# WxuanYuan/diffusynth

Measured on AMD Instinct MI355X. Metric: denoising-steps/sec (batch x T) on 256x64 latents, higher is better.
Workload: dtype bf16x3; 1 GPU; BASELINE configs[2]: DiffSynthSampler.sample() wall-clock, production ConditionedUnet (random init, torch.manual_seed(0)), bf16x3 (fp32 tensors, dense convolutions as 3 bf16 MFMA terms with fp32 accumulation: meets 1e-3 vs the fp32 reference), batch 64/GPU, latent (4,256,64), text condition, CFG=6.0 (U-Net batch 128 per step), 33-step respaced ddpm schedule, Philox noise on device; global_batch=64, parallelism=batch-shard x1, weights replicated

## Files before the change

### diffusynth_amd/_lib.py

```python
import ctypes as C
import os
import re

_HERE = os.path.dirname(os.path.abspath(__file__))
_HEADER = os.path.join(os.path.dirname(_HERE), "include", "diffusynth_hip.h")
_LIBNAME = "libdiffusynth_hip.so"

DS_F32, DS_BF16 = 0, 1
ACT_NONE, ACT_GELU, ACT_SILU, ACT_RELU = 0, 1, 2, 3
from .conv_policy import (TILE_64x192, TILE_128x32, TILE_128x192, TILE_256x96, TILE_HALO3_256x96, TILE_HALO3_N16,
                          TILE_INIT7, TILE_QUAD_HALO3)

_SCALARS = {"int32_t": C.c_int32, "int": C.c_int, "float": C.c_float, "double": C.c_double, "int64_t": C.c_int64,
            "uint64_t": C.c_uint64, "size_t": C.c_size_t}


def _parse_structs(text):
    text = re.sub(r"/\*.*?\*/", "", text, flags=re.S)
    out = {}
    for body, name in re.findall(r"typedef\s+struct\s*\{(.*?)\}\s*(\w+)\s*;", text, flags=re.S):
        fields = []
        for decl in body.split(";"):
            decl = " ".join(decl.split())
            if not decl:
                continue
            if "*" in decl:
                names = decl.rsplit("*", 1)[1]
                ctype = C.c_void_p
            else:
                tname, names = decl.replace("const ", "").split(" ", 1)
                ctype = _SCALARS[tname]
            for n in names.split(","):
                fields.append((n.strip(), ctype))
        out[name] = type(name, (C.Structure,), {"_fields_": fields})
    return out


def _parse_defines(text, prefix):
    return {k: int(v) for k, v in re.findall(r"^#define\s+(%s\w*)\s+(-?\d+)\b" % prefix, text, flags=re.M)}


with open(_HEADER) as _f:
    _HEADER_TEXT = _f.read()
_STRUCTS = _parse_structs(_HEADER_TEXT)
SR = _parse_defines(_HEADER_TEXT, "DS_SR_")
CR = _parse_defines(_HEADER_TEXT, "DS_CR_")
DW_FAMILY = {v: k[6:].lower() for k, v in _parse_defines(_HEADER_TEXT, "DS_DW_").items()}
PV = _parse_defines(_HEADER_TEXT, "DS_PV_")
MIX_BLOCK = _parse_defines(_HEADER_TEXT, "DS_MIX_")["DS_MIX_BLOCK"]
TAIL = _parse_defines(_HEADER_TEXT, "DS_TAIL_")
ConvParams = _STRUCTS["ds_conv_params"]
PackConvParams = _STRUCTS["ds_pack_conv_params"]
DwconvParams = _STRUCTS["ds_dwconv_params"]
GnApplyParams = _STRUCTS["ds_gn_apply_params"]
AttnParams = _STRUCTS["ds_attn_params"]
StepParams = _STRUCTS["ds_step_params"]
StepRowsParams = _STRUCTS["ds_step_rows_params"]
DpmStepParams = _STRUCTS["ds_dpm_step_params"]
CfgRescaleParams = _STRUCTS["ds_cfg_rescale_params"]
CfgRescaleRowsParams = _STRUCTS["ds_cfg_rescale_rows_params"]
AttnFusedParams = _STRUCTS["ds_attn_fused_params"]
AttnX3Params = _STRUCTS["ds_attn_x3_params"]
VqAttnParams = _STRUCTS["ds_vq_attn_params"]

_P, _I, _F, _D, _SZ, _U64 = C.c_void_p, C.c_int, C.c_float, C.c_double, C.c_size_t, C.c_uint64
_PROTOS = {
    "ds_abi_version": (C.c_int, []),
    "ds_conv_igemm": (C.c_int, [C.POINTER(ConvParams), _P]),
    "ds_conv_splitk_reduce": (C.c_int, [C.POINTER(ConvParams), _P]),
    "ds_conv1x1_x3": (C.c_int, [C.POINTER(ConvParams), _P]),
    "ds_conv1x1_x3_stats_parts": (C.c_int, [C.POINTER(ConvParams)]),
    "ds_conv1x1_x3_weight_elems": (C.c_size_t, [_I, _I]),
    "ds_conv_stats_parts": (C.c_int, [C.POINTER(ConvParams)]),
    "ds_conv_tile_bn": (C.c_int, [_I]),
    "ds_pack_conv_weight": (C.c_int, [C.POINTER(PackConvParams), _P]),
    "ds_pack_conv_elems": (_SZ, [_I, _I, _I, _I, _I]),
    "ds_conv_fold_tables": (C.c_int, [_P, _P, _P, _P, _I, _I, _I, _I, _P, _P, _P]),
    "ds_dwconv7": (C.c_int, [C.POINTER(DwconvParams), _P]),
    "ds_dwconv_stats_parts": (C.c_int, [C.POINTER(DwconvParams)]),
    "ds_dwconv_launch_choice": (C.c_int, [C.POINTER(DwconvParams), C.POINTER(C.c_int32), C.POINTER(C.c_int32), C.POINTER(C.c_int32)]),
    "ds_pack_dw_weight": (C.c_int, [_P, _I, _P, _P]),
    "ds_pack_dw_weight_mfma": (C.c_int, [_P, _I, _P, _P]),
    "ds_split_planes": (C.c_int, [_P, _P, C.c_longlong, _I, _P]),
    "ds_gn_finalize": (C.c_int, [_P, _I, _I, _D, _F, _P, _P]),
    "ds_gn_stats": (C.c_int, [_P, _I, _I, _I, _I, _I, _F, _P, _P]),
    "ds_gn_stats_stream": (C.c_int, [_P, _I, _I, _I, _I, _I, _F, _P, _P, _P]),
    "ds_gn_stats_ws_floats": (_SZ, [_I, _I, _I]),
    "ds_gn_apply": (C.c_int, [C.POINTER(GnApplyParams), _P]),
    "ds_linattn_context": (C.c_int, [C.POINTER(AttnParams), _P]),
    "ds_linattn_output": (C.c_int, [C.POINTER(AttnParams), _P]),
    "ds_linattn_part_floats": (_SZ, [_I, _I, _I]),
    "ds_pack_attn_fused": (C.c_int, [_P, _P, _P, _P, _P, _I, _P]),
    "ds_attn_fused_context": (C.c_int, [C.POINTER(AttnFusedParams), _P]),
    "ds_attn_fused_output": (C.c_int, [C.POINTER(AttnFusedParams), _P]),
    "ds_attn_fused_stats_parts": (C.c_int, [C.POINTER(AttnFusedParams)]),
    "ds_attn_fused_generations": (C.c_int, [C.POINTER(AttnFusedParams)]),
    "ds_attn_fused_segments": (C.c_int, [_I, _I, _I]),
    "ds_attn_fused_segments_gen": (C.c_int, [_I, _I, _I, _I]),
    "ds_pack_attn_x3": (C.c_int, [_P, _P, _P, _I, _P]),
    "ds_attn_x3_context": (C.c_int, [C.POINTER(AttnX3Params), _P]),
    "ds_attn_x3_output": (C.c_int, [C.POINTER(AttnX3Params), _P]),
    "ds_attn_x3_stats_parts": (C.c_int, [C.POINTER(AttnX3Params)]),
    "ds_attn_x3_segments": (C.c_int, [_I, _I, _I]),
    "ds_vq_attn_segments": (C.c_int, [_I, _I, _I]),
    "ds_vq_attn_wfold_bytes": (_SZ, [_I, _I]),
    "ds_vq_attn_context": (C.c_int, [C.POINTER(VqAttnParams), _P]),
    "ds_vq_attn_output": (C.c_int, [C.POINTER(VqAttnParams), _P]),
    "ds_attn_x3_qplane_bytes": (_SZ, [_I, _I]),
    "ds_attn_x3_mfold_bytes": (_SZ, [_I, _I]),
    "ds_sinusoid": (C.c_int, [_P, _P, _I, _I, _P, _P]),
    "ds_linear": (C.c_int, [_P, _I, _P, _P, _I, _I, _I, _I, _P, _I, _P]),
    "ds_conv3x3_f32_n4_weight_floats": (C.c_size_t, [_I]),
    "ds_pack_conv3x3_f32_n4": (C.c_int, [_P, _P, _I, _I, _P, _P]),
    "ds_conv3x3_f32_n4": (C.c_int, [_P, _I, _I, _I, _I, _P, _P, _P]),
    "ds_activation": (C.c_int, [_P, C.c_size_t, _I, _P, _P]),
    "ds_add_layernorm": (C.c_int, [_P, _P, _P, _P, _I, _I, _F, _P, _P]),
    "ds_dup_batch": (C.c_int, [_P, _P, _SZ, _P]),
    "ds_nchw_to_nhwc": (C.c_int, [_P, _I, _I, _I, _I, _P, _I, _I, _P]),
    "ds_conv1x1_in_nchw": (C.c_int, [_P, _I, _I, _I, _P, _P, _I, _P, _P]),
    "ds_nhwc_to_nchw": (C.c_int, [_P, _I, _I, _I, _I, _I, _I, _P, _P]),
    "ds_ddim_step": (C.c_int, [C.POINTER(StepParams), _P]),
    "ds_step_rows": (C.c_int, [C.POINTER(StepRowsParams), _P]),
    "ds_dpm_step": (C.c_int, [C.POINTER(DpmStepParams), _P]),
    "ds_dpm_step_rows": (C.c_int, [C.POINTER(StepRowsParams), _P, _P]),
    "ds_cfg_rescale": (C.c_int, [C.POINTER(CfgRescaleParams), _P]),
    "ds_cfg_rescale_rows": (C.c_int, [C.POINTER(CfgRescaleRowsParams), _P]),
    "ds_philox_normal": (C.c_int, [_P, _SZ, _U64, _U64, _P]),
    "ds_gather_cols": (C.c_int, [_P, _I, _I, _P, _I, _P, _P]),
    "ds_vq_nearest": (C.c_int, [_P, _P, _P, _I, _I, _I, _I, _P, _P, _P]),
    "ds_vq_stats_ws_bytes": (_SZ, [_I]),
    "ds_vq_stats": (C.c_int, [_P, _P, _P, _I, _I, _I, _I, _F, _I, _P, _P, _P]),
    "ds_decoder_tail": (C.c_int, [_P, _I, _I, _I, _I, _P, _P]),
    "ds_dec_final": (C.c_int, [_P, _I, _I, _I, _I, _P, _I, _P, _P, _P, _P, _P, _P, _P, _P]),
    "ds_conv7x7_c4_weight_elems": (C.c_size_t, []),
    "ds_pack_conv7x7_c4": (C.c_int, [_P, _I, _I, _P, _P]),
    "ds_conv7x7_c4": (C.c_int, [_P, _I, _I, _I, _I, _P, _P, _P, _P]),
    "ds_pack_conv7x7_c4_x3": (C.c_int, [_P, _I, _I, _P, _P]),
    "ds_conv7x7_c4_x3": (C.c_int, [_P, _I, _I, _I, _P, _P, _P, _P]),
    "ds_conv3x3_c80_weight_elems": (C.c_size_t, []),
    "ds_pack_conv3x3_c80": (C.c_int, [_P, _I, _I, _P, _P]),
    "ds_conv3x3_c80": (C.c_int, [_P, _I, _I, _I, _P, _P, _P, _P, _I, _P, _P, _I, _I, _P, _P]),
    "ds_conv3x3_c80_stats_slots": (C.c_int, [_I, _I, _I]),
    "ds_conv3x3_c80_res": (C.c_int, [_P, _P, _I, _I, _I, _P, _P, _P, _P, _P]),
    "ds_convt4x4_c80_stats_slots": (C.c_int, [_I, _I, _I, _I]),
    "ds_gn_stats_finish": (C.c_int, [_P, _I, _I, _I, _I, _I, _F, _P, _P]),
    "ds_convt4x4_c80_weight_elems": (C.c_size_t, [_I]),
    "ds_pack_convt4x4_c80": (C.c_int, [_P, _I, _I, _P, _P]),
    "ds_convt4x4_c80": (C.c_int, [_P, _I, _I, _I, _I, _P, _P, _P, _P, _I, _P, _P, _P, _P]),
    "ds_istft_plus": (C.c_int, [_P, _I, _I, _I, _I, _P, _P, _P]),
    "ds_istft_ws_floats": (_SZ, [_I, _I, _I]),
    "ds_stft_plus": (C.c_int, [_P, _I, _I, _I, _I, _I, _P, _P]),
    "ds_stft_images_ws_floats": (_SZ, [_I, _I, _I]),
    "ds_stft_images": (C.c_int, [_P, _P, C.c_longlong, _I, _I, _I, _P, _P, _P, _P]),
    "ds_latent_image_ws_floats": (_SZ, [_I, _I]),
    "ds_latent_image": (C.c_int, [_P, _I, _I, _I, _I, _P, _P, _P]),
    "ds_pv_stft": (C.c_int, [_P, _P, _I, _I, C.c_longlong, C.c_longlong, _P, _P]),
    "ds_pv_vocode": (C.c_int, [_P, _P, _P, _P, _I, C.c_longlong, C.c_longlong, _P, _P]),
    "ds_pv_istft_ws_bytes": (_SZ, [C.c_longlong]),
    "ds_pv_istft": (C.c_int, [_P, _P, _I, _I, _I, C.c_longlong, C.c_longlong, _P, _P, _P]),
    "ds_resample_sinc": (C.c_int, [_P, _P, _P, _I, _I, C.c_longlong, C.c_longlong, _P, _P]),
    "ds_peak_normalize_ws_bytes": (_SZ, [_I, _I]),
    "ds_peak_normalize": (C.c_int, [_P, _P, _I, _I, C.c_longlong, _P, _P, _P]),
    "ds_mix_notes": (C.c_int, [_P, C.c_longlong, _P, _I, _P, _P, _I, _P, _I, _P]),
    "ds_lstm_ws_floats": (_SZ, [_I, _I]),
    "ds_lstm_layer": (C.c_int, [_P, C.c_longlong, C.c_longlong, _P, _I, _I, _I, _P, _P, _P, _P]),
    "ds_timbre_heads": (C.c_int, [_P, _I, _I, _I, _I, _I, _I, _P]),
    "ds_text_embed": (C.c_int, [_P, _I, _I, _I, _P, _I, _P, _I, _P, _P, _P, _I, _F, _P, _P]),
    "ds_text_attention": (C.c_int, [_P, _P, _I, _I, _I, _I, _I, _P, _P]),
    "ds_text_tail": (C.c_int, [_P, _I, _I, _I, _F, _P, _P]),
    "ds_bounds_report": (C.c_int, [C.c_char_p, _I, _I]),
}
_UNCHECKED = {"ds_conv3x3_f32_n4_weight_floats", "ds_bounds_report", "ds_abi_version", "ds_conv_stats_parts", "ds_conv1x1_x3_stats_parts", "ds_conv_tile_bn", "ds_dwconv_stats_parts", "ds_attn_fused_stats_parts", "ds_attn_fused_generations", "ds_attn_fused_segments", "ds_attn_fused_segments_gen", "ds_attn_x3_stats_parts", "ds_attn_x3_segments", "ds_vq_attn_segments", "ds_conv3x3_c80_stats_slots", "ds_convt4x4_c80_stats_slots"}
EXPORTS = sorted(list(_PROTOS) + ["ds_last_error_string"])

_lib = None


def lib_path():
    return os.path.join(_HERE, os.environ.get("DS_LIB", _LIBNAME))


class DsError(RuntimeError):
    pass


def load():
    global _lib
    if _lib is not None:
        return _lib
    path = lib_path()
    if not os.path.exists(path):
        raise DsError(f"{path} is missing: build it with `python -c 'import __graft_entry__ as g; g.build()'` "
                      "(hipcc --offload-arch=gfx950).  diffusynth_amd has no CPU fallback.")
    lib = C.CDLL(path)
    lib.ds_last_error_string.restype = C.c_char_p
    lib.ds_last_error_string.argtypes = []
    for name, (res, args) in _PROTOS.items():
        fn = getattr(lib, name)
        fn.restype, fn.argtypes = res, args
    _lib = lib
    return lib


def check(rc, what=""):
    if rc != 0:
        msg = load().ds_last_error_string().decode("utf-8", "replace")
        raise DsError(f"{what} failed with code {rc}: {msg}")


def call(name, *args):
    rc = getattr(load(), name)(*args)
    if name not in _UNCHECKED:
        check(rc, name)
    return rc


def ptr(t):
    return None if t is None else t.data_ptr()


def current_stream():
    import torch
    return C.c_void_p(torch.cuda.current_stream().cuda_stream)
```

### diffusynth_amd/conv_policy.py

```python
from collections import namedtuple

KSPLIT_FILL = 256
TILE_128x192, TILE_256x96, TILE_128x32, TILE_64x192 = 0, 1, 2, 3
TILE_HALO3_256x96, TILE_QUAD_HALO3, TILE_HALO3_N16, TILE_INIT7 = 11, 12, 13, 14
_IGEMM_BM_BN = {TILE_64x192: (64, 192), TILE_128x192: (128, 192), TILE_256x96: (256, 96)}


def up(x, m):
    return (x + m - 1) // m * m


class ConvLayer(namedtuple("ConvLayer", "Cout Cin cin_pad k transposed gain halo small_out bf16 split3")):
    bn = property(lambda s: 32 if s.small_out else 192 if s.Cout % 192 == 0 else 96)
    cout_pad = property(lambda s: up(s.Cout, s.bn))
    dense3x3 = property(lambda s: s.k == (3, 3) and not s.transposed and s.cin_pad == s.Cin and s.Cin % 32 == 0)
    k_order = property(lambda s: int(s.halo and s.bf16 and s.k == (3, 3) and not s.transposed and s.cin_pad % 32 == 0 and s.bn in (96, 192)))
    f32n4_fits = property(lambda s: not s.bf16 and not s.gain and s.dense3x3 and s.Cout <= 4)
    n16_fits = property(lambda s: s.bf16 and not s.gain and s.dense3x3 and s.Cout <= 16)
    x3_1x1_fits = property(lambda s: s.split3 and s.k == (1, 1) and not s.transposed and s.cin_pad == s.Cin and s.Cin % 32 == 0
                           and s.Cout % 8 == 0)
    split3_fits = property(lambda s: s.halo and s.split3 and s.dense3x3 and s.cout_pad % 96 == 0 and s.Cout % 8 == 0)
    init7_fits = property(lambda s: s.bf16 and s.k == (7, 7) and s.Cout == 96 and s.Cin <= 4 and s.cin_pad in (4, 8))
    init7x3_fits = property(lambda s: s.split3 and s.k == (7, 7) and s.Cout == 96 and s.Cin <= 4 and s.cin_pad == 4)

    @property
    def quad_fits(s):
        return ((s.bf16 or (s.split3 and s.Cout % 8 == 0)) and not s.gain and s.cin_pad == s.Cin and s.Cin % 32 == 0 and s.k == (4, 4)
                and ((s.transposed and (s.Cin // 32) % 6 == 0 and s.Cout % 96 == 0) or (not s.transposed and (s.Cin // 32) % 3 == 0)))


def igemm_tile(bn, npix, korder):
    if korder == 1:
        return TILE_HALO3_256x96
    if bn == 192:
        return TILE_64x192 if npix <= 1024 else TILE_128x192
    return TILE_256x96 if bn == 96 else TILE_128x32


def halo_patches(H, W):
    twl = 3
    while (1 << twl) < W and twl < 5:
        twl += 1
    return -(-H // (256 >> twl)) * -(-W // (1 << twl))


def _fill(blocks, factors):
    ks = 1
    if blocks < KSPLIT_FILL:
        for c in factors:
            ks = c
            if blocks * c >= KSPLIT_FILL:
                break
    return ks


def halo3_ksplit(B, H, W, cout_pad, ncc, split):
    ok = [c for c in ((2, 3, 4, 6, 8) if split else (2, 4, 8)) if ncc % c == 0 and ncc // c >= (1 if split else 2)]
    return _fill(halo_patches(H, W) * (cout_pad // 96) * B, ok)


def quad_ksplit(B, Ho, Wo, cout_pad, nch, split):
    ok = [c for c in ((2, 3, 4, 6, 8) if split else (2, 4, 8)) if nch % c == 0 and (nch // c) % 6 == 0]
    return _fill(halo_patches(Ho, Wo) * (cout_pad // 96) * B, ok)


def x3_1x1_ksplit(B, Ho, Wo, cout_pad, nq):
    ok = [c for c in (2, 3, 4, 6, 8) if nq // c >= 3 and (c - 1) * -(-nq // c) < nq]
    return _fill(-(-(Ho * Wo) // 256) * (cout_pad // 96) * B, ok)


def igemm_ksplit(B, tile, Ho, Wo, cout_pad, nq, phases):
    if tile not in _IGEMM_BM_BN:
        return 1
    bm, bn = _IGEMM_BM_BN[tile]
    blocks = -(-(Ho * Wo) // bm) * (cout_pad // bn) * B * phases
    ks = 1
    while ks < 8 and blocks * ks < 384 and nq // (ks * 2) >= 6:
        ks *= 2
    while ks > 1 and (ks - 1) * -(-nq // ks) >= nq:
        ks //= 2
    return ks


def conv_meta(tile, B, Ho, Wo, Cout, kh, kw, transposed, cin, cin_real, res_cin=0):
    flops = 2.0 * B * Ho * Wo * Cout * (16 if transposed else kh * kw) * min(cin, cin_real)
    if res_cin:
        flops += 2.0 * B * Ho * Wo * Cout * res_cin
    return (tile, flops, f"{kh}x{kw}{'T' if transposed else ''} {cin}->{Cout} @{Ho}x{Wo}" + (f" +1x1 {res_cin}" if res_cin else ""))
```

### diffusynth_amd/csrc/conv1x1_x3.hip

```cpp
#include "common.hpp"
#include "conv_halo3_common.hpp"

namespace {

constexpr int X3_OFF_XH = 0, X3_OFF_XL = BM * PSTR, X3_OFF_WH = 2 * BM * PSTR, X3_OFF_WL = X3_OFF_WH + B_BYTES, X3_OFF_SHL = X3_OFF_WL + B_BYTES;
constexpr int X3_OFF_RED = X3_OFF_SHL + SHL_BYTES, X3_LDS = X3_OFF_RED + 64;
constexpr int X3_XIT = BM * 8 / NT;
constexpr int X3_WIT = 2 * BN * 4 / NT;

static_assert(4 * EPI_F32_WAVE <= X3_OFF_SHL, "the epilogue's staging tiles reuse the x / w buffers, the shift table stays");

__global__ __launch_bounds__(NT, DS_MINBLK) void conv1x1_x3_kernel(const ds_conv_params p) {
    extern __shared__ __attribute__((aligned(16))) char smem[];
    float* const shl = reinterpret_cast<float*>(smem + X3_OFF_SHL);
    float* const red = reinterpret_cast<float*>(smem + X3_OFF_RED);
    const int tid = threadIdx.x, lane = tid & 63, wave = tid >> 6, m = lane & 15, q = lane >> 4;
    const int gy = p.cout_pad / BN, HW = p.H * p.W, gx = (HW + BM - 1) / BM, nwg = gridDim.x;
    int wid = blockIdx.x;
    if ((nwg & 7) == 0) wid = (wid & 7) * (nwg >> 3) + (wid >> 3);
    const int by = wid % gy, bxz = wid / gy, bx = bxz % gx;
    const int zb = bxz / gx, ksplit = p.ksplit > 1 ? p.ksplit : 1, kz = zb / p.B;
    const int b = zb - kz * p.B, n0 = by * BN, px0 = bx * BM;
    const int NC0 = p.C0 >> 5, NCC = (p.C0 + p.C1) >> 5;
    const int ncs = (NCC + ksplit - 1) / ksplit, c_lo = kz * ncs, c_hi = min(NCC, c_lo + ncs);
    const bool raw = p.ksplit > 1;

    const float* const sp0 = reinterpret_cast<const float*>(p.src0) + (size_t)b * HW * p.C0;
    const float* const sp1 = p.C1 ? reinterpret_cast<const float*>(p.src1) + (size_t)b * p.H1 * p.W1 * p.C1 : nullptr;
    unsigned off0[X3_XIT], off1[X3_XIT];
#pragma unroll
    for (int it = 0; it < X3_XIT; ++it) {
        const int px = px0 + (tid >> 3) + 32 * it;
        off0[it] = ((unsigned)(px * p.C0 + 4 * (tid & 7)) * 4u & 0x7fffffffu) | ((unsigned)(px >= HW) << 31);
        off1[it] = 0x80000000u;
        if (p.C1) {
            const int h = px / p.W - p.off_h1, w = px % p.W - p.off_w1;
            const unsigned bad = (unsigned)(px >= HW) | (unsigned)((unsigned)h >= (unsigned)p.H1) | (unsigned)((unsigned)w >= (unsigned)p.W1);
            off1[it] = ((unsigned)((h * p.W1 + w) * p.C1 + 4 * (tid & 7)) * 4u & 0x7fffffffu) | (bad << 31);
        }
    }
    const rsrc_t rs0 = __builtin_amdgcn_make_buffer_rsrc(const_cast<float*>(sp0), (short)0, HW * p.C0 * 4, 0x00020000);
    const rsrc_t rs1 = __builtin_amdgcn_make_buffer_rsrc(const_cast<float*>(p.C1 ? sp1 : sp0), (short)0, p.C1 ? p.H1 * p.W1 * p.C1 * 4 : 0, 0x00020000);
    const char* const wbase = reinterpret_cast<const char*>(p.wpk);
    const size_t wchunk = (size_t)2 * p.cout_pad * 64;
    f32x4 rx[X3_XIT];
    u32x4 rw[X3_WIT];
    auto load_chunk = [&](int cc) {
        const bool first = cc < NC0;
        const float* const s = first ? sp0 : sp1;
        const int c0 = (first ? cc : cc - NC0) * 32;
#if DS_BOUNDS
#pragma unroll
        for (int it = 0; it < X3_XIT; ++it) {
            const unsigned o = first ? off0[it] : off1[it];
            const bool in = o < 0x80000000u;
            const f32x4 v = DS_LD(f32x4, reinterpret_cast<const f32x4*>(reinterpret_cast<const char*>(s) + (in ? o + c0 * 4 : 0)), first ? DS_BX_SRC0 : DS_BX_SRC1);
            rx[it] = in ? v : f32x4{0.f, 0.f, 0.f, 0.f};
        }
#else
        (void)s;
#pragma unroll
        for (int it = 0; it < X3_XIT; ++it)
            rx[it] = __builtin_bit_cast(f32x4, __builtin_amdgcn_raw_buffer_load_b128(first ? rs0 : rs1, (int)((first ? off0[it] : off1[it]) + c0 * 4), 0, 0));
#endif
#pragma unroll
        for (int it = 0; it < X3_WIT; ++it) {
            const int piece = tid + it * NT, plane = piece / (BN * 4), r = piece - plane * (BN * 4);
            rw[it] = DS_LD(u32x4, reinterpret_cast<const u32x4*>(wbase + (size_t)cc * wchunk + ((size_t)plane * p.cout_pad + n0) * 64 + (size_t)r * 16), DS_BX_W);
        }
    };
    auto store_chunk = [&]() {
#pragma unroll
        for (int it = 0; it < X3_XIT; ++it) {
            const int pl = (tid >> 3) + 32 * it, e = tid & 7;
            const int a = pl * PSTR + ((((e >> 1) ^ (((pl >> 2) & 1) << 1))) << 4) + ((e & 1) << 3);
            const f32x4 v = rx[it];
            uint2 hi, lo;
            ds_split2(v[0], v[1], hi.x, lo.x);
            ds_split2(v[2], v[3], hi.y, lo.y);
            *reinterpret_cast<uint2*>(smem + X3_OFF_XH + a) = hi;
            *reinterpret_cast<uint2*>(smem + X3_OFF_XL + a) = lo;
        }
#pragma unroll
        for (int it = 0; it < X3_WIT; ++it) {
            const int piece = tid + it * NT, plane = piece / (BN * 4), r = piece - plane * (BN * 4), row = r >> 2, qq = r & 3;
            *reinterpret_cast<u32x4*>(smem + (plane ? X3_OFF_WL : X3_OFF_WH) + row * PSTR + ((qq ^ W_SWZ(row)) << 4)) = rw[it];
        }
    };

    load_chunk(c_lo);
    float gn_a = 1.f, gn_am = 0.f;
    const bool fold = p.gn_ab != nullptr && !raw;
    if (fold) {
        gn_a = DS_LD(float, p.gn_ab + 2 * b, DS_BX_GNAB);
        gn_am = DS_LD(float, p.gn_ab + 2 * b + 1, DS_BX_GNAB);
    }
    for (int e = tid; e < 10 * BN; e += NT) {
        float v = 0.f;
        const int n = n0 + e;
        if (e < BN && n < p.Cout) {
            if (fold) v = DS_LD(float, p.fold_t1 + n, DS_BX_T1) - gn_am * DS_LD(float, p.fold_t2 + n, DS_BX_T2);
            else if (p.bias && !raw) v = DS_LD(float, p.bias + n, DS_BX_BIAS);
        }
        shl[e] = v;
    }
    int xa[XT];
#pragma unroll
    for (int i = 0; i < XT; ++i) {
        const int pl = 64 * wave + 16 * i + m;
        xa[i] = pl * PSTR + ((q ^ (((pl >> 2) & 1) << 1)) << 4);
    }
    const int wa = W_ROW0(m) * PSTR + ((q ^ ((-(m >> 2)) & 3)) << 4);
    f32x4 acc[XT][WT];
#pragma unroll
    for (int i = 0; i < XT; ++i)
#pragma unroll
        for (int j = 0; j < WT; ++j) acc[i][j] = f32x4{0.f, 0.f, 0.f, 0.f};

    for (int cc = c_lo; cc < c_hi; ++cc) {
        store_chunk();
        __syncthreads();
        if (cc + 1 < c_hi) load_chunk(cc + 1);
        bf16x8 xh[XT], xl[XT];
#pragma unroll
        for (int i = 0; i < XT; ++i) {
            xh[i] = *reinterpret_cast<const bf16x8*>(smem + X3_OFF_XH + xa[i]);
            xl[i] = *reinterpret_cast<const bf16x8*>(smem + X3_OFF_XL + xa[i]);
        }
#pragma unroll
        for (int j = 0; j < WT; ++j) {
            const bf16x8 wh = *reinterpret_cast<const bf16x8*>(smem + X3_OFF_WH + wa + EPI_CH(j) * PSTR);
            const bf16x8 wl = *reinterpret_cast<const bf16x8*>(smem + X3_OFF_WL + wa + EPI_CH(j) * PSTR);
#pragma unroll
            for (int i = 0; i < XT; ++i) {
                acc[i][j] = __builtin_amdgcn_mfma_f32_16x16x32_bf16(wl, xh[i], acc[i][j], 0, 0, 0);
                acc[i][j] = __builtin_amdgcn_mfma_f32_16x16x32_bf16(wh, xl[i], acc[i][j], 0, 0, 0);
                acc[i][j] = __builtin_amdgcn_mfma_f32_16x16x32_bf16(wh, xh[i], acc[i][j], 0, 0, 0);
            }
        }
        __syncthreads();
    }

    auto coord2 = [&](int i, int mm) {
        ConvCoord c;
        const int px = px0 + 64 * wave + 16 * i + mm;
        c.ok = px < HW;
        c.ho = 0;
        c.wo = 0;
        c.pix = px;
        return c;
    };
    auto coord = [&](int i) { return coord2(i, m); };
    float s1 = 0.f, s2 = 0.f;
    char* const stage = smem + wave * EPI_F32_WAVE;
    if (raw) {
        ds_conv_params qp = p;
        qp.out = p.slab;
        qp.out_C = (p.Cout + 7) / 8 * 8;
        qp.out_c0 = 0;
        qp.res = nullptr;
        halo3_epilogue_rows_f32<false, false>(qp, acc, zb, n0, HW, shl, coord, coord2, stage, s1, s2, 1.0f, lane);
        return;
    }
    if (p.res) halo3_epilogue_rows_f32<false, true>(p, acc, b, n0, HW, shl, coord, coord2, stage, s1, s2, gn_a, lane);
    else halo3_epilogue_rows_f32<false, false>(p, acc, b, n0, HW, shl, coord, coord2, stage, s1, s2, gn_a, lane);
    if (p.stats_part) block_stats_write(s1, s2, red, p.stats_part + ((size_t)b * (gx * gy) + by * gx + bx) * 2);
}

}

extern "C" size_t ds_conv1x1_x3_weight_elems(int Cin, int Cout) { return (size_t)((Cin + 31) / 32) * 2 * ((Cout + BN - 1) / BN * BN) * 32; }

int ds_conv_splitk_parts(const ds_conv_params* p);
extern "C" int ds_conv1x1_x3_stats_parts(const ds_conv_params* p) {
    return p->ksplit > 1 ? ds_conv_splitk_parts(p) : ((p->H * p->W + BM - 1) / BM) * (p->cout_pad / BN);
}

extern "C" int ds_conv1x1_x3(const ds_conv_params* p, void* stream) {
    DS_REQUIRE(p && p->src0 && p->wpk && p->out, "conv1x1_x3: null pointer");
    DS_REQUIRE(p->KH == 1 && p->KW == 1 && p->stride == 1 && p->pad_h == 0 && p->pad_w == 0 && !p->transposed && p->Ho == p->H && p->Wo == p->W,
               "conv1x1_x3: 1x1 stride 1 only");
    DS_REQUIRE(p->B > 0 && p->H > 0 && p->W > 0 && p->Cout > 0, "conv1x1_x3: empty problem");
    DS_REQUIRE(p->batch_hint >= 0, "conv1x1_x3: batch_hint must be 0 or a batch (this launcher takes no decision from either), got %d", p->batch_hint);
    DS_REQUIRE(p->C0 > 0 && p->C0 % 32 == 0 && p->C1 >= 0 && p->C1 % 32 == 0, "conv1x1_x3: channel counts (%d,%d) must be multiples of 32", p->C0, p->C1);
    DS_REQUIRE(p->C1 == 0 || (p->src1 && p->H1 > 0 && p->W1 > 0), "conv1x1_x3: second source incomplete");
    DS_REQUIRE(p->cout_pad % BN == 0 && p->Cout <= p->cout_pad, "conv1x1_x3: cout_pad %d must be a multiple of %d", p->cout_pad, BN);
    DS_REQUIRE(p->flags == (DS_CONV_F_IN_F32 | DS_CONV_F_OUT_F32) && p->act == DS_ACT_NONE && !p->res_steps && !p->gn_part && !p->out_nchw_f32,
               "conv1x1_x3: fp32 in / fp32 out (flags = DS_CONV_F_IN_F32 | DS_CONV_F_OUT_F32), no activation, no fused res_conv, statistics through gn_ab");
    {
        const int nq = (p->C0 + p->C1) / 32, ks = p->ksplit, nqs = ks > 1 ? (nq + ks - 1) / ks : nq;
        DS_REQUIRE(ks <= 1 || (p->slab && (ks == 2 || ks == 3 || ks == 4 || ks == 6 || ks == 8) && (ks - 1) * nqs < nq),
                   "conv1x1_x3: ksplit=%d needs a slab, a value in {2, 3, 4, 6, 8} and no empty slice over %d chunks", ks, nq);
    }
    DS_REQUIRE(!p->gn_ab || (p->fold_t1 && p->fold_t2 && p->ncls == 1), "conv1x1_x3: the GroupNorm fold needs t1 / t2 tables with one border class");
    DS_REQUIRE(p->out_C % 4 == 0 && p->out_c0 % 4 == 0 && p->out_C >= p->out_c0 + p->Cout && p->Cout % 8 == 0, "conv1x1_x3: out_C / out_c0 multiples of 4, Cout a multiple of 8");
    DS_REQUIRE((long long)p->H * p->W * p->out_C * 4 < (1ll << 31) && (long long)p->H * p->W * p->C0 * 4 < (1ll << 31) && (long long)p->H1 * p->W1 * p->C1 * 4 < (1ll << 31),
               "conv1x1_x3: one sample of the output and of either source must stay below 2 GiB (32-bit buffer offsets)");
    if (!ds_aligned16(p->src0) || !ds_aligned16(p->wpk) || !ds_aligned16(p->out) || (p->C1 && !ds_aligned16(p->src1)) || (p->res && !ds_aligned16(p->res)))
        DS_FAIL(DS_EALIGN, "conv1x1_x3: tensors must be 16-byte aligned");
    hipStream_t st = reinterpret_cast<hipStream_t>(stream);
    const int gx = (p->H * p->W + BM - 1) / BM, gy = p->cout_pad / BN;
    dim3 grid(gx * gy * p->B * (p->ksplit > 1 ? p->ksplit : 1));
#if DS_BOUNDS
    {
        DsBxHost h(DS_K_CONV_IGEMM);
        const int NCC = (p->C0 + p->C1) / 32;
        h.set(DS_BX_SRC0, p->src0, (long long)p->B * p->H * p->W * p->C0 * 4);
        h.set(DS_BX_SRC1, p->C1 ? p->src1 : nullptr, (long long)p->B * p->H1 * p->W1 * p->C1 * 4);
        h.set(DS_BX_W, p->wpk, (long long)NCC * 2 * p->cout_pad * 64);
        if (p->ksplit > 1) h.set(DS_BX_OUT, p->slab, (long long)p->ksplit * p->B * p->H * p->W * ((p->Cout + 7) / 8 * 8) * 4);
        else h.set(DS_BX_OUT, p->out, (long long)p->B * p->H * p->W * p->out_C * 4);
        h.set(DS_BX_RES, p->res, (long long)p->B * p->H * p->W * p->out_C * 4);
        h.set(DS_BX_BIAS, p->bias, (long long)p->Cout * 4);
        h.set(DS_BX_T1, p->fold_t1, (long long)p->Cout * 4).set(DS_BX_T2, p->fold_t2, (long long)p->Cout * 4);
        h.set(DS_BX_GNAB, p->gn_ab, (long long)p->B * 2 * 4);
        h.set(DS_BX_STATS, p->stats_part, (long long)p->B * gx * gy * 2 * 4);
        h.publish(st);
    }
#endif
    DS_SET_MAX_LDS(conv1x1_x3_kernel, X3_LDS, "conv1x1_x3");
    hipLaunchKernelGGL(conv1x1_x3_kernel, grid, dim3(NT), X3_LDS, st, *p);
    DS_CHECK_LAUNCH("conv1x1_x3");
    return DS_OK;
}

#if DS_BOUNDS
extern "C" int ds_bounds_fetch_conv1x1_x3(ds_bounds_rec* out, int reset) { return ds_bounds_fetch_tu(out, reset); }
#endif
```

### diffusynth_amd/csrc/conv3x3_halo3.hip

```cpp
#include "common.hpp"
#ifndef DS_STAMP
#define DS_STAMP 0
#endif
#if DS_BOUNDS
void ds_conv_bounds_table(const ds_conv_params& p, int kernel, int stats_parts, ds_bx* out);
#endif

#include "conv_halo3_common.hpp"

namespace {

__device__ __attribute__((aligned(16))) float g_gelu_lut[GELU_TAB_N];

#ifdef DS_FORCE_VGPRS
#define DS_VGPR_ATTR __attribute__((amdgpu_num_vgpr(DS_FORCE_VGPRS)))
#else
#define DS_VGPR_ATTR
#endif
template <int TWL, bool HP, bool PAIR = false>
__global__ __launch_bounds__(NT, PAIR ? 1 : DS_MINBLK) DS_VGPR_ATTR void conv3x3_halo3_kernel(const ds_conv_params p) {
    static_assert(!PAIR || (HP && TWL == 3), "two samples per block: the 8 x 32 tile of the split-precision instantiation");
    using G = HG<TWL>;
    constexpr int TW = G::TW, TH = G::TH, HCP = G::HCP, NPX = G::NPX, H_IT = G::H_IT, HH0 = G::HH0, HH1 = G::HH1;
    extern __shared__ __attribute__((aligned(16))) char smem[];
    float* const shl = reinterpret_cast<float*>(smem + OFF_SHL);
    float* const red = reinterpret_cast<float*>(smem + OFF_B);

    const int tid = threadIdx.x, lane = tid & 63, wave = tid >> 6;
    const long st_k0 = DS_STAMP ? __builtin_amdgcn_s_memrealtime() : 0;
    const int m = lane & 15, q = lane >> 4;
    const int tiles_w = (p.W + TW - 1) >> TWL;
    const int gx = gridDim.x, gy = gridDim.y, nwg = gx * gy * gridDim.z;
    int wid = blockIdx.x + gx * (blockIdx.y + gy * blockIdx.z);
    if ((nwg & 7) == 0) wid = (wid & 7) * (nwg >> 3) + (wid >> 3);
    constexpr int NGROUP = 2;
    int by, bxz;
    if (gy % NGROUP == 0 && gy > NGROUP) {
        const int lo = wid % NGROUP, t = wid / NGROUP, nxz = gx * (int)gridDim.z;
        bxz = t % nxz;
        by = (t / nxz) * NGROUP + lo;
    } else {
        by = wid % gy;
        bxz = wid / gy;
    }
    const int bx = bxz % gx, bz = bxz / gx;
    const int th = bx / tiles_w, tw = bx - th * tiles_w;
    const int h0 = th * TH, w0 = tw * TW;
    const int ksplit = p.ksplit > 1 ? p.ksplit : 1;
    const int b = (PAIR ? 2 : 1) * (bz / ksplit), kz = bz - (bz / ksplit) * ksplit, n0 = by * BN;
    const bool has2 = PAIR && b + 1 < p.B;
    constexpr bool split_in = HP;
    const int Cin = p.C0, NSRC = Cin >> 5;
    const int NCC = (split_in ? NSRC + (NSRC >> 1) : NSRC) / ksplit;
    const int cc_lo = kz * NCC;
    const int nsteps = NCC * 9;
    auto src_chunk = [&](int cc) {
        const int v = cc_lo + cc;
        if (!split_in) return v;
        const int c = v / 3, j = v - 3 * c;
        return j == 2 ? (NSRC >> 1) + c : c;
    };

    const int NR = (HP || ksplit > 1) ? 0 : p.res_steps, R0 = p.res_C0 >> 5;
    const char* const wbase = reinterpret_cast<const char*>(p.wpk);
    const unsigned wbytes = (unsigned)(NCC * ksplit * 9 + p.res_steps) * p.cout_pad * 64;
    const rsrc_t rs_w = __builtin_amdgcn_make_buffer_rsrc(const_cast<char*>(wbase), (short)0, (int)wbytes, 0x00020000);

    unsigned hvo[H_IT];
    rsrc_t rs_h;
    const char* hbase;
    int h_buf = DS_BX_SRC0;
    auto use_source = [&](const void* ptr, int sH, int sW, int sC, int offh, int offw, bool centre_only, int bounds_buf) {
        hbase = reinterpret_cast<const char*>(ptr) + (size_t)b * sH * sW * sC * 2;
        rs_h = __builtin_amdgcn_make_buffer_rsrc(const_cast<char*>(hbase), (short)0, (int)((unsigned)sH * sW * sC * 2) * (has2 ? 2 : 1), 0x00020000);
        h_buf = bounds_buf;
#pragma unroll
        for (int it = 0; it < H_IT; ++it) {
            const int slot = tid + it * NT, hp = slot >> 2, dq = slot & 3;
            int hr = hp / HCP;
            const int hc = hp - hr * HCP;
            const int smp = PAIR ? (int)(hr >= 18) : 0;
            if constexpr (PAIR) hr -= 18 * smp;
            const int hi = h0 + hr - 1 - offh, wi = w0 + hc - 1 - offw;
            const unsigned ring = (unsigned)(hr < 1) | (unsigned)(hr > TH) | (unsigned)(hc < 1) | (unsigned)(hc > TW);
            const unsigned bad = (unsigned)(hp >= (PAIR ? 36 * HCP : NPX)) | (unsigned)(hc >= TW + 2) | ((unsigned)centre_only & ring) |
                                 (unsigned)((unsigned)hi >= (unsigned)sH) | (unsigned)((unsigned)wi >= (unsigned)sW) | (unsigned)(smp && !has2);
            hvo[it] = (((unsigned)(((smp * sH + hi) * sW + wi) * sC + dq * 8) * 2u) & 0x7fffffffu) | (bad << 31);
        }
    };
    unsigned h_so = 0;
    auto set_res_src = [&](int r) {
        if (r == R0 && r < NR) use_source(p.res_src1, p.res_H1, p.res_W1, p.res_C1, p.res_off_h1, p.res_off_w1, true, DS_BX_AUX1);
        if (r == NR) use_source(p.src0, p.H, p.W, Cin, 0, 0, false, DS_BX_SRC0);
        h_so = r == NR ? (unsigned)src_chunk(0) * 64u : (unsigned)(r < R0 ? r : r - R0) * 64u;
    };
    if (NR > 0) use_source(p.res_src0, p.H, p.W, p.res_C0, 0, 0, true, DS_BX_AUX0);
    else use_source(p.src0, p.H, p.W, Cin, 0, 0, false, DS_BX_SRC0);

    const int lds_h = OFF_H + (tid >> 2) * PSTR + (((tid & 3) ^ (((tid >> 4) & 1) << 1)) << 4);
    const int wr0 = tid >> 2, wr1 = 64 + (tid >> 2);
    const int bst0 = OFF_B + wr0 * PSTR + (((tid & 3) ^ W_SWZ(wr0)) << 4);
    const int bst1 = tid < BN * 4 - NT ? OFF_B + wr1 * PSTR + (((tid & 3) ^ W_SWZ(wr1)) << 4) : OFF_B + B_BYTES;
    const unsigned wvo0 = (unsigned)tid * 16u, wvo1 = tid < BN * 4 - NT ? (unsigned)(tid + NT) * 16u : VOFF_NONE;
    const unsigned wstep = (unsigned)p.cout_pad * 64u;
    const unsigned w_first = ((unsigned)(p.res_steps - NR + cc_lo * 9) * p.cout_pad + n0) * 64u, w_last = w_first + (unsigned)(nsteps + NR - 1) * wstep;
    unsigned w_pf = w_first;

    u32x4 rb[3][2], rh[H_IT];
    auto load_b = [&](auto slotc) {
        constexpr int sl = decltype(slotc)::value;
        rb[sl][0] = buf_ld16(rs_w, wbase, wvo0, w_pf, DS_BX_W);
        rb[sl][1] = buf_ld16(rs_w, wbase, wvo1, w_pf, DS_BX_W);
        const unsigned nx = w_pf + wstep;
        w_pf = nx < w_last ? nx : w_last;
    };
    auto store_b = [&](auto slotc, auto bufc) {
        constexpr int sl = decltype(slotc)::value, buf = decltype(bufc)::value;
        *reinterpret_cast<u32x4*>(smem + buf * B_STRIDE + bst0) = rb[sl][0];
        *reinterpret_cast<u32x4*>(smem + buf * B_STRIDE + bst1) = rb[sl][1];
    };
    auto load_halo_to = [&](u32x4* dst, auto halfc) {
        constexpr int half = decltype(halfc)::value, n = half ? HH1 : HH0;
#pragma unroll
        for (int k = 0; k < n; ++k) dst[k] = buf_ld16(rs_h, hbase, hvo[half * HH0 + k], h_so, h_buf);
    };
    auto load_halo = [&](auto halfc) { load_halo_to(rh, halfc); };
    auto store_halo_from = [&](const u32x4* src, auto bufc, auto halfc) {
        constexpr int buf = decltype(bufc)::value, half = decltype(halfc)::value, n = half ? HH1 : HH0;
#pragma unroll
        for (int k = 0; k < n; ++k) *reinterpret_cast<u32x4*>(smem + lds_h + buf * G::HB + (half * HH0 + k) * 64 * PSTR) = src[k];
    };
    auto store_halo = [&](auto bufc, auto halfc) { store_halo_from(rh, bufc, halfc); };

    int xb[XT];
#pragma unroll
    for (int i = 0; i < XT; ++i) {
        int row_l, col_l;
        halo_tile_rc<TWL>(wave, i, m, row_l, col_l);
        const int hp0 = (row_l + (PAIR ? 2 * (row_l >> 4) : 0)) * HCP + col_l;
        xb[i] = OFF_H + hp0 * PSTR + ((q ^ (((hp0 >> 2) & 1) << 1)) << 4);
    }
    static_assert(((HCP >> 2) & 1) == 1 && ((2 * HCP >> 2) & 1) == 0, "tap-row swizzle flips assume HCP / 4 odd");
    const int xm1 = ((m & 3) == 3) << 5, xm2 = ((m & 3) >= 2) << 5;
    const int xm1n = xm1 ^ 32, xm2n = xm2 ^ 32;
    const int bw = OFF_B + W_ROW0(m) * PSTR + ((q ^ ((-(m >> 2)) & 3)) << 4);

    bf16x8 fx[2][XT], fw[WT];
    auto read_x = [&](auto setc, auto tyc, auto txc, int imm) {
        constexpr int set = decltype(setc)::value, ty = decltype(tyc)::value, tx = decltype(txc)::value;
#pragma unroll
        for (int i = 0; i < XT; ++i) {
            int a = xb[i];
            if constexpr (HP) {
                if constexpr (tx == 1) a ^= xm1;
                if constexpr (tx == 2) a ^= xm2;
                if constexpr (ty == 1) {
                    if constexpr (tx != 0) asm volatile("" : "+v"(a));
                    a ^= 32;
                }
            } else {
                if constexpr (tx == 0 && ty == 1) a ^= 32;
                if constexpr (tx == 1) a ^= (ty == 1 ? xm1n : xm1);
                if constexpr (tx == 2) a ^= (ty == 1 ? xm2n : xm2);
            }
            fx[set][i] = *reinterpret_cast<const bf16x8*>(smem + a + (ty * HCP + tx) * PSTR + imm);
        }
    };
#ifndef DS_HALO3_ABL
#define DS_HALO3_ABL 0
#endif
    auto read_w = [&](int j, int imm) { fw[j] = *reinterpret_cast<const bf16x8*>(smem + bw + EPI_CH(j) * PSTR + imm); };
    f32x4 acc[XT][WT];
    auto mma_j = [&](auto setc, int j) {
        constexpr int set = decltype(setc)::value;
#pragma unroll
        for (int i = 0; i < XT; ++i) acc[i][j] = __builtin_amdgcn_mfma_f32_16x16x32_bf16(fw[j], fx[set][i], acc[i][j], 0, 0, 0);
    };
    using I0 = std::integral_constant<int, 0>;
    using I1 = std::integral_constant<int, 1>;
    using I2 = std::integral_constant<int, 2>;

    GnPartialLoads gnl;
    const bool raw = ksplit > 1;
    if (p.gn_part && !raw) gn_partials_issue(p.gn_part, p.gn_parts, b, gnl);
    const bool fold = !raw && CONV_FOLD(p);
    const int ncls = fold ? p.ncls : 1;
    constexpr int ST_IT = (10 * BN + NT - 1) / NT;
#if !DS_BOUNDS
    float t1v[ST_IT], t2v[ST_IT], rbv[ST_IT];
    {
        auto tab = [&](const float* ptr, int n) {
            return __builtin_amdgcn_make_buffer_rsrc(const_cast<char*>(ptr ? reinterpret_cast<const char*>(ptr) : wbase), (short)0, ptr ? n * 4 : 0, 0x00020000);
        };
        const bool use_bias = !fold && p.bias && !raw;
        const rsrc_t rs_t1 = tab(fold ? p.fold_t1 : (use_bias ? p.bias : nullptr), fold ? ncls * p.Cout : p.Cout);
        const rsrc_t rs_t2 = tab(fold ? p.fold_t2 : nullptr, ncls * p.Cout);
        const rsrc_t rs_rb = tab((NR > 0 && p.res_bias) ? p.res_bias : nullptr, p.Cout);
#pragma unroll
        for (int k = 0; k < ST_IT; ++k) {
            const int e = tid + k * NT, cls = e / BN, n = n0 + e - cls * BN;
            const unsigned bad = ((unsigned)(e >= ncls * BN) | (unsigned)(n >= p.Cout)) << 31;
            const unsigned o = (unsigned)((fold ? cls * p.Cout : 0) + n) * 4u;
            t1v[k] = __builtin_bit_cast(float, __builtin_amdgcn_raw_buffer_load_b32(rs_t1, (int)((o & 0x7fffffffu) | bad), 0, 0));
            t2v[k] = __builtin_bit_cast(float, __builtin_amdgcn_raw_buffer_load_b32(rs_t2, (int)((o & 0x7fffffffu) | bad), 0, 0));
            rbv[k] = NR > 0 ? __builtin_bit_cast(float, __builtin_amdgcn_raw_buffer_load_b32(rs_rb, (int)((((unsigned)n * 4u) & 0x7fffffffu) | bad), 0, 0)) : 0.f;
        }
    }
#endif
    const bool use_lut = !HP && G::LUT && p.act == DS_ACT_GELU && !raw;
    static_assert(GELU_TAB_N * 4 <= 2 * NT * 16 && GELU_TAB_N % 4 == 0, "the table is staged as two 16-byte vectors per thread");
    u32x4 lutv = {0u, 0u, 0u, 0u}, lutv2 = {0u, 0u, 0u, 0u};
    if (use_lut) {
        lutv = *reinterpret_cast<const u32x4*>(reinterpret_cast<const char*>(g_gelu_lut) + tid * 16);
        lutv2 = *reinterpret_cast<const u32x4*>(reinterpret_cast<const char*>(g_gelu_lut) + (NT + min(tid, GELU_TAB_N / 4 - NT - 1)) * 16);
    }
    const long st_p1 = DS_STAMP ? __builtin_amdgcn_s_memrealtime() : 0;
    u32x4 rh2[HH0];
    h_so = NR > 0 ? 0u : (unsigned)src_chunk(0) * 64u;
    load_halo_to(rh2, I0{});
    load_halo(I1{});
    load_b(I0{});
    load_b(I1{});
    float gn_a = 1.f, gn_am = 0.f;
    if (raw) {
    } else if (p.gn_part) gn_partials_finish(gnl, p.gn_part, p.gn_parts, p.gn_count, p.gn_eps, b, gn_a, gn_am);
    else if (p.gn_ab) {
        gn_a = DS_LD(float, p.gn_ab + 2 * b, DS_BX_GNAB);
        gn_am = DS_LD(float, p.gn_ab + 2 * b + 1, DS_BX_GNAB);
    }
    if constexpr (PAIR) {
        const int b1 = has2 ? b + 1 : b;
        float a1 = 1.f, am1 = 0.f;
        if (p.gn_part) gn_from_partials(p.gn_part, p.gn_parts, p.gn_count, p.gn_eps, b1, a1, am1);
        else if (p.gn_ab) {
            a1 = DS_LD(float, p.gn_ab + 2 * b1, DS_BX_GNAB);
            am1 = DS_LD(float, p.gn_ab + 2 * b1 + 1, DS_BX_GNAB);
        }
        if (tid == 0) {
            reinterpret_cast<float*>(smem + G::LDS)[0] = a1;
            reinterpret_cast<float*>(smem + G::LDS)[1] = am1;
        }
    }
#if DS_BOUNDS
    conv_shift_table<BN, 10, NT>(raw ? conv_kslice_view(p) : p, fold, n0, gn_am, NR > 0 ? p.res_bias : nullptr, shl);
#else
#pragma unroll
    for (int k = 0; k < ST_IT; ++k) {
        const int e = tid + k * NT;
        if (e < 10 * BN) shl[e] = (t1v[k] + rbv[k]) - gn_am * t2v[k];
    }
#endif
    const long st_p2 = DS_STAMP ? __builtin_amdgcn_s_memrealtime() : 0;
#pragma unroll
    for (int i = 0; i < XT; ++i)
#pragma unroll
        for (int j = 0; j < WT; ++j) acc[i][j] = f32x4{0.f, 0.f, 0.f, 0.f};
    if (use_lut) {
        *reinterpret_cast<u32x4*>(smem + G::OFF_LUT + tid * 16) = lutv;
        if (tid < GELU_TAB_N / 4 - NT) *reinterpret_cast<u32x4*>(smem + G::OFF_LUT + (NT + tid) * 16) = lutv2;
    }
    store_halo_from(rh2, I0{}, I0{});
    store_halo(I0{}, I1{});
    store_b(I0{}, I0{});
    store_b(I1{}, I1{});
    load_b(I2{});
    load_b(I0{});
    load_b(I1{});
    __syncthreads();

    if constexpr (!HP) if (NR > 0) {
        set_res_src(1);
        load_halo_to(rh, I0{});
        load_halo_to(rh + HH0, I1{});
        auto res_step = [&](auto hbc, auto phc, int r) {
            constexpr int hb = decltype(hbc)::value, ph = decltype(phc)::value, rs = (ph + 2) % 3;
            read_x(I0{}, I1{}, I1{}, hb * G::HB);
#pragma unroll
            for (int j = 0; j < WT; ++j) read_w(j, ph * B_STRIDE);
            __builtin_amdgcn_sched_barrier(0);
            store_halo_from(rh, std::integral_constant<int, hb ^ 1>{}, I0{});
            store_halo_from(rh + HH0, std::integral_constant<int, hb ^ 1>{}, I1{});
            store_b(std::integral_constant<int, rs>{}, std::integral_constant<int, rs>{});
            __builtin_amdgcn_sched_barrier(0);
            load_b(std::integral_constant<int, rs>{});
            if (r + 2 <= NR) {
                set_res_src(r + 2);
                __builtin_amdgcn_sched_barrier(0);
                load_halo_to(rh, I0{});
                load_halo_to(rh + HH0, I1{});
            }
            __builtin_amdgcn_sched_barrier(0);
#pragma unroll
            for (int j = 0; j < WT; ++j) mma_j(I0{}, j);
            __builtin_amdgcn_sched_barrier(0);
            __syncthreads();
        };
        for (int r = 0; r < NR; r += 6) {
            res_step(I0{}, I0{}, r);
            res_step(I1{}, I1{}, r + 1);
            res_step(I0{}, I2{}, r + 2);
            if (r + 3 < NR) {
                res_step(I1{}, I0{}, r + 3);
                res_step(I0{}, I1{}, r + 4);
                res_step(I1{}, I2{}, r + 5);
            }
        }
        const float inv_a = 1.0f / gn_a;
#pragma unroll
        for (int i = 0; i < XT; ++i)
#pragma unroll
            for (int j = 0; j < WT; ++j)
#pragma unroll
                for (int r = 0; r < 4; ++r) acc[i][j][r] *= inv_a;
    }
    const int par = HP ? 0 : (NR & 1);
    if (par) read_x(I1{}, I0{}, I0{}, G::HB);
    else read_x(I0{}, I0{}, I0{}, 0);
#pragma unroll
    for (int j = 0; j < WT; ++j) read_w(j, 0);

    auto chunk = [&](auto hbufc, auto keepc, auto fsc, int cc) {
        constexpr int hbuf = decltype(hbufc)::value, KEEP = decltype(keepc)::value, FS = decltype(fsc)::value;
        if constexpr (!KEEP) h_so = (unsigned)src_chunk(cc + 1 < NCC ? cc + 1 : cc) * 64u;
        auto step = [&](auto tapc) {
            constexpr int tap = decltype(tapc)::value;
            constexpr int rs = (tap + 2) % 3;
            constexpr int cur = (tap + FS) & 1;
            constexpr int ntap = (tap + 1) % 9, nty = ntap / 3, ntx = ntap % 3, nhb = (tap == 8 && !KEEP) ? (hbuf ^ 1) : hbuf;
            constexpr int nW = 2 + (KEEP ? 0 : (tap == 3 ? HH0 : (tap == 7 ? HH1 : 0))), nV = 2 + (KEEP ? 0 : (tap == 1 ? HH0 : (tap == 4 ? HH1 : 0)));
            if constexpr (tap == 3 && !KEEP) store_halo(std::integral_constant<int, hbuf ^ 1>{}, I0{});
            if constexpr (tap == 7 && !KEEP) store_halo(std::integral_constant<int, hbuf ^ 1>{}, I1{});
            store_b(std::integral_constant<int, rs>{}, std::integral_constant<int, rs>{});
            load_b(std::integral_constant<int, rs>{});
            if constexpr (tap == 1 && !KEEP) load_halo(I0{});
            if constexpr (tap == 4 && !KEEP) load_halo(I1{});
            mma_j(std::integral_constant<int, (DS_HALO3_ABL & 2) ? 0 : cur>{}, 0);
            if constexpr (!(DS_HALO3_ABL & 1)) read_w(0, ((tap + 1) % 3) * B_STRIDE);
            if constexpr (!(DS_HALO3_ABL & 2))
                read_x(std::integral_constant<int, cur ^ 1>{}, std::integral_constant<int, nty>{}, std::integral_constant<int, ntx>{}, nhb * G::HB);
#pragma unroll
            for (int j = 1; j < WT; ++j) {
                mma_j(std::integral_constant<int, (DS_HALO3_ABL & 2) ? 0 : cur>{}, j);
                if constexpr (!(DS_HALO3_ABL & 1)) read_w(j, ((tap + 1) % 3) * B_STRIDE);
            }
#pragma unroll
            for (int k = 0; k < nW; ++k) { SGB(SG_MFMA, 1); SGB(SG_DSW, 1); }
#pragma unroll
            for (int k = 0; k < nV; ++k) { SGB(SG_MFMA, 1); SGB(SG_VMEM, 1); }
            constexpr int L0 = nW + nV;
#pragma unroll
            for (int k = 0; k < 5; ++k) { SGB(SG_MFMA, 1); SGB(SG_DSR, 1); }
            constexpr int L1 = L0 + 5;
#pragma unroll
            for (int j = 1; j < WT; ++j) {
                const int before = (4 * j + 4 > L1 + j - 1 ? 4 * j + 4 : L1 + j - 1);
                const int prev = j == 1 ? L1 : (4 * (j - 1) + 4 > L1 + j - 2 ? 4 * (j - 1) + 4 : L1 + j - 2);
                if (before - prev == 1) SGB(SG_MFMA, 1);
                else if (before - prev == 2) SGB(SG_MFMA, 2);
                else if (before - prev == 3) SGB(SG_MFMA, 3);
                else if (before - prev == 4) SGB(SG_MFMA, 4);
                else if (before - prev == 5) SGB(SG_MFMA, 5);
                else if (before - prev == 6) SGB(SG_MFMA, 6);
                else if (before - prev == 7) SGB(SG_MFMA, 7);
                SGB(SG_DSR, 1);
            }
            __builtin_amdgcn_sched_barrier(0);
#if DS_BOUNDS || defined(DS_LGKM0)
            asm volatile("s_waitcnt lgkmcnt(0)" ::: "memory");
#else
            asm volatile("s_waitcnt lgkmcnt(10)" ::: "memory");
#endif
            if constexpr (!(DS_HALO3_ABL & 4)) __builtin_amdgcn_s_barrier();
            __builtin_amdgcn_sched_barrier(0);
        };
        step(std::integral_constant<int, 0>{});
        step(std::integral_constant<int, 1>{});
        step(std::integral_constant<int, 2>{});
        step(std::integral_constant<int, 3>{});
        step(std::integral_constant<int, 4>{});
        step(std::integral_constant<int, 5>{});
        step(std::integral_constant<int, 6>{});
        step(std::integral_constant<int, 7>{});
        step(std::integral_constant<int, 8>{});
    };
    long st_t0 = 0, st_r0 = 0;
    if constexpr (DS_STAMP) {
        st_t0 = __builtin_amdgcn_s_memtime();
        st_r0 = __builtin_amdgcn_s_memrealtime();
        __builtin_amdgcn_s_waitcnt(0xC07F);
    }
    if constexpr (HP) {
        int cc = 0;
        for (; cc + 6 <= NCC; cc += 6) {
            chunk(I0{}, I1{}, I0{}, cc);
            chunk(I0{}, I0{}, I1{}, cc + 1);
            chunk(I1{}, I0{}, I0{}, cc + 2);
            chunk(I0{}, I1{}, I1{}, cc + 3);
            chunk(I0{}, I0{}, I0{}, cc + 4);
            chunk(I1{}, I0{}, I1{}, cc + 5);
        }
        if (cc < NCC) {
            chunk(I0{}, I1{}, I0{}, cc);
            chunk(I0{}, I0{}, I1{}, cc + 1);
            chunk(I1{}, I0{}, I0{}, cc + 2);
        }
    } else {
        int cc0 = 0;
        if (par) {
            chunk(I1{}, I0{}, I1{}, 0);
            cc0 = 1;
        }
        for (int cc = cc0; cc < NCC; cc += 2) {
            chunk(I0{}, I0{}, I0{}, cc);
            if (cc + 1 < NCC) chunk(I1{}, I0{}, I1{}, cc + 1);
        }
    }

#pragma unroll
    for (int i = 0; i < XT; ++i) {
        asm volatile("" ::"v"(fx[0][i]));
        asm volatile("" ::"v"(fx[1][i]));
    }
#pragma unroll
    for (int j = 0; j < WT; ++j) asm volatile("" ::"v"(fw[j]));
    if constexpr (DS_STAMP) {
        const long st_t1 = __builtin_amdgcn_s_memtime();
        if (p.slab && lane == 0) {
            long* d = reinterpret_cast<long*>(p.slab) + ((size_t)(bz * gy + by) * gx + bx) * 32 + wave * 8;
            d[0] = st_t1 - st_t0; d[1] = st_p1 - st_k0; d[2] = st_p2 - st_k0; d[3] = nsteps;
            d[4] = st_r0 - st_k0; d[5] = __builtin_amdgcn_s_memrealtime() - st_r0; d[6] = st_k0;
        }
    }
    auto at = [&](int row_l, int col_l) {
        ConvCoord c;
        if constexpr (PAIR) {
            const int smp = row_l >> 4;
            c.ho = row_l & 15;
            c.wo = w0 + col_l;
            c.ok = c.ho < p.H && c.wo < p.W && (!smp || has2);
            c.pix = (smp * p.H + c.ho) * p.W + c.wo;
            return c;
        }
        c.ho = h0 + row_l;
        c.wo = w0 + col_l;
        c.ok = c.ho < p.H && c.wo < p.W;
        c.pix = c.ho * p.W + c.wo;
        return c;
    };
    auto coord2 = [&](int i, int mm) { int row_l, col_l; halo_tile_rc<TWL>(wave, i, mm, row_l, col_l); return at(row_l, col_l); };
    auto coord = [&](int i) { return coord2(i, m); };
    char* const stage = smem + OFF_H + wave * EPI_F32_WAVE;
    static_assert(4 * EPI_F32_WAVE <= 2 * G::HB, "the staging tiles fit the halo buffers");
    float s1 = 0.f, s2 = 0.f;
    const int outHW = p.H * p.W;
    const long st_e1 = DS_STAMP ? __builtin_amdgcn_s_memrealtime() : 0;
    const int out_mode = HP ? (p.flags >> 1) & 3 : 0;
    const float* shl_w = shl;
    float ga_w = gn_a;
    int b_e = b, outHW_e = outHW;
    if constexpr (PAIR) {
        const float gn_a1 = reinterpret_cast<const float*>(smem + G::LDS)[0], gn_am1 = reinterpret_cast<const float*>(smem + G::LDS)[1];
        float* const shl1 = reinterpret_cast<float*>(smem + OFF_H + 4 * EPI_F32_WAVE);
        static_assert(4 * EPI_F32_WAVE + SHL_BYTES <= 2 * G::HB, "the second shift table fits the halo buffers too");
        conv_shift_table<BN, 10, NT>(p, fold, n0, gn_am1, nullptr, shl1);
        __syncthreads();
        if (__builtin_amdgcn_readfirstlane(wave) >= 2) {
            shl_w = shl1;
            ga_w = gn_a1;
        }
        b_e = b >> 1;
        outHW_e = 2 * outHW;
    }
    if (raw) {
        halo3_epilogue_hp<DS_ACT_NONE, 2>(conv_kslice_view(p), acc, kz * p.B + b, n0, outHW, shl, coord, s1, s2, 1.0f, lane);
    } else if constexpr (HP) {
      if (out_mode == 1) {
        if (p.act == DS_ACT_GELU) halo3_epilogue_hp<DS_ACT_GELU, 1>(p, acc, b_e, n0, outHW_e, shl_w, coord, s1, s2, ga_w, lane);
        else halo3_epilogue_hp<DS_ACT_NONE, 1>(p, acc, b_e, n0, outHW_e, shl_w, coord, s1, s2, ga_w, lane);
      } else if (out_mode == 2) {
        if (p.res) halo3_epilogue_rows_f32<true, true>(p, acc, b_e, n0, outHW_e, shl_w, coord, coord2, stage, s1, s2, ga_w, lane);
        else halo3_epilogue_rows_f32<true, false>(p, acc, b_e, n0, outHW_e, shl_w, coord, coord2, stage, s1, s2, ga_w, lane);
      } else {
        if (p.act == DS_ACT_GELU) halo3_epilogue<DS_ACT_GELU, true, false>(p, acc, b_e, n0, outHW_e, shl_w, coord, s1, s2, ga_w, lane);
        else halo3_epilogue<DS_ACT_NONE, true, false>(p, acc, b_e, n0, outHW_e, shl_w, coord, s1, s2, ga_w, lane);
      }
    } else
    if (p.act == DS_ACT_GELU) {
        const char* const lut = smem + G::OFF_LUT;
        if (use_lut) {
            if (p.res) halo3_epilogue<DS_ACT_GELU, true, true, true>(p, acc, b, n0, outHW, shl, coord, s1, s2, gn_a, lane, lut);
            else halo3_epilogue<DS_ACT_GELU, true, false, true>(p, acc, b, n0, outHW, shl, coord, s1, s2, gn_a, lane, lut);
        } else {
            if (p.res) halo3_epilogue<DS_ACT_GELU, true, true>(p, acc, b, n0, outHW, shl, coord, s1, s2, gn_a, lane);
            else halo3_epilogue<DS_ACT_GELU, true, false>(p, acc, b, n0, outHW, shl, coord, s1, s2, gn_a, lane);
        }
    } else {
        if (p.res) halo3_epilogue_rows<DS_ACT_NONE, true, true>(p, acc, b, n0, outHW, shl, coord, coord2, stage, s1, s2, gn_a, lane);
        else halo3_epilogue<DS_ACT_NONE, true, false>(p, acc, b, n0, outHW, shl, coord, s1, s2, gn_a, lane);
    }
    long st_e2 = 0, st_e3 = 0;
    if constexpr (DS_STAMP) {
        st_e2 = __builtin_amdgcn_s_memrealtime();
        __builtin_amdgcn_s_waitcnt(0x0F70);
        st_e3 = __builtin_amdgcn_s_memrealtime();
    }
    __syncthreads();
    if (p.stats_part && !raw) {
        const int parts = gridDim.x * gridDim.y;
        if constexpr (PAIR) {
            s1 = wave_sum(s1);
            s2 = wave_sum(s2);
            if (lane == 0) {
                red[2 * wave] = s1;
                red[2 * wave + 1] = s2;
            }
            __syncthreads();
            if (lane == 0 && (wave == 0 || (wave == 2 && has2))) {
                float* const dst = p.stats_part + ((size_t)(b + (wave >> 1)) * parts + by * gx + bx) * 2;
                DS_ST(float, dst, DS_BX_STATS, red[2 * wave] + red[2 * wave + 2]);
                DS_ST(float, dst + 1, DS_BX_STATS, red[2 * wave + 1] + red[2 * wave + 3]);
            }
        } else
        block_stats_write(s1, s2, red, p.stats_part + ((size_t)b * parts + by * gx + bx) * 2);
    }
    if constexpr (DS_STAMP) {
        if (p.slab && lane == 0) {
            long* d = reinterpret_cast<long*>(p.slab) + ((size_t)(bz * gy + by) * gx + bx) * 32 + wave * 8;
            d[7] = __builtin_amdgcn_s_memrealtime() - st_k0;
            if (DS_STAMP == 2) { d[1] = st_e2 - st_e1; d[2] = st_e3 - st_e2; }
        }
    }
}

}

int ds_conv3x3_halo3_parts(const ds_conv_params* p) {
    const int twl = halo_twl(p->W), TW = 1 << twl, TH = BM >> twl;
    return ((p->H + TH - 1) / TH) * ((p->W + TW - 1) / TW) * (p->cout_pad / BN);
}

static int halo3_batch(const ds_conv_params* p) { return p->batch_hint > 0 ? p->batch_hint : p->B; }

int ds_conv3x3_halo3_launch(const ds_conv_params* p, hipStream_t st) {
    DS_REQUIRE(p->dtype == DS_BF16, "conv3x3_halo3: bf16 only");
    DS_REQUIRE(p->KH == 3 && p->KW == 3 && p->stride == 1 && p->pad_h == 1 && p->pad_w == 1 && !p->transposed,
               "conv3x3_halo3: 3x3 stride 1 pad 1 only");
    DS_REQUIRE(p->C1 == 0 && p->C0 % 32 == 0, "conv3x3_halo3: single source, Cin multiple of 32 (got %d+%d)", p->C0, p->C1);
    DS_REQUIRE(p->Ho == p->H && p->Wo == p->W && !p->out_nchw_f32, "conv3x3_halo3: same-size NHWC output only");
    DS_REQUIRE(p->cout_pad % BN == 0 && p->wk_order == 1, "conv3x3_halo3: cout_pad %% 96 == 0 and chunk-major weights (wk_order = 1)");
    const bool split_in = (p->flags & DS_CONV_F_SPLIT_IN) != 0;
    DS_REQUIRE(p->ksplit <= 1 || (p->slab && (p->flags == 0 || split_in) && ((split_in ? p->C0 / 64 : p->C0 / 32) % p->ksplit) == 0 && !p->res_steps),
               "conv3x3_halo3: ksplit=%d needs a slab, must divide the %d source chunks and excludes the fused res_conv", p->ksplit, split_in ? p->C0 / 64 : p->C0 / 32);
    const int out_mode = (p->flags >> 1) & 3;
    DS_REQUIRE(out_mode <= 2 && (p->flags & ~7) == 0, "conv3x3_halo3: unknown flags %d", p->flags);
    DS_REQUIRE(!split_in || (p->C0 % 64 == 0 && !p->res_steps), "conv3x3_halo3: split input needs C0 = 2C with C %% 32 == 0 and no fused res_conv");
    DS_REQUIRE(p->flags == 0 || split_in, "conv3x3_halo3: the split-precision launches (flags != 0) take a split input (DS_CONV_F_SPLIT_IN)");
    DS_REQUIRE(out_mode == 0 || !p->res_steps, "conv3x3_halo3: split / fp32 output excludes the fused res_conv");
    DS_REQUIRE(out_mode != 2 || p->act == DS_ACT_NONE, "conv3x3_halo3: fp32 output has no activation variant");
    DS_REQUIRE(!p->res || out_mode == 2 || p->flags == 0, "conv3x3_halo3: in the split-precision modes a residual needs the fp32 output");
    DS_REQUIRE(out_mode != 1 || p->out_C >= p->out_c0 + 2 * p->Cout, "conv3x3_halo3: split output needs out_C >= 2 Cout");
    const int nchunks = split_in ? (p->C0 / 32) * 3 / 2 : p->C0 / 32;
    if (p->res_steps) {
        DS_REQUIRE(!p->res, "conv3x3_halo3: a fused res_conv excludes a residual tensor");
        DS_REQUIRE(p->res_src0 && p->res_C0 > 0 && p->res_C0 % 32 == 0 && p->res_C1 % 32 == 0 && p->res_steps == (p->res_C0 + p->res_C1) / 32 &&
                       p->res_steps % 3 == 0,
                   "conv3x3_halo3: res_conv channels (%d,%d) must be multiples of 32 (96 in total) and res_steps = their chunks", p->res_C0, p->res_C1);
        DS_REQUIRE(p->res_C1 == 0 || (p->res_src1 && p->res_H1 > 0 && p->res_W1 > 0), "conv3x3_halo3: second res_conv source incomplete");
        DS_REQUIRE(ds_aligned16(p->res_src0) && (!p->res_C1 || ds_aligned16(p->res_src1)), "conv3x3_halo3: res_conv sources must be 16-byte aligned");
    }
    DS_REQUIRE((long long)p->H * p->W * (p->C0 > p->res_C0 ? p->C0 : p->res_C0) * 2 < (1ll << 31) &&
                   (long long)(nchunks * 9 + p->res_steps) * p->cout_pad * 64 < (1ll << 31),
               "conv3x3_halo3: one sample / the packed weights must stay below 2 GiB (32-bit buffer offsets)");
    DS_REQUIRE((long long)p->H * p->W * p->out_C * (out_mode == 2 ? 4 : 2) < (1ll << 31), "conv3x3_halo3: one output sample must stay below 2 GiB (32-bit buffer offsets)");
    const int twl = halo_twl(p->W), TW = 1 << twl, TH = BM >> twl;
    const bool pair = p->flags != 0 && twl == 3 && 2 * p->H <= TH && p->W <= TW && p->ksplit <= 1 && !p->res_steps && halo3_batch(p) >= 2;
    dim3 grid(((p->H + TH - 1) / TH) * ((p->W + TW - 1) / TW), p->cout_pad / BN, pair ? (p->B + 1) / 2 : p->B * (p->ksplit > 1 ? p->ksplit : 1));
#if DS_BOUNDS
    {
        DsBxHost h(DS_K_CONV_HALO);
        ds_conv_bounds_table(*p, DS_K_CONV_HALO, grid.x * grid.y, &h.t);
        h.set(DS_BX_W, p->wpk, (long long)(nchunks * 9 + p->res_steps) * p->cout_pad * 64);
        h.set(DS_BX_AUX0, p->res_steps ? p->res_src0 : nullptr, (long long)p->B * p->H * p->W * p->res_C0 * 2);
        h.set(DS_BX_AUX1, p->res_C1 ? p->res_src1 : nullptr, (long long)p->B * p->res_H1 * p->res_W1 * p->res_C1 * 2);
        h.set(DS_BX_AUX2, p->res_bias, (long long)p->Cout * 4);
        if (out_mode == 2) {
            h.set(DS_BX_OUT, p->out, (long long)p->B * p->H * p->W * p->out_C * 4);
            h.set(DS_BX_RES, p->res, (long long)p->B * p->H * p->W * p->out_C * 4);
        }
        h.publish(st);
    }
#endif
    {
        static DsDevOnce once;
        int dev;
        if (once.need(&dev)) {
            float h[GELU_TAB_N];
            auto T = [](double a) { return a * 0.5 * erfc(a * 0.70710678118654752440); };
            for (int i = 0; i < GELU_TAB_N; ++i) {
                const unsigned lo = (unsigned)(GELU_TAB_BASE + i) << 16, hi = lo + 0x10000u;
                float flo, fhi;
                memcpy(&flo, &lo, 4);
                memcpy(&fhi, &hi, 4);
                h[i] = (float)T(0.5 * ((double)flo + (double)fhi));
            }
            hipError_t e = hipMemcpyToSymbol(HIP_SYMBOL(g_gelu_lut), h, sizeof(h));
            if (e != hipSuccess) DS_FAIL(DS_ELAUNCH, "conv3x3_halo3: GELU table upload: %s", hipGetErrorString(e));
            once.done(dev);
        }
    }
    int lds = twl == 3 ? HG<3>::LDS : (twl == 4 ? HG<4>::LDS : HG<5>::LDS);
#define DS_H3_LAUNCH(TWL_, HP_, PAIR_)                                                                        \
    do {                                                                                               \
        DS_SET_MAX_LDS((conv3x3_halo3_kernel<TWL_, HP_, PAIR_>), 100 * 1024, "conv3x3_halo3");                \
        hipLaunchKernelGGL((conv3x3_halo3_kernel<TWL_, HP_, PAIR_>), grid, dim3(NT), lds, st, *p);            \
    } while (0)
    if (pair) {
        lds += 64;
        DS_H3_LAUNCH(3, true, true);
    }
    else if (p->flags) {
        if (twl == 5) DS_H3_LAUNCH(5, true, false);
        else if (twl == 4) DS_H3_LAUNCH(4, true, false);
        else DS_H3_LAUNCH(3, true, false);
    } else {
        if (twl == 5) DS_H3_LAUNCH(5, false, false);
        else if (twl == 4) DS_H3_LAUNCH(4, false, false);
        else DS_H3_LAUNCH(3, false, false);
    }
#undef DS_H3_LAUNCH
    DS_CHECK_LAUNCH("conv3x3_halo3");
    return DS_OK;
}

#if DS_BOUNDS
extern "C" int ds_bounds_fetch_conv_halo3(ds_bounds_rec* out, int reset) { return ds_bounds_fetch_tu(out, reset); }
#endif
```

### diffusynth_amd/csrc/conv_igemm.hip

```cpp
#include <type_traits>

#include "common.hpp"
#include "conv_epilogue.hpp"

namespace {

inline bool is_halo_tile(int tile) { return tile == DS_CONV_TILE_HALO3_256x96; }

template <typename T> struct Lds;
template <> struct Lds<float> {
    static constexpr int CPR = 8;
    static constexpr int RPB = 2;
    static constexpr int RB = 128;
};
template <> struct Lds<bf16> {
    static constexpr int CPR = 4;
    static constexpr int RPB = 4;
    static constexpr int RB = 64;
};

template <typename T> __device__ __forceinline__ int swz(int row, int chunk) {
    return row * Lds<T>::RB + ((chunk ^ ((row / Lds<T>::RPB) & (Lds<T>::CPR - 1))) << 4);
}

template <typename T> __device__ __forceinline__ void store_out(T* p, float v);
template <> __device__ __forceinline__ void store_out<float>(float* p, float v) { *p = v; }
template <> __device__ __forceinline__ void store_out<bf16>(bf16* p, float v) { *p = (bf16)v; }

template <typename T, int BM, int BN, int WM, int WN>
__global__ __launch_bounds__(256, (sizeof(T) == 4 && BM == 256) ? 1 : 2) void conv_igemm_kernel(const ds_conv_params p) {
    using L = Lds<T>;
    constexpr int EPC = ElemTr<T>::EPC;
    constexpr int CPR = L::CPR;
    constexpr int RSTEP = 256 / CPR;
    constexpr int A_IT = (BM + RSTEP - 1) / RSTEP;
    constexpr int B_IT = (BN + RSTEP - 1) / RSTEP;
    constexpr int TM = BM / WM, TN = BN / WN;
    constexpr int FM = TM / 32, FN = TN / 32;
    static_assert(WM * WN == 4, "4 waves");
    static_assert(TM % 32 == 0 && TN % 32 == 0, "tile shape");
    constexpr int A_BYTES = BM * L::RB, B_BYTES = BN * L::RB;

    extern __shared__ __attribute__((aligned(16))) char smem[];
    char* const ldsA = smem;
    char* const ldsB = smem + 2 * A_BYTES;
    float* const red = reinterpret_cast<float*>(smem);

    const int tid = threadIdx.x, lane = tid & 63, wave = tid >> 6;
    const int wm = wave / WN, wn = wave % WN;
    const int nphase = p.transposed ? 4 : 1;
    const int ksplit = p.ksplit > 1 ? p.ksplit : 1;
    const int zb = blockIdx.z / ksplit, kz = blockIdx.z - zb * ksplit;
    const int b = zb / nphase, phase = zb % nphase;
    const int pa = phase >> 1, pb = phase & 1;
    const int HoWo = p.Ho * p.Wo;
    const int m0 = blockIdx.x * BM, n0 = blockIdx.y * BN;
    const int Cin = p.C0 + p.C1;
    const int pad_h = p.transposed ? 1 - pa : p.pad_h;
    const int pad_w = p.transposed ? 1 - pb : p.pad_w;
    const int ntap = p.KH * p.KW;
    const int nq = (ntap * Cin + 31) / 32;

    float gn_a = 1.f, gn_am = 0.f;

    const T* src0 = reinterpret_cast<const T*>(p.src0) + (size_t)b * p.H * p.W * p.C0;
    const T* src1 = p.C1 ? reinterpret_cast<const T*>(p.src1) + (size_t)b * p.H1 * p.W1 * p.C1 : nullptr;
    const T* wq = reinterpret_cast<const T*>(p.wpk) + ((size_t)phase * nq * p.cout_pad + n0) * 32 +
                  (tid * EPC / 32 < BN ? tid * EPC : (tid * EPC) % 32);

    const int ch = tid % CPR, r0 = tid / CPR;
    int hb[A_IT], wb[A_IT];
#pragma unroll
    for (int i = 0; i < A_IT; ++i) {
        const int m = m0 + r0 + i * RSTEP;
        if (m < HoWo && r0 + i * RSTEP < BM) {
            const int ho = m / p.Wo, wo = m - ho * p.Wo;
            hb[i] = ho * p.stride - pad_h;
            wb[i] = wo * p.stride - pad_w;
        } else {
            hb[i] = -(1 << 28);
            wb[i] = -(1 << 28);
        }
    }
    const int nqs = (nq + ksplit - 1) / ksplit, q_lo = kz * nqs, q_hi = min(nq, q_lo + nqs);
    int kc = (q_lo * 32 + ch * EPC) % Cin, tap = (q_lo * 32 + ch * EPC) / Cin;
    int tap_h = tap / p.KW;

    constexpr int PF = sizeof(T) == 2 ? 3 : 2;
    u32x4 ra[PF][A_IT], rb[PF][B_IT];
    int qload = q_lo;
    int boff[B_IT];
#pragma unroll
    for (int i = 0; i < B_IT; ++i) boff[i] = ((i + 1) * RSTEP <= BN || r0 + i * RSTEP < BN) ? i * 256 * EPC : 0;
    auto load_tiles = [&](auto slotc) {
        constexpr int sl = decltype(slotc)::value;
        const int kh = tap_h, kw = tap - tap_h * p.KW;
        const bool tap_ok = tap < ntap && qload < q_hi;
        const bool first = kc < p.C0;
        const T* base = first ? src0 : src1;
        const int Cs = first ? p.C0 : p.C1, cc = first ? kc : kc - p.C0;
        const int Hs = first ? p.H : p.H1, Ws = first ? p.W : p.W1;
        const int dh = first ? kh : kh - p.off_h1, dw = first ? kw : kw - p.off_w1;
#pragma unroll
        for (int i = 0; i < A_IT; ++i) {
            const int hi = hb[i] + dh, wi = wb[i] + dw;
            const bool ok = tap_ok && (unsigned)hi < (unsigned)Hs && (unsigned)wi < (unsigned)Ws;
            const u32x4 v = DS_LD(u32x4, ok ? base + ((size_t)(hi * Ws + wi) * Cs + cc) : src0, (ok && !first) ? DS_BX_SRC1 : DS_BX_SRC0);
            ra[sl][i] = ok ? v : u32x4{0u, 0u, 0u, 0u};
        }
        const T* wsrc = wq + (size_t)(qload < q_hi ? qload : (q_lo < nq ? q_lo : nq - 1)) * p.cout_pad * 32;
#pragma unroll
        for (int i = 0; i < B_IT; ++i) rb[sl][i] = DS_LD(u32x4, wsrc + boff[i], DS_BX_W);
        ++qload;
        kc += 32;
        while (kc >= Cin) {
            kc -= Cin;
            ++tap;
            if (tap - tap_h * p.KW >= p.KW) ++tap_h;
        }
    };
    auto store_tiles = [&](auto slotc, int buf) {
        constexpr int sl = decltype(slotc)::value;
        char* a = ldsA + buf * A_BYTES;
        char* bb = ldsB + buf * B_BYTES;
#pragma unroll
        for (int i = 0; i < A_IT; ++i)
            if ((i + 1) * RSTEP <= BM || r0 + i * RSTEP < BM) *reinterpret_cast<u32x4*>(a + swz<T>(r0 + i * RSTEP, ch)) = ra[sl][i];
#pragma unroll
        for (int i = 0; i < B_IT; ++i)
            if ((i + 1) * RSTEP <= BN || r0 + i * RSTEP < BN) *reinterpret_cast<u32x4*>(bb + swz<T>(r0 + i * RSTEP, ch)) = rb[sl][i];
    };

    f32x16 acc[FM][FN];
#pragma unroll
    for (int i = 0; i < FM; ++i)
#pragma unroll
        for (int j = 0; j < FN; ++j)
#pragma unroll
            for (int r = 0; r < 16; ++r) acc[i][j][r] = 0.f;

    const int frow = lane & 31, fh = lane >> 5;
    auto compute = [&](int buf) {
        const char* a = ldsA + buf * A_BYTES;
        const char* bb = ldsB + buf * B_BYTES;
        if constexpr (sizeof(T) == 2) {
#pragma unroll
            for (int s = 0; s < 2; ++s) {
                bf16x8 af[FM], bf[FN];
#pragma unroll
                for (int i = 0; i < FM; ++i)
                    af[i] = *reinterpret_cast<const bf16x8*>(a + swz<T>(wm * TM + i * 32 + frow, 2 * s + fh));
#pragma unroll
                for (int j = 0; j < FN; ++j)
                    bf[j] = *reinterpret_cast<const bf16x8*>(bb + swz<T>(wn * TN + j * 32 + frow, 2 * s + fh));
#pragma unroll
                for (int i = 0; i < FM; ++i)
#pragma unroll
                    for (int j = 0; j < FN; ++j)
                        acc[i][j] = __builtin_amdgcn_mfma_f32_32x32x16_bf16(af[i], bf[j], acc[i][j], 0, 0, 0);
            }
        } else {
#pragma unroll
            for (int u = 0; u < 4; ++u) {
                f32x4 af[FM], bf[FN];
#pragma unroll
                for (int i = 0; i < FM; ++i)
                    af[i] = *reinterpret_cast<const f32x4*>(a + swz<T>(wm * TM + i * 32 + frow, 2 * u + fh));
#pragma unroll
                for (int j = 0; j < FN; ++j)
                    bf[j] = *reinterpret_cast<const f32x4*>(bb + swz<T>(wn * TN + j * 32 + frow, 2 * u + fh));
#pragma unroll
                for (int e = 0; e < 4; ++e)
#pragma unroll
                    for (int i = 0; i < FM; ++i)
#pragma unroll
                        for (int j = 0; j < FN; ++j)
                            acc[i][j] = __builtin_amdgcn_mfma_f32_32x32x2f32(af[i][e], bf[j][e], acc[i][j], 0, 0, 0);
            }
        }
    };

    using R0 = std::integral_constant<int, 0>;
    using R1 = std::integral_constant<int, 1>;
    using R2 = std::integral_constant<int, 2>;
    load_tiles(R0{});
    load_tiles(R1{});
    if constexpr (PF == 3) load_tiles(R2{});
    if (p.gn_part) gn_from_partials(p.gn_part, p.gn_parts, p.gn_count, p.gn_eps, b, gn_a, gn_am);
    store_tiles(R0{}, 0);
    __syncthreads();
    const int nqp = (q_hi - q_lo + PF - 1) / PF * PF;
    auto step = [&](auto sc, int q) {
        constexpr int sl = decltype(sc)::value;
        load_tiles(sc);
        compute(q & 1);
        store_tiles(std::integral_constant<int, (sl + 1) % PF>{}, (q + 1) & 1);
        __syncthreads();
    };
    for (int q0 = 0; q0 < nqp; q0 += PF) {
        step(R0{}, q0);
        step(R1{}, q0 + 1);
        if constexpr (PF == 3) step(R2{}, q0 + 2);
    }

    const int outW = p.transposed ? 2 * p.Wo : p.Wo;
    const int outHW = p.transposed ? 4 * HoWo : HoWo;
    const bool need_hw = p.ncls == 9 || p.transposed;
    auto coord = [&](int ml) {
        ConvCoord c;
        const int m = m0 + ml;
        c.ok = m < HoWo;
        c.ho = c.wo = 0;
        c.pix = m;
        if (need_hw) {
            c.ho = m / p.Wo;
            c.wo = m - c.ho * p.Wo;
            if (p.transposed) c.pix = (2 * c.ho + pa) * outW + 2 * c.wo + pb;
        }
        return c;
    };
    float s1 = 0.f, s2 = 0.f;
    float* stage = reinterpret_cast<float*>(smem) + wave * (32 * (TN + 4));
    if (ksplit > 1) {
        const ds_conv_params q = conv_kslice_view(p);
        conv_epilogue_body<float, FM, FN, DS_ACT_NONE, false>(q, acc, kz * p.B + b, n0 + wn * TN, wm * TM, outHW, stage, coord, s1, s2);
        return;
    }
    conv_epilogue<T, FM, FN>(p, acc, b, n0 + wn * TN, wm * TM, outHW, stage, coord, s1, s2, gn_a, gn_am);
    __syncthreads();
    if (p.stats_part) {
        const int parts = gridDim.x * gridDim.y * nphase;
        const int slot = (phase * gridDim.y + blockIdx.y) * gridDim.x + blockIdx.x;
        block_stats_write(s1, s2, red, p.stats_part + ((size_t)b * parts + slot) * 2);
    }
}

}
#if DS_BOUNDS
void ds_conv_bounds_table(const ds_conv_params& p, int kernel, int stats_parts, ds_bx* out) {
    DsBxHost h(kernel);
    const long long es = p.dtype == DS_BF16 ? 2 : 4;
    const long long oH = p.transposed ? 2 * p.Ho : p.Ho, oW = p.transposed ? 2 * p.Wo : p.Wo;
    const int Cin = p.C0 + p.C1;
    h.set(DS_BX_SRC0, p.src0, (long long)p.B * p.H * p.W * p.C0 * es);
    h.set(DS_BX_SRC1, p.C1 ? p.src1 : nullptr, (long long)p.B * p.H1 * p.W1 * p.C1 * es);
    h.set(DS_BX_W, p.wpk, (long long)ds_pack_conv_elems(Cin, p.KH, p.KW, p.cout_pad, p.transposed) * es);
    if (p.ksplit > 1) h.set(DS_BX_OUT, p.slab, (long long)p.ksplit * p.B * oH * oW * ((p.Cout + 7) / 8 * 8) * 4);
    else h.set(DS_BX_OUT, p.out, (long long)p.B * oH * oW * p.out_C * es);
    h.set(DS_BX_RES, p.res, (long long)p.B * oH * oW * p.out_C * es);
    h.set(DS_BX_BIAS, p.bias, (long long)p.Cout * 4);
    h.set(DS_BX_T1, p.fold_t1, (long long)p.ncls * p.Cout * 4);
    h.set(DS_BX_T2, p.fold_t2, (long long)p.ncls * p.Cout * 4);
    h.set(DS_BX_GNAB, p.gn_ab, (long long)p.B * 2 * 4);
    h.set(DS_BX_GNPART, p.gn_part, (long long)p.B * p.gn_parts * 2 * 4);
    h.set(DS_BX_STATS, p.stats_part, (long long)p.B * stats_parts * 2 * 4);
    *out = h.t;
}
static void ds_conv_publish_bounds(const ds_conv_params& p, int kernel, int stats_parts, hipStream_t st) {
    DsBxHost h(kernel);
    ds_conv_bounds_table(p, kernel, stats_parts, &h.t);
    h.publish(st);
}
extern "C" int ds_bounds_fetch_conv_igemm(ds_bounds_rec* out, int reset) { return ds_bounds_fetch_tu(out, reset); }
__global__ void ds_bounds_selftest_kernel(const float* buf, float* sink) {
    const f32x4 v = DS_LD(f32x4, buf + 14, DS_BX_AUX3);
    if (v[0] == 12345.f) *sink = v[1];
}
extern "C" int ds_bounds_selftest(const float* buf64, float* sink, void* stream) {
    hipStream_t st = reinterpret_cast<hipStream_t>(stream);
    DsBxHost h(DS_K_CONV_IGEMM);
    h.set(DS_BX_AUX3, buf64, 64);
    h.publish(st);
    hipLaunchKernelGGL(ds_bounds_selftest_kernel, dim3(1), dim3(1), 0, st, buf64, sink);
    DS_CHECK_LAUNCH("bounds_selftest");
    return DS_OK;
}
#endif
namespace {

template <typename T, int BM, int BN, int WM, int WN>
int launch_cfg(const ds_conv_params& p, hipStream_t st) {
    constexpr size_t lds_main = 2 * (size_t)(BM + BN) * Lds<T>::RB;
    constexpr size_t lds_epi = 4 * 32 * (size_t)(BN / WN + 4) * sizeof(float);
    constexpr size_t lds = lds_main > lds_epi ? lds_main : lds_epi;
    auto kern = conv_igemm_kernel<T, BM, BN, WM, WN>;
    DS_SET_MAX_LDS(kern, lds, "conv_igemm");
    const int HoWo = p.Ho * p.Wo;
    dim3 grid((HoWo + BM - 1) / BM, p.cout_pad / BN, p.B * (p.transposed ? 4 : 1) * (p.ksplit > 1 ? p.ksplit : 1));
#if DS_BOUNDS
    ds_conv_publish_bounds(p, DS_K_CONV_IGEMM, grid.x * grid.y * (p.transposed ? 4 : 1), st);
#endif
    hipLaunchKernelGGL(kern, grid, dim3(256), lds, st, p);
    DS_CHECK_LAUNCH("conv_igemm");
    return DS_OK;
}

template <typename T> int launch_tile(const ds_conv_params& p, hipStream_t st) {
    switch (p.tile) {
        case DS_CONV_TILE_128x192: return launch_cfg<T, 128, 192, 2, 2>(p, st);
        case DS_CONV_TILE_256x96: return launch_cfg<T, 256, 96, 4, 1>(p, st);
        case DS_CONV_TILE_128x32: return launch_cfg<T, 128, 32, 4, 1>(p, st);
        case DS_CONV_TILE_64x96: return launch_cfg<T, 64, 192, 2, 2>(p, st);
    }
    DS_FAIL(DS_EINVAL, "conv_igemm: unknown tile %d", p.tile);
}

void tile_dims(int tile, int* bm, int* bn) {
    switch (tile) {
        case DS_CONV_TILE_QUAD_HALO3:
        case DS_CONV_TILE_HALO3_256x96: *bm = 256; *bn = 96; break;
        case DS_CONV_TILE_128x192: *bm = 128; *bn = 192; break;
        case DS_CONV_TILE_256x96: *bm = 256; *bn = 96; break;
        case DS_CONV_TILE_128x32: *bm = 128; *bn = 32; break;
        case DS_CONV_TILE_HALO3_N16: *bm = 256; *bn = 16; break;
        case DS_CONV_TILE_64x96: *bm = 64; *bn = 192; break;
        default: *bm = 0; *bn = 0;
    }
}

int validate(const ds_conv_params* p) {
    DS_REQUIRE(p != nullptr, "conv_igemm: null params");
    int bm, bn;
    tile_dims(p->tile, &bm, &bn);
    DS_REQUIRE(bm > 0, "conv_igemm: unknown tile %d", p->tile);
    const int epc = p->dtype == DS_BF16 ? 8 : 4;
    DS_REQUIRE(p->dtype == DS_F32 || p->dtype == DS_BF16, "conv_igemm: dtype %d", p->dtype);
    DS_REQUIRE(p->B > 0 && p->Ho > 0 && p->Wo > 0 && p->H > 0 && p->W > 0, "conv_igemm: empty problem");
    DS_REQUIRE(p->batch_hint >= 0, "conv_igemm: batch_hint must be 0 (use B) or the batch the launch decisions look at, got %d", p->batch_hint);
    DS_REQUIRE(p->C0 > 0 && p->C0 % epc == 0 && p->C1 >= 0 && p->C1 % epc == 0,
               "conv_igemm: channel counts (%d,%d) must be multiples of %d", p->C0, p->C1, epc);
    DS_REQUIRE(p->C1 == 0 || (p->src1 && p->H1 > 0 && p->W1 > 0), "conv_igemm: second source incomplete");
    DS_REQUIRE(p->cout_pad % bn == 0 && p->Cout <= p->cout_pad && p->Cout > 0,
               "conv_igemm: cout_pad %d must be a multiple of the tile's BN %d", p->cout_pad, bn);
    DS_REQUIRE(p->KH > 0 && p->KW > 0 && p->stride > 0, "conv_igemm: bad geometry");
    DS_REQUIRE(!p->transposed || (p->KH == 2 && p->KW == 2 && p->stride == 1), "conv_igemm: transposed needs KH=KW=2");
    DS_REQUIRE(p->ncls == 1 || p->ncls == 9, "conv_igemm: ncls must be 1 or 9");
    DS_REQUIRE(!(p->gn_ab || p->gn_part) || (p->fold_t1 && p->fold_t2), "conv_igemm: GN fold needs t1/t2 tables");
    DS_REQUIRE(!p->gn_part || (p->gn_parts > 0 && p->gn_count > 0), "conv_igemm: gn_part needs gn_parts and gn_count");
    DS_REQUIRE(p->ncls == 1 || (p->KH == 3 && p->KW == 3 && p->pad_h == 1 && p->pad_w == 1 && p->stride == 1 &&
                                p->Ho == p->H && p->Wo == p->W && p->H >= 2 && p->W >= 2),
               "conv_igemm: 9 border classes are defined for 3x3 pad 1 stride 1 only");
    DS_REQUIRE(!p->out_nchw_f32, "conv_igemm: NCHW output was removed from the kernel; convert with ds_nhwc_to_nchw");
    DS_REQUIRE(p->act == DS_ACT_NONE || p->act == DS_ACT_GELU, "conv_igemm: epilogue activation must be NONE or GELU (got %d)", p->act);
    DS_REQUIRE(p->out_C % epc == 0 && p->out_c0 % epc == 0 && p->out_C >= p->out_c0 + (p->Cout + epc - 1) / epc * epc,
               "conv_igemm: out_C=%d / out_c0=%d must be multiples of %d and hold Cout=%d rounded up", p->out_C, p->out_c0, epc, p->Cout);
    if (!ds_aligned16(p->src0) || !ds_aligned16(p->wpk) || (p->C1 && !ds_aligned16(p->src1)))
        DS_FAIL(DS_EALIGN, "conv_igemm: src/weight pointers must be 16-byte aligned");
    DS_REQUIRE(p->out != nullptr, "conv_igemm: null output");
    DS_REQUIRE(p->ksplit <= 1 || (p->dtype == DS_BF16 && p->slab && (p->ksplit == 2 || p->ksplit == 3 || p->ksplit == 4 || p->ksplit == 6 || p->ksplit == 8)),
               "conv_igemm: split-K needs bf16, a slab and ksplit in {2, 3, 4, 6, 8} (got %d)", p->ksplit);
    DS_REQUIRE(p->ksplit <= 1 || is_halo_tile(p->tile) ||
                   ((p->transposed ? 4 : p->KH * p->KW) * (p->C0 + p->C1) + 31) / 32 >= 2 * p->ksplit,
               "conv_igemm: ksplit=%d leaves fewer than two K steps per slice", p->ksplit);
    if (p->ksplit > 1 && !is_halo_tile(p->tile)) {
        const int nq = ((p->transposed ? 4 : p->KH * p->KW) * (p->C0 + p->C1) + 31) / 32, nqs = (nq + p->ksplit - 1) / p->ksplit;
        DS_REQUIRE((p->ksplit - 1) * nqs < nq, "conv_igemm: ksplit=%d over %d K steps leaves the last slice empty", p->ksplit, nq);
    }
    DS_REQUIRE((p->wk_order == 2) == (p->tile == DS_CONV_TILE_QUAD_HALO3), "conv_igemm: wk_order=%d does not match tile %d (quad tiles are for DS_CONV_TILE_QUAD_HALO3 only)",
               p->wk_order, p->tile);
    DS_REQUIRE((p->wk_order == 1) == (p->tile == DS_CONV_TILE_HALO3_256x96 || p->tile == DS_CONV_TILE_HALO3_N16),
               "conv_igemm: wk_order=%d does not match tile %d (chunk-major weights are for DS_CONV_TILE_HALO3_256x96 / _N16 only)", p->wk_order, p->tile);
    DS_REQUIRE(p->flags == 0 || p->tile == DS_CONV_TILE_HALO3_256x96 || p->tile == DS_CONV_TILE_QUAD_HALO3,
               "conv_igemm: flags=%d (split precision) is implemented by DS_CONV_TILE_HALO3_256x96 / QUAD_HALO3 only, not tile %d", p->flags, p->tile);
    DS_REQUIRE(p->res_steps == 0 || p->tile == DS_CONV_TILE_HALO3_256x96,
               "conv_igemm: a fused res_conv (res_steps=%d) is implemented by DS_CONV_TILE_HALO3_256x96 only, not tile %d", p->res_steps, p->tile);
    DS_REQUIRE(p->res_steps != 0 || (!p->res_src0 && !p->res_src1 && !p->res_bias),
               "conv_igemm: res_src0 / res_src1 / res_bias given with res_steps = 0");
    return DS_OK;
}

}

int ds_conv_splitk_parts(const ds_conv_params* p);
int ds_conv3x3_halo3_launch(const ds_conv_params* p, hipStream_t st);
int ds_conv3x3_halo3_parts(const ds_conv_params* p);
int ds_conv_quad_halo3_launch(const ds_conv_params* p, hipStream_t st);
int ds_conv_quad_halo3_parts(const ds_conv_params* p);
int ds_conv3x3_smalln_launch(const ds_conv_params* p, hipStream_t st);

extern "C" int ds_conv_tile_bn(int tile) {
    int bm, bn;
    tile_dims(tile, &bm, &bn);
    return bn;
}

extern "C" int ds_conv_stats_parts(const ds_conv_params* p) {
    int bm, bn;
    tile_dims(p->tile, &bm, &bn);
    if (!bm) return DS_EINVAL;
    if (p->ksplit > 1) return ds_conv_splitk_parts(p);
    if (p->tile == DS_CONV_TILE_QUAD_HALO3) return ds_conv_quad_halo3_parts(p);
    if (p->tile == DS_CONV_TILE_HALO3_256x96) return ds_conv3x3_halo3_parts(p);
    return ((p->Ho * p->Wo + bm - 1) / bm) * (p->cout_pad / bn) * (p->transposed ? 4 : 1);
}

extern "C" int ds_conv_igemm(const ds_conv_params* p, void* stream) {
    int rc = validate(p);
    if (rc) return rc;
    hipStream_t st = reinterpret_cast<hipStream_t>(stream);
    if (p->tile == DS_CONV_TILE_HALO3_256x96) return ds_conv3x3_halo3_launch(p, st);
    if (p->tile == DS_CONV_TILE_QUAD_HALO3) return ds_conv_quad_halo3_launch(p, st);
    if (p->tile == DS_CONV_TILE_HALO3_N16) return ds_conv3x3_smalln_launch(p, st);
    return p->dtype == DS_BF16 ? launch_tile<bf16>(*p, st) : launch_tile<float>(*p, st);
}

namespace {

template <typename T>
__global__ void pack_conv_kernel(const ds_pack_conv_params p, int nq, size_t total) {
    for (size_t idx = blockIdx.x * (size_t)blockDim.x + threadIdx.x; idx < total; idx += (size_t)gridDim.x * blockDim.x) {
        const int j = idx & 31;
        size_t r = idx >> 5;
        const int n = r % p.cout_pad;
        r /= p.cout_pad;
        const int q = r % nq;
        const int phase = r / nq;
        const int k = q * 32 + j;
        int tap = k / p.cin_pad, c = k % p.cin_pad;
        if (p.k_order == 1) {
            const int ntap = p.KH * p.KW;
            tap = q % ntap;
            c = (q / ntap) * 32 + j;
        }
        float v = 0.f;
        if (n < p.Cout && c < p.Cin && tap < p.KH * p.KW) {
            const int kh = tap / p.KW, kw = tap % p.KW;
            if (p.transposed) {
                const int a = phase >> 1, bph = phase & 1;
                const int ky = a ? 2 - 2 * kh : 3 - 2 * kh, kx = bph ? 2 - 2 * kw : 3 - 2 * kw;
                v = p.w[(((size_t)c * p.Cout + n) * 4 + ky) * 4 + kx];
            } else {
                v = p.w[(((size_t)n * p.Cin + c) * p.KH + kh) * p.KW + kw];
            }
            if (p.gamma) v *= p.gamma[c];
        }
        reinterpret_cast<T*>(p.dst)[idx] = from_f32<T>(v);
    }
}

__global__ void fold_tables_kernel(const float* w, const float* bias, const float* gamma, const float* beta, int Cout,
                                   int Cin, int KH, int KW, float* t1, float* t2) {
    const int ncls = (KH == 3 && KW == 3) ? 9 : 1;
    const int wid = (blockIdx.x * blockDim.x + threadIdx.x) >> 6, lane = threadIdx.x & 63;
    if (wid >= ncls * Cout) return;
    const int cls = wid / Cout, o = wid % Cout;
    const int ch = cls / 3, cw = cls % 3;
    float a1 = 0.f, a2 = 0.f;
    for (int idx = lane; idx < Cin * KH * KW; idx += 64) {
        const int c = idx / (KH * KW), t = idx % (KH * KW), kh = t / KW, kw = t % KW;
        bool ok = true;
        if (ncls == 9) ok = !(ch == 0 && kh == 0) && !(ch == 2 && kh == 2) && !(cw == 0 && kw == 0) && !(cw == 2 && kw == 2);
        if (ok) {
            const float wv = w[((size_t)o * Cin + c) * KH * KW + t];
            a1 += wv * beta[c];
            a2 += wv * gamma[c];
        }
    }
    a1 = wave_sum(a1);
    a2 = wave_sum(a2);
    if (lane == 0) {
        t1[cls * Cout + o] = a1 + (bias ? bias[o] : 0.f);
        t2[cls * Cout + o] = a2;
    }
}

}

extern "C" size_t ds_pack_conv_elems(int cin_pad, int KH, int KW, int cout_pad, int transposed) {
    const size_t nq = ((size_t)KH * KW * cin_pad + 31) / 32;
    return (transposed ? 4 : 1) * nq * cout_pad * 32;
}

extern "C" int ds_pack_conv_weight(const ds_pack_conv_params* p, void* stream) {
    DS_REQUIRE(p && p->w && p->dst, "pack_conv: null pointer");
    DS_REQUIRE(p->cin_pad >= p->Cin && p->cout_pad >= p->Cout, "pack_conv: pads too small");
    DS_REQUIRE(!p->transposed || (p->KH == 2 && p->KW == 2), "pack_conv: transposed packs 2x2 sub-kernels");
    DS_REQUIRE(p->k_order == 0 || (p->k_order == 1 && p->cin_pad % 32 == 0 && !p->transposed), "pack_conv: k_order 1 needs cin_pad %% 32 == 0");
    const int nq = (p->KH * p->KW * p->cin_pad + 31) / 32;
    const size_t total = ds_pack_conv_elems(p->cin_pad, p->KH, p->KW, p->cout_pad, p->transposed);
    const int blocks = (int)((total + 255) / 256 < 4096 ? (total + 255) / 256 : 4096);
    hipStream_t st = reinterpret_cast<hipStream_t>(stream);
    if (p->dtype == DS_BF16) hipLaunchKernelGGL(pack_conv_kernel<bf16>, dim3(blocks), dim3(256), 0, st, *p, nq, total);
    else hipLaunchKernelGGL(pack_conv_kernel<float>, dim3(blocks), dim3(256), 0, st, *p, nq, total);
    DS_CHECK_LAUNCH("pack_conv");
    return DS_OK;
}

extern "C" int ds_conv_fold_tables(const float* w, const float* bias, const float* gamma, const float* beta, int Cout,
                                   int Cin, int KH, int KW, float* t1, float* t2, void* stream) {
    DS_REQUIRE(w && gamma && beta && t1 && t2, "fold_tables: null pointer");
    DS_REQUIRE((KH == 3 && KW == 3) || (KH == 1 && KW == 1), "fold_tables: 3x3 or 1x1 only");
    const int ncls = KH == 3 ? 9 : 1;
    const int waves = ncls * Cout;
    hipLaunchKernelGGL(fold_tables_kernel, dim3((waves + 3) / 4), dim3(256), 0, reinterpret_cast<hipStream_t>(stream), w, bias,
                       gamma, beta, Cout, Cin, KH, KW, t1, t2);
    DS_CHECK_LAUNCH("fold_tables");
    return DS_OK;
}
```

### diffusynth_amd/engine.py

```python
import collections
import ctypes as C
import math
import os
from typing import NamedTuple

import torch

from . import _lib as L
from . import conv_policy as policy
from .conv_policy import up as _up

_ESIZE = {L.DS_F32: 4, L.DS_BF16: 2}
_TDT = {L.DS_F32: torch.float32, L.DS_BF16: torch.bfloat16}
_X, _TIME, _COND, _OUT = range(4)


class _Arena:

    def __init__(self):
        self.free = [[0, 1 << 62]]
        self.peak = 0

    def alloc(self, nbytes):
        nbytes = _up(max(int(nbytes), 1), 256)
        for seg in self.free:
            if seg[1] - seg[0] >= nbytes:
                off = seg[0]
                seg[0] += nbytes
                if seg[0] == seg[1]:
                    self.free.remove(seg)
                self.peak = max(self.peak, off + nbytes)
                return off, nbytes
        raise MemoryError("arena exhausted")

    def release(self, off, nbytes):
        self.free.append([off, off + nbytes])
        self.free.sort()
        merged = []
        for s in self.free:
            if merged and merged[-1][1] >= s[0]:
                merged[-1][1] = max(merged[-1][1], s[1])
            else:
                merged.append(s)
        self.free = merged


class _Partials(NamedTuple):
    buf: tuple
    parts: int


class _Finished(NamedTuple):
    buf: tuple


class _ChanSums(NamedTuple):
    buf: tuple
    slots: int


class _Op(NamedTuple):
    name: str
    fn: object
    args: tuple
    late: tuple = None


class _Act:
    __slots__ = ("off", "nbytes", "C", "H", "W", "stats", "split", "planes")

    def __init__(self, off, nbytes, Cc, H, W):
        self.off, self.nbytes, self.C, self.H, self.W = off, nbytes, Cc, H, W
        self.stats = None
        self.split = False
        self.planes = None


class _ConvW:
    __slots__ = ("w", "bias", "t1", "t2", "ncls", "Cout", "cout_pad", "cin_pad", "cin_real", "KH", "KW", "bn", "transposed", "k_order",
                 "w_f32n4", "w_x3", "x3_cout_pad", "w_n16", "w_split", "w_quad", "quad_cout_pad", "w_init7", "w_init7x3",
                 "w_fused", "res_steps", "res_bias")

    def __init__(self, s):
        self.Cout, self.cin_pad, self.cin_real, self.transposed = s.Cout, s.cin_pad, s.Cin, s.transposed
        self.KH, self.KW = (2, 2) if s.transposed else s.k
        self.bn, self.cout_pad, self.k_order = s.bn, s.cout_pad, s.k_order
        self.w = self.bias = self.t1 = self.t2 = None
        self.w_f32n4 = self.w_x3 = self.w_n16 = self.w_split = self.w_quad = self.w_init7 = self.w_init7x3 = None
        self.ncls, self.x3_cout_pad, self.quad_cout_pad = 1, 0, 0
        self.w_fused, self.res_steps, self.res_bias = None, 0, None


def split3_weight(w, gamma=None):
    w = w.detach().float()
    if gamma is not None:
        w = w * gamma.detach().float().view(1, -1, 1, 1)
    hi = w.bfloat16().float()
    lo = w - hi
    Cout, Cin, kh, kw = w.shape
    assert Cin % 32 == 0, Cin
    hic, loc = hi.view(Cout, Cin // 32, 32, kh, kw), lo.view(Cout, Cin // 32, 32, kh, kw)
    return torch.stack([hic, loc, hic], 2).reshape(Cout, 3 * Cin, kh, kw).contiguous()


def pack_x3_1x1(w, gamma=None):
    w = w.detach().float().reshape(w.shape[0], -1)
    if gamma is not None:
        w = w * gamma.detach().float().view(1, -1)
    Cout, Cin = w.shape
    cout_pad, ncc = _up(Cout, 96), _up(Cin, 32) // 32
    wp = torch.zeros(cout_pad, ncc * 32, dtype=torch.float32, device=w.device)
    wp[:Cout, :Cin] = w
    hi = wp.bfloat16()
    lo = (wp - hi.float()).bfloat16()
    planes = torch.stack([hi, lo], 0).view(2, cout_pad, ncc, 32).permute(2, 0, 1, 3)
    return planes.contiguous().view(-1), cout_pad


def to_split_planes(x_nhwc):
    hi = x_nhwc.float().bfloat16()
    lo = (x_nhwc.float() - hi.float()).bfloat16()
    return torch.cat([hi, lo], -1).contiguous()


def pack_quad_weights(w, transposed, dtype=torch.bfloat16):
    w = w.detach().float()
    if transposed:
        Cin, Cout = w.shape[:2]
        cc, cp = Cin // 32, 4 * Cout
        out = torch.zeros(cc, 4, cp, 32, device=w.device)
        for ph in range(4):
            py, px = ph >> 1, ph & 1
            for t in range(4):
                a, b = t >> 1, t & 1
                m = w[:, :, 3 - py - 2 * a, 3 - px - 2 * b]
                out[:, t, ph * Cout:(ph + 1) * Cout, :] = m.t().reshape(Cout, cc, 32).permute(1, 0, 2)
    else:
        Cout, Cin = w.shape[:2]
        cc, cp = Cin // 32, _up(Cout, 96)
        out = torch.zeros(4, cc, 4, cp, 32, device=w.device)
        for par in range(4):
            p_, q_ = par >> 1, par & 1
            for t in range(4):
                a, b = t >> 1, t & 1
                m = w[:, :, 1 - p_ + 2 * a, 1 - q_ + 2 * b]
                out[par, :, t, :Cout, :] = m.reshape(Cout, cc, 32).permute(1, 0, 2)
    return out.reshape(-1).to(dtype).contiguous(), cp


def max_plans():
    return max(1, int(os.environ.get("DS_MAX_PLANS", "8")))


class _EngineBase:

    def _init_common(self, module, compute_dtype):
        L.load()
        self.m = module
        self.dt = L.DS_BF16 if compute_dtype == "bf16" else L.DS_F32
        self.split3 = compute_dtype == "bf16x3"
        self.es = _ESIZE[self.dt]
        self.vec = 16 // self.es
        self.dev = next(module.parameters()).device
        if self.dev.type != "cuda":
            raise RuntimeError("parameters must live on a HIP device ('cuda'); diffusynth_amd has no CPU path")
        self.plans = collections.OrderedDict()
        self._max_plans = max_plans()
        self._arena, self._arena_base, self._arena_bytes = None, 0, 0
        self.hip_graph = False
        self.plan_builds = 0
        self._keep = []
        self.side_stream = None
        self._tb_total = 0
        self._lab_total = 0
        self._pack_tmp = []

    def _pack_done(self):
        torch.cuda.current_stream(self.dev).synchronize()
        self._pack_tmp = []

    def _cached_plan(self, key, make):
        plan = self.plans.get(key)
        if plan is not None:
            self.plans.move_to_end(key)
            return plan
        self.plan_builds += 1
        dry = make()
        dry.build(0)
        peak = dry.arena.peak
        if peak > self._arena_bytes:
            self.plans.clear()
            self._arena_bytes = int(max(peak, 1.25 * self._arena_bytes))
            self._arena = torch.empty(self._arena_bytes + 256, dtype=torch.uint8, device=self.dev)
            self._arena_base = _up(self._arena.data_ptr(), 256)
        plan = make()
        plan.build(self._arena_base)
        plan.ws = self._arena
        self.plans[key] = plan
        while len(self.plans) > self._max_plans:
            self.plans.popitem(last=False)
        return plan

    def _f32(self, t):
        return t.detach().to(device=self.dev, dtype=torch.float32).contiguous()

    def _pack_weight(self, w, gamma, dtype, Cout, Cin, cin_pad, KH, KW, cout_pad, transposed=False, k_order=1):
        dst = torch.empty(L.load().ds_pack_conv_elems(cin_pad, KH, KW, cout_pad, int(transposed)), dtype=_TDT[dtype], device=self.dev)
        pp = L.PackConvParams(w=w.data_ptr(), gamma=L.ptr(gamma), dst=dst.data_ptr(), dtype=dtype, Cout=Cout, Cin=Cin, cin_pad=cin_pad,
                              KH=KH, KW=KW, cout_pad=cout_pad, transposed=int(transposed), k_order=k_order)
        L.call("ds_pack_conv_weight", C.byref(pp), L.current_stream())
        return dst

    def _pack_init7(self, w, fn, planes):
        dst = torch.empty(planes * L.load().ds_conv7x7_c4_weight_elems(), dtype=torch.bfloat16, device=self.dev)
        L.call(fn, w.data_ptr(), 96, int(w.shape[1]), dst.data_ptr(), L.current_stream())
        return dst

    def _pack_conv(self, weight, bias, cin_pad=None, gamma=None, beta=None, transposed=False, small_out=False, halo=False):
        w = self._f32(weight)
        Cin, Cout = (w.shape[0], w.shape[1]) if transposed else (w.shape[1], w.shape[0])
        s = policy.ConvLayer(Cout, Cin, Cin if cin_pad is None else cin_pad, tuple(w.shape[2:]), transposed, gamma is not None, halo,
                             small_out, self.dt == L.DS_BF16, self.split3)
        cw = _ConvW(s)
        g = self._f32(gamma) if gamma is not None else None
        cw.w = self._pack_weight(w, g, self.dt, Cout, Cin, s.cin_pad, cw.KH, cw.KW, cw.cout_pad, transposed, cw.k_order)
        cw.bias = self._f32(bias) if bias is not None else None
        if s.f32n4_fits:
            cw.w_f32n4 = torch.empty(L.load().ds_conv3x3_f32_n4_weight_floats(Cin), dtype=torch.float32, device=self.dev)
            L.call("ds_pack_conv3x3_f32_n4", w.data_ptr(), L.ptr(cw.bias), Cout, Cin, cw.w_f32n4.data_ptr(), L.current_stream())
        if s.x3_1x1_fits:
            cw.w_x3, cw.x3_cout_pad = pack_x3_1x1(weight.to(self.dev), gamma.to(self.dev) if gamma is not None else None)
        if s.n16_fits:
            cw.w_n16 = self._pack_weight(w, None, L.DS_BF16, Cout, Cin, Cin, 3, 3, 16)
        if s.split3_fits:
            ws = split3_weight(weight, gamma)
            cw.w_split = self._pack_weight(ws, None, L.DS_BF16, Cout, 3 * Cin, 3 * Cin, 3, 3, cw.cout_pad)
            self._pack_tmp.append(ws)
        if s.quad_fits:
            wq = weight
            if self.split3:
                w32 = weight.detach().float()
                hi = w32.bfloat16().float()
                wq = torch.cat([hi, hi, w32 - hi], 0 if transposed else 1)
            cw.w_quad, cw.quad_cout_pad = pack_quad_weights(wq, transposed)
        if s.init7_fits:
            cw.w_init7 = self._pack_init7(w, "ds_pack_conv7x7_c4", 1)
        if s.init7x3_fits:
            cw.w_init7x3 = self._pack_init7(w, "ds_pack_conv7x7_c4_x3", 2)
        if gamma is not None:
            cw.ncls = 9 if cw.KH == 3 else 1
            cw.t1 = torch.empty(cw.ncls * Cout, dtype=torch.float32, device=self.dev)
            cw.t2 = torch.empty(cw.ncls * Cout, dtype=torch.float32, device=self.dev)
            b = self._f32(beta)
            L.call("ds_conv_fold_tables", w.data_ptr(), L.ptr(cw.bias), g.data_ptr(), b.data_ptr(), Cout, Cin, cw.KH, cw.KW,
                   cw.t1.data_ptr(), cw.t2.data_ptr(), L.current_stream())
            self._keep += [g, b]
        self._pack_tmp += [w, g]
        return cw


class _PlanBase:
    prof_all = False

    def __init__(self, eng, B, H, W):
        self.e, self.B, self.H, self.W = eng, B, H, W
        self.alloc_B = 0
        self.Btile = getattr(eng, "launch_batch", None) or B
        self.tb_all = self.lab_all = None
        self.arena = _Arena()
        self.ops = []
        self.ws = None
        self.lib = L.load()
        self.conv_meta = {}
        self.prof = None
        self.prof_every = 1
        self.calls = 0

    def act(self, Cc, H, W):
        off, n = self.arena.alloc(max(self.B, self.alloc_B) * H * W * Cc * self.e.es)
        return _Act(self.base + off, n, Cc, H, W)

    def raw(self, nbytes):
        off, n = self.arena.alloc(nbytes)
        return (self.base + off, n)

    def free(self, a):
        if isinstance(a, _Act):
            if a.nbytes:
                self.arena.release(a.off - self.base, a.nbytes)
            if a.stats is not None:
                self.free_raw(a.stats.buf)
                a.stats = None
            if a.planes is not None:
                self.free(a.planes)
                a.planes = None
        else:
            self.free_raw(a)

    def free_raw(self, r):
        self.arena.release(r[0] - self.base, r[1])

    def op(self, name, *args, late=None):
        self.ops.append(_Op(name, getattr(self.lib, name), args, late))

    def _prof_now(self):
        prof = self.prof
        if prof is not None:
            if self.calls % self.prof_every:
                prof = None
            self.calls += 1
        return prof

    def launch(self, lo, hi, st, tensors, prof):
        meta = None if self.prof_all else self.conv_meta
        for k, (name, fn, args, late) in enumerate(self.ops[lo:hi], lo):
            if late is not None:
                args = list(args)
                for pos, t in late:
                    args[pos] = tensors[t].data_ptr()
            if prof is not None and (meta is None or k in meta):
                ev0, ev1 = torch.cuda.Event(enable_timing=True), torch.cuda.Event(enable_timing=True)
                ev0.record()
                rc = fn(*args, st)
                ev1.record()
                prof.append((k, ev0, ev1))
            else:
                rc = fn(*args, st)
            if rc != 0:
                L.check(rc, name)

    def _halo3_ksplit(self, cw, x, split):
        return policy.halo3_ksplit(self.Btile, x.H, x.W, cw.cout_pad, x.C // 32, split)

    def _split_takes(self, cw, src1=None, stride=1, pad=1, out_nchw_ptr=False):
        return cw.w_split is not None and src1 is None and stride == 1 and pad == 1 and not out_nchw_ptr

    def _quad_takes(self, cw, x, stride=1, pad=0, src1=None, res=None, gn_ab=None, out_nchw_ptr=False):
        return (cw.w_quad is not None and src1 is None and res is None and gn_ab is None and not out_nchw_ptr and (not x.split or self.e.split3)
                and (cw.transposed or (stride == 2 and pad == 1 and x.H % 2 == 0 and x.W % 2 == 0)))

    def _conv_route(self, cw, src0, src1, stride, pad, gn_ab, act, res, want_stats, out, out_nchw_ptr, gn_src, res_fuse):
        plain = src1 is None and stride == 1 and pad == 1 and not out_nchw_ptr and res is None and gn_ab is None and not want_stats
        if cw.w_f32n4 is not None and plain and not src0.split and out.C == 4 and act == L.ACT_NONE and res_fuse is None:
            return "f32n4"
        if (cw.w_x3 is not None and stride == 1 and pad == 0 and not out_nchw_ptr and not src0.split and gn_src is None and act == L.ACT_NONE
                and src0.C % 32 == 0 and (src1.C if src1 is not None else 0) % 32 == 0):
            return "x3"
        if cw.w_n16 is not None and plain and not src0.split:
            return "n16"
        if self._split_takes(cw, src1, stride, pad, out_nchw_ptr) and src0.split:
            return "split"
        if self._quad_takes(cw, src0, stride, pad, src1, res, gn_ab, out_nchw_ptr):
            return "quad"
        if cw.k_order == 1:
            assert src1 is None and stride == 1 and pad == 1 and src0.C % 32 == 0, "chunk-major weights reached a layer the halo kernel cannot run"
            return "halo3"
        return "igemm"

    def conv(self, cw, src0, src1=None, off1=(0, 0), stride=1, pad=0, gn_ab=None, act=L.ACT_NONE, res=None,
             want_stats=False, out=None, out_nchw_ptr=False, gn_src=None, res_fuse=None, out_split=False):
        if gn_src is not None:
            gn_ab = True
        e, B = self.e, self.B
        H, W = src0.H, src0.W
        if cw.transposed:
            Ho, Wo, oh, ow = H, W, 2 * H, 2 * W
        else:
            Ho = (H + 2 * pad - cw.KH) // stride + 1
            Wo = (W + 2 * pad - cw.KW) // stride + 1
            oh, ow = Ho, Wo
        C1 = src1.C if src1 is not None else 0
        assert src0.C + C1 == cw.cin_pad, (src0.C, C1, cw.cin_pad)
        if out is None:
            out = self.act(_up(cw.Cout, e.vec), oh, ow)
        route = self._conv_route(cw, src0, src1, stride, pad, gn_ab, act, res, want_stats, out, out_nchw_ptr, gn_src, res_fuse)
        if route == "f32n4":
            self.op("ds_conv3x3_f32_n4", src0.off, B, H, W, src0.C, cw.w_f32n4.data_ptr(), out.off)
            return out
        tile, dtype, src, C0, flags, wpk, cout_pad, korder, out_C = None, e.dt, src0, src0.C, 0, cw.w, cw.cout_pad, cw.k_order, out.C
        xsplit = None
        if route == "x3":
            tile, dtype, flags, wpk, cout_pad, korder = 0, L.DS_BF16, 8 | 4, cw.w_x3, cw.x3_cout_pad, 0
        elif route == "n16":
            tile, wpk, cout_pad, korder = L.TILE_HALO3_N16, cw.w_n16, 16, 1
        elif route == "split":
            tile, dtype, C0, flags, wpk, korder = L.TILE_HALO3_256x96, L.DS_BF16, 2 * src0.C, 1 | (2 if out_split else 4), cw.w_split, 1
            out_C = 2 * out.C if out_split else out.C
            out.split = bool(out_split)
        elif route == "quad":
            tile, wpk, cout_pad, korder = L.TILE_QUAD_HALO3, cw.w_quad, cw.quad_cout_pad, 2
            if e.split3:
                src = src0 if src0.split else src0.planes
                if src is None:
                    src = xsplit = self.act(src0.C, H, W)
                    self.op("ds_split_planes", src0.off, xsplit.off, B * H * W, src0.C)
                elif not src0.split:
                    xsplit, src0.planes = src, None
                dtype, C0, flags = L.DS_BF16, 2 * src0.C, 1 | 4
        else:
            tile = policy.igemm_tile(cw.bn, Ho * Wo, cw.k_order)
        extra = {}
        if gn_src is not None:
            extra.update(gn_part=gn_src[0], gn_parts=gn_src[1], gn_count=float(gn_src[2]), gn_eps=gn_src[3])
        if res_fuse is not None:
            x0, x1, xoff = res_fuse
            assert tile == L.TILE_HALO3_256x96 and cw.res_steps == (x0.C + (x1.C if x1 is not None else 0)) // 32 and res is None
            wpk = cw.w_fused
            extra.update(res_src0=x0.off, res_C0=x0.C, res_steps=cw.res_steps, res_bias=L.ptr(cw.res_bias))
            if x1 is not None:
                extra.update(res_src1=x1.off, res_C1=x1.C, res_H1=x1.H, res_W1=x1.W, res_off_h1=xoff[0], res_off_w1=xoff[1])
        ks = 1
        if route in ("halo3", "split") and res_fuse is None:
            ks = self._halo3_ksplit(cw, src0, route == "split")
        elif route == "quad":
            ks = policy.quad_ksplit(self.Btile, Ho, Wo, cw.quad_cout_pad, (1 if cw.transposed else 4) * (3 if e.split3 else 1) * src0.C // 32, e.split3)
        elif route == "igemm" and e.dt == L.DS_BF16:
            nq = -(-((4 if cw.transposed else cw.KH * cw.KW) * (src0.C + C1)) // 32)
            ks = policy.igemm_ksplit(self.Btile, tile, Ho, Wo, cw.cout_pad, nq, 4 if cw.transposed else 1)
        elif route == "x3":
            ks = policy.x3_1x1_ksplit(self.Btile, Ho, Wo, cw.x3_cout_pad, (src0.C + C1) // 32)
        slab = None
        if ks > 1:
            slab = self.raw(ks * B * oh * ow * _up(cw.Cout, 8) * 4)
            extra.update(ksplit=ks, slab=slab[0])
        if src1 is not None:
            extra.update(src1=src1.off, H1=src1.H, W1=src1.W)
        p = L.ConvParams(src0=src.off, C0=C0, C1=C1, H=H, W=W, off_h1=off1[0], off_w1=off1[1], wpk=wpk.data_ptr(), Cout=cw.Cout,
                         cout_pad=cout_pad, KH=cw.KH, KW=cw.KW, stride=stride, pad_h=pad, pad_w=pad, Ho=Ho, Wo=Wo,
                         transposed=int(cw.transposed), out=out.off, out_C=out_C, out_c0=0, out_nchw_f32=0,
                         bias=L.ptr(cw.bias), gn_ab=(gn_ab if gn_src is None else None), fold_t1=L.ptr(cw.t1) if gn_ab else None,
                         fold_t2=L.ptr(cw.t2) if gn_ab else None, ncls=cw.ncls if gn_ab else 1, act=act,
                         res=(res.off if res is not None else None), stats_part=None, B=B, dtype=dtype, tile=tile, wk_order=korder,
                         flags=flags, batch_hint=self.Btile, **extra)
        if want_stats:
            parts = (self.lib.ds_conv1x1_x3_stats_parts if route == "x3" else self.lib.ds_conv_stats_parts)(C.byref(p))
            st = self.raw(B * parts * 2 * 4)
            p.stats_part = st[0]
            out.stats = _Partials(st, parts)
        if route == "x3":
            self.op("ds_conv1x1_x3", C.byref(p))
        else:
            self.conv_meta[len(self.ops)] = policy.conv_meta(tile, B, Ho, Wo, cw.Cout, cw.KH, cw.KW, cw.transposed, src0.C + C1, cw.cin_real,
                                                             32 * cw.res_steps if res_fuse is not None else 0)
            self.op("ds_conv_igemm", C.byref(p))
        if xsplit is not None:
            self.free(xsplit)
        if slab is not None:
            self.op("ds_conv_splitk_reduce", C.byref(p))
            self.free_raw(slab)
        return out

    @staticmethod
    def _partials(a, who):
        assert isinstance(a.stats, _Partials), f"{who}() reads a producer's partial sums, not {type(a.stats).__name__}"
        return a.stats

    def finalize(self, a, count, eps=1e-5):
        st, parts = self._partials(a, "finalize")
        ab = self.raw(self.B * 2 * 4)
        self.op("ds_gn_finalize", st[0], self.B, parts, float(count), eps, ab[0])
        self.free_raw(st)
        a.stats = None
        return ab

    def stats_src(self, a, count, eps=1e-5):
        st, parts = self._partials(a, "stats_src")
        a.stats = None
        return (st[0], parts, count, eps), st

    def srcs(self, x):
        if isinstance(x, _Act):
            return x, None, (0, 0)
        enc, dec = x
        return enc, dec, ((enc.H - dec.H) // 2, (enc.W - dec.W) // 2)

    def _stats_op(self, a, G, eps, ab):
        e, B = self.e, self.B
        if isinstance(a.stats, _ChanSums):
            ws, slots = a.stats
            self.op("ds_gn_stats_finish", ws[0], B, slots, a.C, G, a.H * a.W, eps, ab[0])
            self.free_raw(ws)
            a.stats = None
            return
        if a.C % e.vec == 0 and a.C // e.vec <= 256:
            ws = self.raw(self.lib.ds_gn_stats_ws_floats(B, a.H * a.W, a.C) * 4)
            self.op("ds_gn_stats_stream", a.off, e.dt, B, a.H * a.W, a.C, G, eps, ws[0], ab[0])
            self.free_raw(ws)
        else:
            self.op("ds_gn_stats", a.off, e.dt, B, a.H * a.W, a.C, G, eps, ab[0])

    def _gn_explicit(self, y, nrm, G, act, cbias=None, res=None, eps=1e-5):
        e, B = self.e, self.B
        ab = self.raw(B * G * 2 * 4)
        self._stats_op(y, G, eps, ab)
        out = self.act(y.C, y.H, y.W)
        p = L.GnApplyParams(x=y.off, res=(res.off if res is not None else None), out=out.off, gn_ab=ab[0],
                            gamma=nrm[0].data_ptr(), beta=nrm[1].data_ptr(),
                            cbias=(self.tb_all[0] + 4 * cbias) if (cbias is not None and self.tb_all) else None,
                            cb_stride=e._tb_total, B=B, HW=y.H * y.W, C=y.C, G=G, act=act, dtype=e.dt)
        self.op("ds_gn_apply", C.byref(p))
        self.free_raw(ab)
        return out


class UnetEngine(_EngineBase):
    use_cfg_pair = True

    def __init__(self, module, compute_dtype="fp32"):
        self._init_common(module, compute_dtype)
        self.cfg = module.config
        self.launch_batch = None
        with torch.cuda.device(self.dev):
            self._pack()
            self._pack_done()

    def _pack_block(self, blk, dim):
        d = {}
        if self.cfg["use_convnext"]:
            C_ = blk.ds_conv.weight.shape[0]
            dw = torch.empty(49 * C_, dtype=torch.float32, device=self.dev)
            w = self._f32(blk.ds_conv.weight)
            L.call("ds_pack_dw_weight", w.data_ptr(), C_, dw.data_ptr(), L.current_stream())
            self._pack_tmp.append(w)
            d["dw"], d["dw_bias"] = dw, self._f32(blk.ds_conv.bias)
            d["dw_exp"] = None
            if self.dt == L.DS_BF16 and C_ % 32 == 0:
                we = torch.empty(C_ * 6 * 64 * 8, dtype=torch.bfloat16, device=self.dev)
                L.call("ds_pack_dw_weight_mfma", w.data_ptr(), C_, we.data_ptr(), L.current_stream())
                d["dw_exp"] = we
            n0, c1, n3, c4 = blk.net[0], blk.net[1], blk.net[3], blk.net[4]
            d["conv1"] = self._pack_conv(c1.weight, c1.bias, gamma=n0.weight, beta=n0.bias, halo=True)
            d["conv2"] = self._pack_conv(c4.weight, c4.bias, gamma=n3.weight, beta=n3.bias, halo=True)
            d["dim"], d["dim_out"] = C_, c4.weight.shape[0]
        else:
            b1, b2 = blk.block1, blk.block2
            d["conv1"] = self._pack_conv(b1.proj.weight, b1.proj.bias)
            d["conv2"] = self._pack_conv(b2.proj.weight, b2.proj.bias, halo=True)
            d["n1"] = (self._f32(b1.norm.weight), self._f32(b1.norm.bias))
            d["n2"] = (self._f32(b2.norm.weight), self._f32(b2.norm.bias))
            d["dim"], d["dim_out"] = b1.proj.weight.shape[1], b1.proj.weight.shape[0]
        d["res"] = None
        if isinstance(blk.res_conv, torch.nn.Conv2d):
            d["res"] = self._pack_conv(blk.res_conv.weight, blk.res_conv.bias)
            c2, cx = d["conv2"], blk.res_conv.weight.shape[1]
            if c2.k_order == 1 and cx % 96 == 0:
                w = self._f32(blk.res_conv.weight)
                c2.w_fused = torch.cat([self._pack_weight(w, None, self.dt, c2.Cout, cx, cx, 1, 1, c2.cout_pad), c2.w])
                c2.res_steps, c2.res_bias = cx // 32, d["res"].bias
                self._pack_tmp.append(w)
        d["tb_off"] = None
        if getattr(blk, "mlp", None) is not None:
            d["tb_off"] = self._tb_total
            self._tb_w.append(self._f32(blk.mlp[1].weight))
            self._tb_b.append(self._f32(blk.mlp[1].bias))
            self._tb_total += blk.mlp[1].weight.shape[0]
        return d

    def _pack_attn(self, res):
        pre, a = res.fn, res.fn.fn
        d = {"C": a.to_qkv.weight.shape[1]}
        d["qkv"] = self._pack_conv(a.to_qkv.weight, None, gamma=pre.norm.weight, beta=pre.norm.bias)
        d["out"] = self._pack_conv(a.to_out[0].weight, a.to_out[0].bias)
        d["on"] = (self._f32(a.to_out[1].weight), self._f32(a.to_out[1].bias))
        d["l_off"] = self._lab_total
        d["fused"] = None
        Cc = d["C"]
        if self.dt == L.DS_BF16 and self.cfg["attn_type"] == "linear_add" and Cc in (96, 192, 384):
            wq = self._f32(a.to_qkv.weight).reshape(384, Cc).contiguous()
            wo = self._f32(a.to_out[0].weight).reshape(Cc, 128).contiguous()
            g = self._f32(pre.norm.weight)
            wq16 = torch.empty(384 * Cc, dtype=torch.bfloat16, device=self.dev)
            wo16 = torch.empty(Cc * 128, dtype=torch.bfloat16, device=self.dev)
            L.call("ds_pack_attn_fused", wq.data_ptr(), g.data_ptr(), wo.data_ptr(), wq16.data_ptr(), wo16.data_ptr(), Cc, L.current_stream())
            self._pack_tmp += [wq, wo, g]
            d["fused"] = (wq16, wo16)
        d["x3"] = None
        if self.split3 and self.cfg["attn_type"] == "linear_add" and Cc in (96, 192, 384):
            wq = self._f32(a.to_qkv.weight).reshape(384, Cc).contiguous()
            g = self._f32(pre.norm.weight)
            whl = torch.empty(2 * 384 * Cc, dtype=torch.bfloat16, device=self.dev)
            L.call("ds_pack_attn_x3", wq.data_ptr(), g.data_ptr(), whl.data_ptr(), Cc, L.current_stream())
            self._pack_tmp += [wq, g]
            d["x3"] = (whl, self._f32(a.to_out[0].weight).reshape(Cc, 128).contiguous())
        if self.cfg["attn_type"] == "linear_add":
            self._lab_w.append(self._f32(a.label_query.weight))
            self._lab_b.append(self._f32(a.label_query.bias))
            self._lab_total += a.label_query.weight.shape[0]
        else:
            self._lab_w += [self._f32(a.label_key.weight), self._f32(a.label_value.weight)]
            self._lab_b += [self._f32(a.label_key.bias), self._f32(a.label_value.bias)]
            self._lab_total += 2 * a.label_key.weight.shape[0]
        return d

    def _pack(self):
        m, cfg = self.m, self.cfg
        self._tb_w, self._tb_b, self._tb_total = [], [], 0
        self._lab_w, self._lab_b, self._lab_total = [], [], 0
        self.cin0 = _up(cfg["in_dim"], self.vec)
        P = {}
        P["init"] = self._pack_conv(m.init_conv.weight, m.init_conv.bias, cin_pad=self.cin0)
        P["downs"] = []
        for blk1, at1, blk2, at2, down in m.downs:
            P["downs"].append((self._pack_block(blk1, None), self._pack_attn(at1), self._pack_block(blk2, None),
                               self._pack_attn(at2), self._pack_conv(down.weight, down.bias)))
        P["mid_left"] = [self._pack_block(b, None) for b in m.mid_left]
        P["mid_mid"] = (self._pack_block(m.mid_mid[0], None), self._pack_attn(m.mid_mid[1]), self._pack_block(m.mid_mid[2], None))
        P["mid_right"] = [self._pack_block(b, None) for b in m.mid_right]
        P["ups"] = []
        for b1, a1, up, b2, a2, b3, a3 in m.ups:
            P["ups"].append((self._pack_block(b1, None), self._pack_attn(a1),
                             self._pack_conv(up.weight, up.bias, transposed=True),
                             self._pack_block(b2, None), self._pack_attn(a2), self._pack_block(b3, None), self._pack_attn(a3)))
        P["final_block"] = self._pack_block(m.final_conv[0], None)
        fc = m.final_conv[1]
        P["final"] = self._pack_conv(fc.weight, fc.bias, small_out=True)
        self.P = P
        if m.time_mlp is not None:
            half = cfg["down_dims"][0] // 2
            self.freqs = torch.exp(torch.arange(half, dtype=torch.float32) * -(math.log(10000) / (half - 1))).to(self.dev)
            self.tm1 = (self._f32(m.time_mlp[1].weight), self._f32(m.time_mlp[1].bias))
            self.tm3 = (self._f32(m.time_mlp[3].weight), self._f32(m.time_mlp[3].bias))
            self.tb_W = torch.cat(self._tb_w, 0).contiguous() if self._tb_w else None
            self.tb_b = torch.cat(self._tb_b, 0).contiguous() if self._tb_b else None
        emb = m.label_embedding.embedding
        self.emb_is_linear = isinstance(emb, torch.nn.Linear)
        self.emb_w = self._f32(emb.weight)
        self.emb_b = self._f32(emb.bias) if self.emb_is_linear else None
        self.lab_W = torch.cat(self._lab_w, 0).contiguous()
        self.lab_b = torch.cat(self._lab_b, 0).contiguous()
        self.label_dim = cfg["label_emb_dim"]

    def _plan(self, B, H, W, has_cond, paired=False):
        key = (B, H, W, has_cond) if not paired else (B, H, W, has_cond, "paired")
        if self.launch_batch is not None:
            key += ("pin", self.launch_batch)
        return self._cached_plan(key, lambda: _PlanBuilder(self, B, H, W, has_cond, paired))

    def forward(self, x, time, condition, paired=False):
        cfg = self.cfg
        assert x.dim() == 4 and x.shape[1] == cfg["in_dim"], "x must be (B, in_dim, H, W)"
        B, _, H, W = x.shape
        x = x.to(torch.float32).contiguous()
        time = time.to(device=x.device, dtype=torch.int64).contiguous()
        cond = None
        if condition is not None:
            if self.emb_is_linear:
                cond = condition.to(device=x.device, dtype=torch.float32).contiguous()
            else:
                cond = self.emb_w[condition.to(x.device)].contiguous()
        out = torch.empty((B, cfg["out_dim"], H, W), dtype=torch.float32, device=x.device)
        with torch.cuda.device(x.device):
            paired = bool(paired) and B % 2 == 0 and cond is not None and self.use_cfg_pair and cfg["use_convnext"]
            plan = self._plan(B, H, W, cond is not None, paired)
            if self.hip_graph and plan.prof is None and not L.lib_path().endswith("_bounds.so"):
                plan.run_graphed(x, time, cond, out)
            else:
                plan.run(x, time, cond, out)
        return out


class _PlanBuilder(_PlanBase):

    def __init__(self, eng, B, H, W, has_cond, paired=False):
        super().__init__(eng, B, H, W)
        self.has_cond, self.paired = has_cond, paired
        self._graph = None

    def launch_signature(self):
        cat, counts = [], []
        lib = self.lib
        for op in self.ops:
            name = op.name
            ref = op.args[0]
            if name in ("ds_conv_igemm", "ds_conv1x1_x3"):
                p = ref._obj
                ks = max(1, p.ksplit)
                pair = bool(name == "ds_conv_igemm" and p.tile == L.TILE_HALO3_256x96 and p.flags != 0 and p.W <= 8 and 2 * p.H <= 32
                            and ks == 1 and not p.res_steps and (p.batch_hint or p.B) >= 2)
                cat.append((name, p.tile, ks, p.flags, p.res_steps, pair))
            elif name == "ds_dwconv7":
                fam, ranges, spc = C.c_int32(), C.c_int32(), C.c_int32()
                L.call("ds_dwconv_launch_choice", ref, C.byref(fam), C.byref(ranges), C.byref(spc))
                cat.append((name, L.DW_FAMILY[fam.value], ranges.value, spc.value > 1))
            elif name == "ds_attn_fused_context":
                counts.append((ref._obj.nseg, lib.ds_attn_fused_stats_parts(ref)))
                cat.append((name, lib.ds_attn_fused_generations(ref)))
            elif name == "ds_attn_x3_context":
                counts.append((ref._obj.nseg, lib.ds_attn_x3_stats_parts(ref)))
                cat.append((name, 0))
            elif name == "ds_linattn_context":
                counts.append((ref._obj.nseg, 0))
                cat.append((name, 0))
            else:
                cat.append((name,))
        return tuple(cat), tuple(counts)

    def dup(self, a):
        nb = (self.B // 2) * a.H * a.W * a.C * self.e.es
        assert a.nbytes >= 2 * nb, "dup() of a tensor not carved at the full batch"
        out = _Act(a.off, a.nbytes, a.C, a.H, a.W)
        out.split = a.split
        self.op("ds_dup_batch", a.off, a.off, nb)
        a.nbytes = 0
        if a.stats is not None:
            st, parts = self._partials(a, "dup")
            ns = self.raw(self.B * parts * 2 * 4)
            self.op("ds_dup_batch", st[0], ns[0], (self.B // 2) * parts * 2 * 4)
            out.stats = _Partials(ns, parts)
        return out

    def convnext(self, d, x, want_stats):
        e, B = self.e, self.B
        s0, s1, off1 = self.srcs(x)
        H, W = s0.H, s0.W
        dim, dim_out = d["dim"], d["dim_out"]
        h = self.act(dim, H, W)
        p = L.DwconvParams(src0=s0.off, src1=(s1.off if s1 else None), C0=s0.C, C1=(s1.C if s1 else 0), H=H, W=W,
                           H1=(s1.H if s1 else 0), W1=(s1.W if s1 else 0), off_h1=off1[0], off_w1=off1[1],
                           wt=d["dw"].data_ptr(), bias=d["dw_bias"].data_ptr(),
                           tbias=(self.tb_all[0] + 4 * d["tb_off"]) if (d["tb_off"] is not None and self.tb_all) else None,
                           tb_stride=e._tb_total, out=h.off, stats_part=None, B=B, dtype=e.dt,
                           wexp=L.ptr(d["dw_exp"]),
                           batch_hint=self.Btile)
        sp = (self._split_takes(d["conv1"]) and self._split_takes(d["conv2"]) and s0.C % 16 == 0 and (s1 is None or s1.C % 16 == 0))
        if sp:
            p.out_split, h.split = 1, True
        parts = self.lib.ds_dwconv_stats_parts(C.byref(p))
        st = self.raw(B * parts * 2 * 4)
        p.stats_part = st[0]
        h.stats = _Partials(st, parts)
        self.op("ds_dwconv7", C.byref(p))
        src1_, st1 = self.stats_src(h, dim * H * W)
        g = self.conv(d["conv1"], h, pad=1, gn_src=src1_, act=L.ACT_GELU, want_stats=True, out_split=sp)
        self.free(h)
        self.free_raw(st1)
        src2_, st2 = self.stats_src(g, d["conv1"].Cout * H * W)
        c2 = d["conv2"]
        if c2.res_steps and self._halo3_ksplit(c2, g, g.split) == 1:
            out = self.conv(c2, g, pad=1, gn_src=src2_, want_stats=want_stats, res_fuse=(s0, s1, off1))
        else:
            out = self.conv(d["res"], s0, s1, off1) if d["res"] is not None else None
            out = self.conv(c2, g, pad=1, gn_src=src2_, res=s0 if out is None else out, want_stats=want_stats, out=out)
        self.free(g)
        self.free_raw(st2)
        return out

    def resnet(self, d, x, want_stats):
        e, B = self.e, self.B
        s0, s1, off1 = self.srcs(x)
        H, W = s0.H, s0.W
        G = e.cfg["resnet_block_groups"]
        co = d["dim_out"]
        y = self.conv(d["conv1"], s0, s1, off1, pad=1)
        h = self._gn_explicit(y, d["n1"], G, L.ACT_SILU, cbias=d["tb_off"])
        self.free(y)
        y = self.conv(d["conv2"], h, pad=1)
        self.free(h)
        if d["res"] is not None:
            r = self.conv(d["res"], s0, s1, off1)
        else:
            r = s0
        out = self._gn_explicit(y, d["n2"], G, L.ACT_SILU, res=r)
        self.free(y)
        if d["res"] is not None:
            self.free(r)
        if want_stats:
            self._direct_stats(out)
        return out

    def _direct_stats(self, a):
        ab = self.raw(self.B * 2 * 4)
        self._stats_op(a, 1, 1e-5, ab)
        a.stats = _Finished(ab)

    def block(self, d, x, want_stats=False):
        return self.convnext(d, x, want_stats) if self.e.cfg["use_convnext"] else self.resnet(d, x, want_stats)

    def attention(self, d, x, planes=None):
        e, B = self.e, self.B
        N, Cc = x.H * x.W, x.C
        xsrc, xst, abx = None, None, (None, 0)
        if isinstance(x.stats, _Finished):
            abx, x.stats = x.stats.buf, None
        elif d["fused"] is not None or d["x3"] is not None:
            xsrc, xst = self.stats_src(x, Cc * N)
        else:
            abx = self.finalize(x, Cc * N)
        lazy = xsrc is not None
        heads = 4
        nseg = max(1, min(N // 1024, 16))
        if d["x3"] is not None:
            return self._attention_x3(d, x, abx, xsrc, xst, planes)
        if d["fused"] is not None:
            nseg = self.lib.ds_attn_fused_segments(self.Btile, N, Cc)
            part = self.raw(self.lib.ds_linattn_part_floats(B, heads, nseg) * 4)
            ctx = self.raw(B * heads * 1024 * 4)
            y = self.act(Cc, x.H, x.W)
            lab = self.lab_all[0] if self.lab_all else None
            fp = L.AttnFusedParams(x=x.off, B=B, N=N, C=Cc, nseg=nseg, wqkv=d["fused"][0].data_ptr(), t1=d["qkv"].t1.data_ptr(),
                                   t2=d["qkv"].t2.data_ptr(), gn_ab=abx[0], label_q=(lab + 4 * d["l_off"]) if lab else None,
                                   lq_stride=e._lab_total, scale=32 ** -0.5, part=part[0], ctx=ctx[0],
                                   wout_perm=d["fused"][1].data_ptr(), bias_out=d["out"].bias.data_ptr(), y=y.off, stats_part=None,
                                   batch_hint=self.Btile)
            if lazy:
                fp.gn_ab, fp.gn_part, fp.gn_parts, fp.gn_count, fp.gn_eps = None, xsrc[0], xsrc[1], float(xsrc[2]), xsrc[3]
            mfold = self.raw(B * Cc * 128 * 2) if Cc in (96, 192) else None
            fp.mfold = mfold[0] if mfold is not None else None
            parts = self.lib.ds_attn_fused_stats_parts(C.byref(fp))
            st = self.raw(B * parts * 2 * 4)
            fp.stats_part = st[0]
            y.stats = _Partials(st, parts)
            self.op("ds_attn_fused_context", C.byref(fp))
            self.op("ds_attn_fused_output", C.byref(fp))
            if lazy:
                self.free_raw(xst)
            else:
                self.free_raw(abx)
            self.free_raw(part)
            self.free_raw(ctx)
            if mfold is not None:
                self.free_raw(mfold)
            out = self.act(Cc, x.H, x.W)
            g = L.GnApplyParams(x=y.off, res=x.off, out=out.off, gn_ab=None, gamma=d["on"][0].data_ptr(),
                                beta=d["on"][1].data_ptr(), cbias=None, cb_stride=0, B=B, HW=N, C=Cc, G=1, act=L.ACT_NONE, dtype=e.dt)
            ysrc, yst = self.stats_src(y, Cc * N)
            g.gn_part, g.gn_parts, g.gn_count, g.gn_eps = ysrc[0], ysrc[1], float(ysrc[2]), ysrc[3]
            self.op("ds_gn_apply", C.byref(g))
            self.free_raw(yst)
            self.free(y)
            return out
        qkv = self.conv(d["qkv"], x, gn_ab=abx[0])
        self.free_raw(abx)
        part = self.raw(self.lib.ds_linattn_part_floats(B, heads, nseg) * 4)
        ctx = self.raw(B * heads * 1024 * 4)
        ao = self.act(heads * 32, x.H, x.W)
        add = e.cfg["attn_type"] == "linear_add"
        lab = self.lab_all[0] if self.lab_all else None
        ls = e._lab_total
        p = L.AttnParams(qkv=qkv.off, B=B, N=N, heads=heads, dtype=e.dt, nseg=nseg, part=part[0], ctx=ctx[0],
                         label_q=(lab + 4 * d["l_off"]) if (lab and add) else None,
                         label_k=(lab + 4 * d["l_off"]) if (lab and not add) else None,
                         label_v=(lab + 4 * (d["l_off"] + heads * 32)) if (lab and not add) else None,
                         lq_stride=ls, lk_stride=ls, lv_stride=ls, q_softmax=1, scale=32 ** -0.5, out=ao.off)
        self.op("ds_linattn_context", C.byref(p))
        self.op("ds_linattn_output", C.byref(p))
        self.free(qkv)
        self.free_raw(part)
        self.free_raw(ctx)
        y = self.conv(d["out"], ao, want_stats=True)
        self.free(ao)
        aby = self.finalize(y, Cc * N)
        out = self.act(Cc, x.H, x.W)
        g = L.GnApplyParams(x=y.off, res=x.off, out=out.off, gn_ab=aby[0], gamma=d["on"][0].data_ptr(),
                            beta=d["on"][1].data_ptr(), cbias=None, cb_stride=0, B=B, HW=N, C=Cc, G=1, act=L.ACT_NONE, dtype=e.dt)
        self.op("ds_gn_apply", C.byref(g))
        self.free(y)
        self.free_raw(aby)
        return out

    def _attention_x3(self, d, x, abx, xsrc, xst, planes=None):
        e, B = self.e, self.B
        N, Cc = x.H * x.W, x.C
        lib, lazy = self.lib, xsrc is not None
        nseg = lib.ds_attn_x3_segments(self.Btile, N, Cc)
        part = self.raw(lib.ds_linattn_part_floats(B, 4, nseg) * 4)
        ctx = self.raw(B * 4 * 1024 * 4)
        qpl = self.raw(lib.ds_attn_x3_qplane_bytes(B, N)) if Cc != 96 else None
        mf = self.raw(lib.ds_attn_x3_mfold_bytes(B, Cc))
        out = self.act(Cc, x.H, x.W) if planes != "only" else None
        pl = self.act(Cc, x.H, x.W) if planes else None
        if pl is not None:
            pl.split = True
        lab = self.lab_all[0] if self.lab_all else None
        fp = L.AttnX3Params(x=x.off, B=B, N=N, C=Cc, nseg=nseg, wqkv_hl=d["x3"][0].data_ptr(), t1=d["qkv"].t1.data_ptr(),
                            t2=d["qkv"].t2.data_ptr(), gn_ab=abx[0], label_q=(lab + 4 * d["l_off"]) if lab else None,
                            lq_stride=e._lab_total, scale=32 ** -0.5, part=part[0], ctx=ctx[0], qplanes=(qpl[0] if qpl else None), mfold=mf[0],
                            wout=d["x3"][1].data_ptr(), bias_out=d["out"].bias.data_ptr(), y=None, stats_part=None,
                            out=(out.off if out is not None else None), on_gamma=d["on"][0].data_ptr(), on_beta=d["on"][1].data_ptr(), on_eps=1e-5,
                            out_planes=(pl.off if pl is not None else None), batch_hint=self.Btile)
        if lazy:
            fp.gn_ab, fp.gn_part, fp.gn_parts, fp.gn_count, fp.gn_eps = None, xsrc[0], xsrc[1], float(xsrc[2]), xsrc[3]
        parts = lib.ds_attn_x3_stats_parts(C.byref(fp))
        st = self.raw(B * parts * 2 * 4)
        fp.stats_part = st[0]
        self.op("ds_attn_x3_context", C.byref(fp))
        self.op("ds_attn_x3_output", C.byref(fp))
        if lazy:
            self.free_raw(xst)
        else:
            self.free_raw(abx)
        for r in (part, ctx, qpl, mf):
            if r is not None:
                self.free_raw(r)
        self.free_raw(st)
        if planes == "only":
            return pl
        if pl is not None:
            out.planes = pl
        return out

    def build(self, base):
        self.base = base
        e, cfg, B, H, W = self.e, self.e.cfg, self.B, self.H, self.W
        P = e.P
        self.sin = self.h1 = self.temb = None
        if e.m.time_mlp is not None:
            half = cfg["down_dims"][0] // 2
            td = cfg["time_dim"]
            self.sin = self.raw(B * 2 * half * 4)
            self.h1 = self.raw(B * td * 4)
            self.temb = self.raw(B * td * 4)
            self.op("ds_sinusoid", None, e.freqs.data_ptr(), B, half, self.sin[0], late=((0, _TIME),))
            self.op("ds_linear", self.sin[0], 2 * half, e.tm1[0].data_ptr(), e.tm1[1].data_ptr(), B, 2 * half, td, L.ACT_NONE, self.h1[0], td)
            self.op("ds_activation", self.h1[0], B * td, L.ACT_GELU, self.h1[0])
            self.op("ds_linear", self.h1[0], td, e.tm3[0].data_ptr(), e.tm3[1].data_ptr(), B, td, td, L.ACT_NONE, self.temb[0], td)
            if e.tb_W is not None:
                self.tb_all = self.raw(B * e._tb_total * 4)
                self.op("ds_activation", self.temb[0], B * td, L.ACT_GELU if cfg["use_convnext"] else L.ACT_SILU, self.temb[0])
                self.op("ds_linear", self.temb[0], td, e.tb_W.data_ptr(), e.tb_b.data_ptr(), B, td, e._tb_total, L.ACT_NONE, self.tb_all[0], e._tb_total)
        if self.has_cond:
            ld = e.label_dim
            self.cemb = None
            if e.emb_is_linear:
                self.cemb = self.raw(B * ld * 4)
                self.op("ds_linear", None, ld, e.emb_w.data_ptr(), e.emb_b.data_ptr(), B, ld, ld, L.ACT_NONE, self.cemb[0], ld, late=((0, _COND),))
            self.lab_all = self.raw(B * e._lab_total * 4)
            self.op("ds_linear", self.cemb[0] if self.cemb else None, ld, e.lab_W.data_ptr(), e.lab_b.data_ptr(), B, ld, e._lab_total, L.ACT_NONE,
                    self.lab_all[0], e._lab_total, late=None if self.cemb else ((0, _COND),))

        self.n_cond = len(self.ops)
        Bfull = self.B
        half = self.paired and len(P["downs"]) > 0
        if half:
            self.B = B = Bfull // 2
            self.alloc_B = Bfull
        xin = self.act(e.cin0, H, W)
        self.op("ds_nchw_to_nhwc", None, self.B, cfg["in_dim"], H, W, xin.off, e.cin0, e.dt, late=((0, _X),))
        cw = P["init"]
        if cw.w_init7 is not None:
            x = self.act(96, H, W)
            self.conv_meta[len(self.ops)] = policy.conv_meta(L.TILE_INIT7, B, H, W, 96, 7, 7, False, cw.cin_real, cw.cin_real)
            self.op("ds_conv7x7_c4", xin.off, B, H, W, e.cin0, cw.w_init7.data_ptr(), L.ptr(cw.bias), x.off)
        elif cw.w_init7x3 is not None:
            x = self.act(96, H, W)
            self.op("ds_conv7x7_c4_x3", xin.off, B, H, W, cw.w_init7x3.data_ptr(), L.ptr(cw.bias), x.off)
        else:
            x = self.conv(cw, xin, pad=3)
        self.free(xin)
        self.n_cond_join = len(self.ops)
        skips = [x]
        for b1, a1, b2, a2, down in P["downs"]:
            y = self.block(b1, x, True)
            if half:
                half = False
                self.B = B = Bfull
                self.alloc_B = 0
                xf, yf = self.dup(x), self.dup(y)
                self.free(x)
                self.free(y)
                x, y = xf, yf
                skips[-1] = x
            if x is not skips[-1]:
                self.free(x)
            x = self.attention(a1, y)
            self.free(y)
            skips.append(x)
            y = self.block(b2, x, True)
            x = self.attention(a2, y, planes="both" if (e.split3 and self._quad_takes(down, y, stride=2, pad=1)) else None)
            self.free(y)
            skips.append(x)
            x = self.conv(down, x, stride=2, pad=1)
            skips.append(x)
        for b in P["mid_left"]:
            x = self.block(b, x)
            skips.append(x)
        b1, a, b2 = P["mid_mid"]
        y = self.block(b1, x, True)
        x = self.attention(a, y)
        self.free(y)
        y = self.block(b2, x)
        self.free(x)
        x = y
        for b in P["mid_right"]:
            sk = skips.pop()
            y = self.block(b, (sk, x))
            self.free(sk)
            self.free(x)
            x = y
        for b1, a1, up, b2, a2, b3, a3 in P["ups"]:
            for blk, at, do_up in ((b1, a1, True), (b2, a2, False), (b3, a3, False)):
                sk = skips.pop()
                y = self.block(blk, (sk, x), True)
                self.free(sk)
                self.free(x)
                x = self.attention(at, y, planes="only" if (do_up and e.split3 and self._quad_takes(up, y)) else None)
                self.free(y)
                if do_up:
                    y = self.conv(up, x)
                    self.free(x)
                    x = y
        sk = skips.pop()
        assert not skips
        y = self.block(P["final_block"], (sk, x))
        self.free(sk)
        self.free(x)
        z = self.conv(P["final"], y, pad=1)
        self.free(y)
        self.op("ds_nhwc_to_nchw", z.off, e.dt, B, cfg["out_dim"], z.C, H, W, None, late=((7, _OUT),))
        self.free(z)

    def run_graphed(self, x, time, cond, out):
        g = self._graph
        if g is None:
            self._gx, self._gt, self._go = torch.empty_like(x), torch.empty_like(time), torch.empty_like(out)
            self._gc = torch.empty_like(cond) if cond is not None else None
            self._gx.copy_(x)
            self._gt.copy_(time)
            if cond is not None:
                self._gc.copy_(cond)
            self.run(self._gx, self._gt, self._gc, self._go)
            torch.cuda.synchronize()
            g = torch.cuda.CUDAGraph()
            with torch.cuda.graph(g):
                self.run(self._gx, self._gt, self._gc, self._go)
            self._graph = g
        self._gx.copy_(x, non_blocking=True)
        self._gt.copy_(time, non_blocking=True)
        if cond is not None:
            self._gc.copy_(cond, non_blocking=True)
        g.replay()
        out.copy_(self._go, non_blocking=True)

    def run(self, x, time, cond, out):
        st = L.current_stream()
        tensors, prof = (x, time, cond, out), self._prof_now()
        e, side, cond_st = self.e, None, st
        if self.n_cond > 0 and self.B * self.H * self.W >= 65536:
            if e.side_stream is None:
                e.side_stream = torch.cuda.Stream()
            side = e.side_stream
            side.wait_stream(torch.cuda.current_stream())
            cond_st = side.cuda_stream
        self.launch(0, self.n_cond, cond_st, tensors, prof)
        self.launch(self.n_cond, self.n_cond_join, st, tensors, prof)
        if side is not None:
            torch.cuda.current_stream().wait_stream(side)
        self.launch(self.n_cond_join, len(self.ops), st, tensors, prof)
```

### include/diffusynth_hip.h

```cpp
#ifndef DIFFUSYNTH_HIP_H
#define DIFFUSYNTH_HIP_H

#include <stddef.h>
#include <stdint.h>

#ifdef __cplusplus
extern "C" {
#endif

#define DS_OK 0
#define DS_EINVAL (-1)
#define DS_ELAUNCH (-2)
#define DS_EALIGN (-3)

typedef enum { DS_F32 = 0, DS_BF16 = 1 } ds_dtype;
typedef enum { DS_ACT_NONE = 0, DS_ACT_GELU = 1, DS_ACT_SILU = 2, DS_ACT_RELU = 3 } ds_act;

const char* ds_last_error_string(void);
int ds_abi_version(void);

#define DS_CONV_TILE_128x192 0
#define DS_CONV_TILE_256x96 1
#define DS_CONV_TILE_128x32 2
#define DS_CONV_TILE_64x96 3
#define DS_CONV_TILE_HALO3_256x96 11
#define DS_CONV_TILE_QUAD_HALO3 12

#define DS_CONV_F_SPLIT_IN 1
#define DS_CONV_F_OUT_SPLIT 2
#define DS_CONV_F_OUT_F32 4
#define DS_CONV_F_IN_F32 8

#define DS_CONV_TILE_HALO3_N16 13

typedef struct {
    const void* src0; const void* src1;
    int32_t C0, C1, H, W, H1, W1, off_h1, off_w1;
    const void* wpk;
    int32_t Cout, cout_pad, KH, KW, stride, pad_h, pad_w;
    int32_t Ho, Wo;
    int32_t transposed;
    void* out;
    int32_t out_C, out_c0;
    int32_t out_nchw_f32;
    const float* bias;
    const float* gn_ab;
    const float* fold_t1; const float* fold_t2;
    int32_t ncls;
    int32_t act;
    const void* res;
    float* stats_part;
    int32_t B, dtype, tile;
    int32_t ksplit;
    int32_t wk_order;
    int32_t batch_hint;
    float* slab;
    const float* gn_part; int32_t gn_parts; float gn_eps; double gn_count;
    const void* res_src0; const void* res_src1;
    int32_t res_C0, res_C1, res_H1, res_W1, res_off_h1, res_off_w1;
    int32_t res_steps;
    int32_t flags;
    const float* res_bias;
} ds_conv_params;

int ds_conv_igemm(const ds_conv_params* p, void* stream);
int ds_split_planes(const float* x, void* out_bf16, long long npix, int C, void* stream);
int ds_conv1x1_x3(const ds_conv_params* p, void* stream);
int ds_conv1x1_x3_stats_parts(const ds_conv_params* p);
size_t ds_conv1x1_x3_weight_elems(int Cin, int Cout);
int ds_conv_splitk_reduce(const ds_conv_params* p, void* stream);
int ds_conv_stats_parts(const ds_conv_params* p);
int ds_conv_tile_bn(int tile);

typedef struct {
    const float* w;
    const float* gamma;
    void* dst; int32_t dtype;
    int32_t Cout, Cin, cin_pad, KH, KW, cout_pad, transposed;
    int32_t k_order;
} ds_pack_conv_params;
int ds_pack_conv_weight(const ds_pack_conv_params* p, void* stream);
size_t ds_pack_conv_elems(int Cin_pad, int KH, int KW, int cout_pad, int transposed);
int ds_conv_fold_tables(const float* w, const float* bias, const float* gamma, const float* beta,
                        int Cout, int Cin, int KH, int KW, float* t1, float* t2, void* stream);

typedef struct {
    const void* src0; const void* src1;
    int32_t C0, C1, H, W, H1, W1, off_h1, off_w1;
    const float* wt;
    const float* bias;
    const float* tbias;
    int32_t tb_stride;
    void* out;
    float* stats_part;
    int32_t B, dtype;
    const void* wexp;
    int32_t out_split;
    int32_t strip;
    int32_t batch_hint;
} ds_dwconv_params;
int ds_dwconv7(const ds_dwconv_params* p, void* stream);
int ds_dwconv_stats_parts(const ds_dwconv_params* p);
#define DS_DW_DIRECT 0
#define DS_DW_TILE 1
#define DS_DW_STRIP 2
#define DS_DW_MFMA 3
int ds_dwconv_launch_choice(const ds_dwconv_params* p, int32_t* family, int32_t* ranges, int32_t* samples_per_chunk);
int ds_pack_dw_weight(const float* w_c1kk, int C, float* dst_tap_major, void* stream);
int ds_pack_dw_weight_mfma(const float* w_c1kk, int C, void* dst_bf16, void* stream);

int ds_gn_finalize(const float* stats_part, int B, int parts, double count, float eps, float* gn_ab, void* stream);
int ds_gn_stats(const void* x, int dtype, int B, int HW, int C, int G, float eps, float* gn_ab, void* stream);
size_t ds_gn_stats_ws_floats(int B, int HW, int C);
int ds_gn_stats_stream(const void* x, int dtype, int B, int HW, int C, int G, float eps, float* ws, float* gn_ab, void* stream);
typedef struct {
    const void* x; const void* res; void* out;
    const float* gn_ab;
    const float* gamma; const float* beta;
    const float* cbias;
    int32_t cb_stride;
    int32_t B, HW, C, G, act, dtype;
    const float* gn_part; int32_t gn_parts; float gn_eps; double gn_count;
} ds_gn_apply_params;
int ds_gn_apply(const ds_gn_apply_params* p, void* stream);

typedef struct {
    const void* qkv;
    int32_t B, N, heads, dtype;
    int32_t nseg;
    float* part;
    float* ctx;
    const float* label_q;
    const float* label_k; const float* label_v;
    int32_t lq_stride, lk_stride, lv_stride;
    int32_t q_softmax;
    float scale;
    void* out;
} ds_attn_params;
int ds_linattn_context(const ds_attn_params* p, void* stream);
int ds_linattn_output(const ds_attn_params* p, void* stream);
size_t ds_linattn_part_floats(int B, int heads, int nseg);

typedef struct {
    const void* x;
    int32_t B, N, C, nseg;
    const void* wqkv;
    const float* t1; const float* t2;
    const float* gn_ab;
    const float* gn_part; int32_t gn_parts; float gn_eps; double gn_count;
    const float* label_q;
    int32_t lq_stride; float scale;
    float* part; float* ctx;
    const void* wout_perm;
    const float* bias_out;
    void* y;
    float* stats_part;
    void* mfold;
    int32_t gen;
    int32_t batch_hint;
} ds_attn_fused_params;
int ds_pack_attn_fused(const float* wqkv_384xC, const float* gamma_C, const float* wout_Cx128, void* wqkv_bf16,
                       void* wout_perm_bf16, int C, void* stream);
int ds_attn_fused_context(const ds_attn_fused_params* p, void* stream);
int ds_attn_fused_output(const ds_attn_fused_params* p, void* stream);
int ds_attn_fused_stats_parts(const ds_attn_fused_params* p);
int ds_attn_fused_segments(int B, int N, int C);
int ds_attn_fused_segments_gen(int B, int N, int C, int gen);
int ds_attn_fused_generations(const ds_attn_fused_params* p);

typedef struct {
    const void* x;
    int32_t B, N, C, nseg;
    const void* wqkv;
    const float* wq;
    const float* wout;
    const float* wnin;
    const float* bias;
    float* part; float* ctx;
    void* wfold;
    void* y;
    float* stats_ws;
} ds_vq_attn_params;
int ds_vq_attn_segments(int B, int N, int C);
size_t ds_vq_attn_wfold_bytes(int B, int C);
int ds_vq_attn_context(const ds_vq_attn_params* p, void* stream);
int ds_vq_attn_output(const ds_vq_attn_params* p, void* stream);

typedef struct {
    const float* x;
    int32_t B, N, C, nseg;
    const void* wqkv_hl;
    const float* t1; const float* t2;
    const float* gn_ab;
    const float* gn_part; int32_t gn_parts; float gn_eps; double gn_count;
    const float* label_q;
    int32_t lq_stride; float scale;
    float* part; float* ctx;
    void* qplanes;
    void* mfold;
    const float* wout;
    const float* bias_out;
    float* y;
    float* stats_part;
    float* out;
    const float* on_gamma; const float* on_beta;
    float on_eps;
    int32_t batch_hint;
    void* out_planes;
} ds_attn_x3_params;
int ds_pack_attn_x3(const float* wqkv_384xC, const float* gamma_C, void* wqkv_hl, int C, void* stream);
int ds_attn_x3_context(const ds_attn_x3_params* p, void* stream);
int ds_attn_x3_output(const ds_attn_x3_params* p, void* stream);
int ds_attn_x3_stats_parts(const ds_attn_x3_params* p);
int ds_attn_x3_segments(int B, int N, int C);
size_t ds_attn_x3_qplane_bytes(int B, int N);
size_t ds_attn_x3_mfold_bytes(int B, int C);

int ds_bounds_report(char* buf, int n, int reset);

size_t ds_conv3x3_f32_n4_weight_floats(int C);
int ds_pack_conv3x3_f32_n4(const float* w, const float* bias, int Cout, int C, float* dst, void* stream);
int ds_conv3x3_f32_n4(const float* x, int B, int H, int W, int C, const float* wpk, float* out, void* stream);

int ds_sinusoid(const int64_t* t, const float* freqs, int B, int half, float* out, void* stream);
int ds_linear(const float* x, int x_stride, const float* W, const float* bias, int B, int K, int O, int act_in,
              float* y, int y_stride, void* stream);
int ds_activation(const float* x, size_t n, int act, float* y, void* stream);

int ds_add_layernorm(const float* a, const float* r, const float* gamma, const float* beta, int B, int D, float eps,
                     float* out, void* stream);

int ds_nchw_to_nhwc(const float* x, int B, int C, int H, int W, void* out, int C_pad, int dtype, void* stream);
int ds_conv1x1_in_nchw(const float* x_nchw, int B, int Cin, int HW, const float* w, const float* bias, int Cout, void* out, void* stream);
int ds_dup_batch(const void* src, void* dst, size_t nbytes, void* stream);
int ds_nhwc_to_nchw(const void* x, int dtype, int B, int C, int C_stride, int H, int W, float* out, void* stream);

typedef struct {
    const float* x; const float* eps; const float* eps_cond;
    const float* noise; float* out;
    const float* coef;
    float cfg_scale;
    int32_t blend_mode;
    const float* guide; const float* init_noise; const float* mask;
    const float* qcoef;
    int32_t B, CHW, HW;
    int32_t mask_chw;
} ds_step_params;
int ds_ddim_step(const ds_step_params* p, void* stream);
#define DS_SR_X 0
#define DS_SR_EPS 1
#define DS_SR_EPSC 2
#define DS_SR_OUT 3
#define DS_SR_DUP 4
#define DS_SR_BLEND 5
#define DS_SR_MASK_CHW 6
#define DS_SR_NOISE 7
#define DS_SR_SAMPLE 8
#define DS_SR_DRAW_ROWS 9
#define DS_SR_DRAW_W 10
#define DS_SR_COLS 11
#define DS_SR_NI 12
#define DS_SR_COEF 0
#define DS_SR_Q0 5
#define DS_SR_Q1 6
#define DS_SR_CFG 7
#define DS_SR_NF 8
#define DS_SR_GUIDE 0
#define DS_SR_INIT 1
#define DS_SR_MASKP 2
#define DS_SR_DRAW 3
#define DS_SR_SEED 4
#define DS_SR_OFFSET 5
#define DS_SR_NP 6
typedef struct {
    const float* x; const float* eps; float* out;
    const int32_t* irow; const float* frow; const uint64_t* prow;
    const int32_t* cols;
    int32_t R, C, H, W;
    int32_t Bx, Beps, Bout, n_cols;
} ds_step_rows_params;
int ds_step_rows(const ds_step_rows_params* p, void* stream);
typedef struct {
    const float* x; const float* eps; const float* eps_cond;
    float* hist; float* out;
    const float* coef;
    float cfg_scale;
    int32_t blend_mode;
    const float* guide; const float* init_noise; const float* mask;
    const float* qcoef;
    int32_t B, C, H, W;
    int32_t mask_chw;
} ds_dpm_step_params;
int ds_dpm_step(const ds_dpm_step_params* p, void* stream);
int ds_dpm_step_rows(const ds_step_rows_params* p, const uint64_t* hrow, void* stream);
typedef struct {
    const float* eps_u; const float* eps_c; float* out;
    float* gain;
    float cfg_scale, phi;
    int32_t B, CHW;
} ds_cfg_rescale_params;
int ds_cfg_rescale(const ds_cfg_rescale_params* p, void* stream);
#define DS_CR_U 0
#define DS_CR_C 1
#define DS_CR_OUT 2
#define DS_CR_NI 3
#define DS_CR_SCALE 0
#define DS_CR_PHI 1
#define DS_CR_NF 2
typedef struct {
    float* eps;
    const int32_t* irow; const float* frow;
    float* gain;
    int32_t R, CHW, Beps;
} ds_cfg_rescale_rows_params;
int ds_cfg_rescale_rows(const ds_cfg_rescale_rows_params* p, void* stream);
int ds_philox_normal(float* out, size_t n, uint64_t seed, uint64_t offset, void* stream);
int ds_gather_cols(const float* src, int rows, int src_w, const int32_t* cols, int out_w, float* out, void* stream);

int ds_vq_nearest(const float* z_nchw, const float* codebook, const float* code_sqnorm, int B, int D, int HW,
                  int ncodes, float* q_nchw, int64_t* idx, void* stream);
size_t ds_vq_stats_ws_bytes(int ncodes);
int ds_vq_stats(const float* z_nchw, const float* q_nchw, const int64_t* idx, int B, int D, int HW, int ncodes, float commitment_cost, int ema,
                float* out3, void* ws, void* stream);
int ds_decoder_tail(const void* x, int dtype, int B, int C_stride, int HW, float* out, void* stream);
size_t ds_conv3x3_c80_weight_elems(void);
int ds_pack_conv3x3_c80(const float* w, int Cout, int Cin, void* dst, void* stream);
int ds_conv3x3_c80(const void* x, int B, int H, int W, const void* wpk, const float* bias, void* out, const float* gn_ab, int G,
                   const float* gamma, const float* beta, int act, int add_x, float* stats_ws, void* stream);
int ds_conv3x3_c80_stats_slots(int B, int H, int W);
int ds_conv3x3_c80_res(const void* h, const void* res, int B, int H, int W, const void* wpk, const float* bias, void* out, float* stats_ws,
                       void* stream);
int ds_convt4x4_c80_stats_slots(int B, int H, int W, int Cin);
int ds_gn_stats_finish(const float* ws, int B, int nblk, int C, int G, int HW, float eps, float* ab, void* stream);

size_t ds_convt4x4_c80_weight_elems(int Cin);
int ds_pack_convt4x4_c80(const float* w, int Cin, int Cout, void* dst, void* stream);
int ds_convt4x4_c80(const void* x, int B, int H, int W, int Cin, const void* wpk, const float* bias, void* out, const float* gn_ab, int G,
                    const float* gamma, const float* beta, float* stats_ws, void* stream);

size_t ds_conv7x7_c4_weight_elems(void);
int ds_pack_conv7x7_c4(const float* w, int Cout, int Cin, void* dst, void* stream);
int ds_conv7x7_c4(const void* x, int B, int H, int W, int Cx, const void* wpk, const float* bias, void* out, void* stream);
int ds_pack_conv7x7_c4_x3(const float* w, int Cout, int Cin, void* dst, void* stream);
int ds_conv7x7_c4_x3(const float* x, int B, int H, int W, const void* wpk, const float* bias, float* out, void* stream);

int ds_dec_final(const void* x, int B, int H, int W, int C, const float* gn_ab, int G, const float* gamma, const float* beta,
                 const void* w3, const float* b3, const float* wnin, const float* bnin, float* out, void* stream);
int ds_istft_plus(const float* enc, int B, int F, int T, int hop, float* frames_ws, float* audio, void* stream);
size_t ds_istft_ws_floats(int B, int F, int T);
int ds_stft_plus(const float* audio, int B, int L, int hop, int reflect_pad, int T_out, float* enc, void* stream);
size_t ds_stft_images_ws_floats(int B, int F, int T);
int ds_stft_images(const float* enc, const float* amp, long long amp_batch_stride, int B, int F, int T, float* ws, unsigned char* spec_img,
                   unsigned char* phase_img, void* stream);
size_t ds_latent_image_ws_floats(int B, int C);
int ds_latent_image(const float* lat, int B, int C, int H, int W, float* ws, unsigned char* img, void* stream);

#define DS_PV_XOFF 0
#define DS_PV_LEN 1
#define DS_PV_FOFF 2
#define DS_PV_NF 3
#define DS_PV_TOFF 4
#define DS_PV_NOUT 5
#define DS_PV_SOFF 6
#define DS_PV_SLEN 7
#define DS_PV_NRES 8
#define DS_PV_NI 9
#define DS_RS_FC 0.95
#define DS_RS_ZEROS 32.0
#define DS_RS_BETA 12.0
int ds_pv_stft(const float* x, const int32_t* tab, int n_signals, int max_frames, long long total_samples, long long total_frames, float* spec,
               void* stream);
int ds_pv_vocode(const float* spec, const int32_t* tab, const int32_t* step_idx, const float* step_alpha, int n_signals, long long total_frames,
                 long long total_out, float* voc, void* stream);
size_t ds_pv_istft_ws_bytes(long long total_out);
int ds_pv_istft(const float* voc, const int32_t* tab, int n_signals, int max_out, int max_stretched, long long total_out, long long total_stretched,
                float* ws, float* y, void* stream);
int ds_resample_sinc(const float* ys, const int32_t* tab, const double* rates, int n_signals, int max_len, long long total_stretched,
                     long long total_samples, float* out, void* stream);
size_t ds_peak_normalize_ws_bytes(int n_signals, int max_len);
int ds_peak_normalize(const float* x, const int32_t* tab, int n_signals, int max_len, long long total_samples, float* ws, float* out, void* stream);
#define DS_MIX_BLOCK 1024
int ds_mix_notes(const float* notes, long long total_samples, const int32_t* ev, int n_events, const int32_t* blk_ptr, const int32_t* blk_ev,
                 int n_blk_ev, float* track, int track_len, void* stream);

size_t ds_lstm_ws_floats(int B, int H);
int ds_lstm_layer(const float* pre, long long pre_batch_stride, long long pre_step_stride, const float* w_hh, int B, int T, int H, float* hs,
                  float* h_last, float* ws, void* stream);
int ds_timbre_heads(float* y, int y_stride, int B, int n0, int n1, int n2, int n3, void* stream);

int ds_text_embed(const int64_t* input_ids, int B, int S, int pad_id, const float* word, int V, const float* pos, int P, const float* type0,
                  const float* gamma, const float* beta, int H, float eps, float* x, void* stream);
int ds_text_attention(const float* qkv, const void* mask, int mask_bytes, int B, int S, int heads, int d, float* ctx, void* stream);
#define DS_TAIL_TANH 0
#define DS_TAIL_RELU 1
#define DS_TAIL_L2NORM 2
int ds_text_tail(const float* x, int B, int D, int op, float eps, float* out, void* stream);

#ifdef __cplusplus
}
#endif
#endif
```

Before: 718.6 denoising-steps/s.

## Co-launch block's 3x3 conv1 with its 1x1 residual conv in one mixed grid

Adds a combined kernel whose 1-D grid holds the blocks of the halo3 3x3 conv and the blocks of the split-precision 1x1 residual projection. Each block decodes which half it belongs to through an interleaved chunk mapping. The engine rewrites the recorded op stream so the residual conv runs alongside conv1 in that launch, instead of as a separate launch after it. The aim is to cut one launch per ConvNeXt-style block and to fill the GPU better when either grid alone is small. The cost is extra aliasing validation, a shared LDS budget across both halves, and restriction to non-ksplit, non-pair-tile cases.

```diff
diff --git a/diffusynth_amd/_lib.py b/diffusynth_amd/_lib.py
--- a/diffusynth_amd/_lib.py
+++ b/diffusynth_amd/_lib.py
@@ -69,6 +69,7 @@
     "ds_conv_igemm": (C.c_int, [C.POINTER(ConvParams), _P]),
     "ds_conv_splitk_reduce": (C.c_int, [C.POINTER(ConvParams), _P]),
     "ds_conv1x1_x3": (C.c_int, [C.POINTER(ConvParams), _P]),
+    "ds_conv3x3_halo3_res": (C.c_int, [C.POINTER(ConvParams), C.POINTER(ConvParams), _P]),
     "ds_conv1x1_x3_stats_parts": (C.c_int, [C.POINTER(ConvParams)]),
     "ds_conv1x1_x3_weight_elems": (C.c_size_t, [_I, _I]),
     "ds_conv_stats_parts": (C.c_int, [C.POINTER(ConvParams)]),
diff --git a/diffusynth_amd/conv_policy.py b/diffusynth_amd/conv_policy.py
--- a/diffusynth_amd/conv_policy.py
+++ b/diffusynth_amd/conv_policy.py
@@ -82,6 +82,14 @@
     return ks
 
 
+def halo3_pair_tile(B, H, W):
+    return W <= 8 and 2 * H <= 32 and B >= 2
+
+
+def res_mixed(B, H, W, c1_cin, c1_cout, res_cin, res_cout, c1_ksplit, res_ksplit):
+    return c1_ksplit == 1 and res_ksplit == 1 and not halo3_pair_tile(B, H, W)
+
+
 def conv_meta(tile, B, Ho, Wo, Cout, kh, kw, transposed, cin, cin_real, res_cin=0):
     flops = 2.0 * B * Ho * Wo * Cout * (16 if transposed else kh * kw) * min(cin, cin_real)
     if res_cin:
diff --git a/diffusynth_amd/csrc/conv1x1_x3.hip b/diffusynth_amd/csrc/conv1x1_x3.hip
--- a/diffusynth_amd/csrc/conv1x1_x3.hip
+++ b/diffusynth_amd/csrc/conv1x1_x3.hip
@@ -1,170 +1,13 @@
-#include "common.hpp"
-#include "conv_halo3_common.hpp"
+#include "conv1x1_x3_body.hpp"
 
 namespace {
 
-constexpr int X3_OFF_XH = 0, X3_OFF_XL = BM * PSTR, X3_OFF_WH = 2 * BM * PSTR, X3_OFF_WL = X3_OFF_WH + B_BYTES, X3_OFF_SHL = X3_OFF_WL + B_BYTES;
-constexpr int X3_OFF_RED = X3_OFF_SHL + SHL_BYTES, X3_LDS = X3_OFF_RED + 64;
-constexpr int X3_XIT = BM * 8 / NT;
-constexpr int X3_WIT = 2 * BN * 4 / NT;
-
-static_assert(4 * EPI_F32_WAVE <= X3_OFF_SHL, "the epilogue's staging tiles reuse the x / w buffers, the shift table stays");
-
 __global__ __launch_bounds__(NT, DS_MINBLK) void conv1x1_x3_kernel(const ds_conv_params p) {
     extern __shared__ __attribute__((aligned(16))) char smem[];
-    float* const shl = reinterpret_cast<float*>(smem + X3_OFF_SHL);
-    float* const red = reinterpret_cast<float*>(smem + X3_OFF_RED);
-    const int tid = threadIdx.x, lane = tid & 63, wave = tid >> 6, m = lane & 15, q = lane >> 4;
-    const int gy = p.cout_pad / BN, HW = p.H * p.W, gx = (HW + BM - 1) / BM, nwg = gridDim.x;
+    const int nwg = gridDim.x;
     int wid = blockIdx.x;
     if ((nwg & 7) == 0) wid = (wid & 7) * (nwg >> 3) + (wid >> 3);
-    const int by = wid % gy, bxz = wid / gy, bx = bxz % gx;
-    const int zb = bxz / gx, ksplit = p.ksplit > 1 ? p.ksplit : 1, kz = zb / p.B;
-    const int b = zb - kz * p.B, n0 = by * BN, px0 = bx * BM;
-    const int NC0 = p.C0 >> 5, NCC = (p.C0 + p.C1) >> 5;
-    const int ncs = (NCC + ksplit - 1) / ksplit, c_lo = kz * ncs, c_hi = min(NCC, c_lo + ncs);
-    const bool raw = p.ksplit > 1;
-
-    const float* const sp0 = reinterpret_cast<const float*>(p.src0) + (size_t)b * HW * p.C0;
-    const float* const sp1 = p.C1 ? reinterpret_cast<const float*>(p.src1) + (size_t)b * p.H1 * p.W1 * p.C1 : nullptr;
-    unsigned off0[X3_XIT], off1[X3_XIT];
-#pragma unroll
-    for (int it = 0; it < X3_XIT; ++it) {
-        const int px = px0 + (tid >> 3) + 32 * it;
-        off0[it] = ((unsigned)(px * p.C0 + 4 * (tid & 7)) * 4u & 0x7fffffffu) | ((unsigned)(px >= HW) << 31);
-        off1[it] = 0x80000000u;
-        if (p.C1) {
-            const int h = px / p.W - p.off_h1, w = px % p.W - p.off_w1;
-            const unsigned bad = (unsigned)(px >= HW) | (unsigned)((unsigned)h >= (unsigned)p.H1) | (unsigned)((unsigned)w >= (unsigned)p.W1);
-            off1[it] = ((unsigned)((h * p.W1 + w) * p.C1 + 4 * (tid & 7)) * 4u & 0x7fffffffu) | (bad << 31);
-        }
-    }
-    const rsrc_t rs0 = __builtin_amdgcn_make_buffer_rsrc(const_cast<float*>(sp0), (short)0, HW * p.C0 * 4, 0x00020000);
-    const rsrc_t rs1 = __builtin_amdgcn_make_buffer_rsrc(const_cast<float*>(p.C1 ? sp1 : sp0), (short)0, p.C1 ? p.H1 * p.W1 * p.C1 * 4 : 0, 0x00020000);
-    const char* const wbase = reinterpret_cast<const char*>(p.wpk);
-    const size_t wchunk = (size_t)2 * p.cout_pad * 64;
-    f32x4 rx[X3_XIT];
-    u32x4 rw[X3_WIT];
-    auto load_chunk = [&](int cc) {
-        const bool first = cc < NC0;
-        const float* const s = first ? sp0 : sp1;
-        const int c0 = (first ? cc : cc - NC0) * 32;
-#if DS_BOUNDS
-#pragma unroll
-        for (int it = 0; it < X3_XIT; ++it) {
-            const unsigned o = first ? off0[it] : off1[it];
-            const bool in = o < 0x80000000u;
-            const f32x4 v = DS_LD(f32x4, reinterpret_cast<const f32x4*>(reinterpret_cast<const char*>(s) + (in ? o + c0 * 4 : 0)), first ? DS_BX_SRC0 : DS_BX_SRC1);
-            rx[it] = in ? v : f32x4{0.f, 0.f, 0.f, 0.f};
-        }
-#else
-        (void)s;
-#pragma unroll
-        for (int it = 0; it < X3_XIT; ++it)
-            rx[it] = __builtin_bit_cast(f32x4, __builtin_amdgcn_raw_buffer_load_b128(first ? rs0 : rs1, (int)((first ? off0[it] : off1[it]) + c0 * 4), 0, 0));
-#endif
-#pragma unroll
-        for (int it = 0; it < X3_WIT; ++it) {
-            const int piece = tid + it * NT, plane = piece / (BN * 4), r = piece - plane * (BN * 4);
-            rw[it] = DS_LD(u32x4, reinterpret_cast<const u32x4*>(wbase + (size_t)cc * wchunk + ((size_t)plane * p.cout_pad + n0) * 64 + (size_t)r * 16), DS_BX_W);
-        }
-    };
-    auto store_chunk = [&]() {
-#pragma unroll
-        for (int it = 0; it < X3_XIT; ++it) {
-            const int pl = (tid >> 3) + 32 * it, e = tid & 7;
-            const int a = pl * PSTR + ((((e >> 1) ^ (((pl >> 2) & 1) << 1))) << 4) + ((e & 1) << 3);
-            const f32x4 v = rx[it];
-            uint2 hi, lo;
-            ds_split2(v[0], v[1], hi.x, lo.x);
-            ds_split2(v[2], v[3], hi.y, lo.y);
-            *reinterpret_cast<uint2*>(smem + X3_OFF_XH + a) = hi;
-            *reinterpret_cast<uint2*>(smem + X3_OFF_XL + a) = lo;
-        }
-#pragma unroll
-        for (int it = 0; it < X3_WIT; ++it) {
-            const int piece = tid + it * NT, plane = piece / (BN * 4), r = piece - plane * (BN * 4), row = r >> 2, qq = r & 3;
-            *reinterpret_cast<u32x4*>(smem + (plane ? X3_OFF_WL : X3_OFF_WH) + row * PSTR + ((qq ^ W_SWZ(row)) << 4)) = rw[it];
-        }
-    };
-
-    load_chunk(c_lo);
-    float gn_a = 1.f, gn_am = 0.f;
-    const bool fold = p.gn_ab != nullptr && !raw;
-    if (fold) {
-        gn_a = DS_LD(float, p.gn_ab + 2 * b, DS_BX_GNAB);
-        gn_am = DS_LD(float, p.gn_ab + 2 * b + 1, DS_BX_GNAB);
-    }
-    for (int e = tid; e < 10 * BN; e += NT) {
-        float v = 0.f;
-        const int n = n0 + e;
-        if (e < BN && n < p.Cout) {
-            if (fold) v = DS_LD(float, p.fold_t1 + n, DS_BX_T1) - gn_am * DS_LD(float, p.fold_t2 + n, DS_BX_T2);
-            else if (p.bias && !raw) v = DS_LD(float, p.bias + n, DS_BX_BIAS);
-        }
-        shl[e] = v;
-    }
-    int xa[XT];
-#pragma unroll
-    for (int i = 0; i < XT; ++i) {
-        const int pl = 64 * wave + 16 * i + m;
-        xa[i] = pl * PSTR + ((q ^ (((pl >> 2) & 1) << 1)) << 4);
-    }
-    const int wa = W_ROW0(m) * PSTR + ((q ^ ((-(m >> 2)) & 3)) << 4);
-    f32x4 acc[XT][WT];
-#pragma unroll
-    for (int i = 0; i < XT; ++i)
-#pragma unroll
-        for (int j = 0; j < WT; ++j) acc[i][j] = f32x4{0.f, 0.f, 0.f, 0.f};
-
-    for (int cc = c_lo; cc < c_hi; ++cc) {
-        store_chunk();
-        __syncthreads();
-        if (cc + 1 < c_hi) load_chunk(cc + 1);
-        bf16x8 xh[XT], xl[XT];
-#pragma unroll
-        for (int i = 0; i < XT; ++i) {
-            xh[i] = *reinterpret_cast<const bf16x8*>(smem + X3_OFF_XH + xa[i]);
-            xl[i] = *reinterpret_cast<const bf16x8*>(smem + X3_OFF_XL + xa[i]);
-        }
-#pragma unroll
-        for (int j = 0; j < WT; ++j) {
-            const bf16x8 wh = *reinterpret_cast<const bf16x8*>(smem + X3_OFF_WH + wa + EPI_CH(j) * PSTR);
-            const bf16x8 wl = *reinterpret_cast<const bf16x8*>(smem + X3_OFF_WL + wa + EPI_CH(j) * PSTR);
-#pragma unroll
-            for (int i = 0; i < XT; ++i) {
-                acc[i][j] = __builtin_amdgcn_mfma_f32_16x16x32_bf16(wl, xh[i], acc[i][j], 0, 0, 0);
-                acc[i][j] = __builtin_amdgcn_mfma_f32_16x16x32_bf16(wh, xl[i], acc[i][j], 0, 0, 0);
-                acc[i][j] = __builtin_amdgcn_mfma_f32_16x16x32_bf16(wh, xh[i], acc[i][j], 0, 0, 0);
-            }
-        }
-        __syncthreads();
-    }
-
-    auto coord2 = [&](int i, int mm) {
-        ConvCoord c;
-        const int px = px0 + 64 * wave + 16 * i + mm;
-        c.ok = px < HW;
-        c.ho = 0;
-        c.wo = 0;
-        c.pix = px;
-        return c;
-    };
-    auto coord = [&](int i) { return coord2(i, m); };
-    float s1 = 0.f, s2 = 0.f;
-    char* const stage = smem + wave * EPI_F32_WAVE;
-    if (raw) {
-        ds_conv_params qp = p;
-        qp.out = p.slab;
-        qp.out_C = (p.Cout + 7) / 8 * 8;
-        qp.out_c0 = 0;
-        qp.res = nullptr;
-        halo3_epilogue_rows_f32<false, false>(qp, acc, zb, n0, HW, shl, coord, coord2, stage, s1, s2, 1.0f, lane);
-        return;
-    }
-    if (p.res) halo3_epilogue_rows_f32<false, true>(p, acc, b, n0, HW, shl, coord, coord2, stage, s1, s2, gn_a, lane);
-    else halo3_epilogue_rows_f32<false, false>(p, acc, b, n0, HW, shl, coord, coord2, stage, s1, s2, gn_a, lane);
-    if (p.stats_part) block_stats_write(s1, s2, red, p.stats_part + ((size_t)b * (gx * gy) + by * gx + bx) * 2);
+    conv1x1_x3_body(p, smem, wid);
 }
 
 }
@@ -176,7 +19,7 @@
     return p->ksplit > 1 ? ds_conv_splitk_parts(p) : ((p->H * p->W + BM - 1) / BM) * (p->cout_pad / BN);
 }
 
-extern "C" int ds_conv1x1_x3(const ds_conv_params* p, void* stream) {
+int ds_conv1x1_x3_validate(const ds_conv_params* p) {
     DS_REQUIRE(p && p->src0 && p->wpk && p->out, "conv1x1_x3: null pointer");
     DS_REQUIRE(p->KH == 1 && p->KW == 1 && p->stride == 1 && p->pad_h == 0 && p->pad_w == 0 && !p->transposed && p->Ho == p->H && p->Wo == p->W,
                "conv1x1_x3: 1x1 stride 1 only");
@@ -198,6 +41,12 @@
                "conv1x1_x3: one sample of the output and of either source must stay below 2 GiB (32-bit buffer offsets)");
     if (!ds_aligned16(p->src0) || !ds_aligned16(p->wpk) || !ds_aligned16(p->out) || (p->C1 && !ds_aligned16(p->src1)) || (p->res && !ds_aligned16(p->res)))
         DS_FAIL(DS_EALIGN, "conv1x1_x3: tensors must be 16-byte aligned");
+    return DS_OK;
+}
+
+extern "C" int ds_conv1x1_x3(const ds_conv_params* p, void* stream) {
+    const int rc = ds_conv1x1_x3_validate(p);
+    if (rc) return rc;
     hipStream_t st = reinterpret_cast<hipStream_t>(stream);
     const int gx = (p->H * p->W + BM - 1) / BM, gy = p->cout_pad / BN;
     dim3 grid(gx * gy * p->B * (p->ksplit > 1 ? p->ksplit : 1));
diff --git a/diffusynth_amd/csrc/conv1x1_x3_body.hpp b/diffusynth_amd/csrc/conv1x1_x3_body.hpp
--- /dev/null
+++ b/diffusynth_amd/csrc/conv1x1_x3_body.hpp
@@ -0,0 +1,168 @@
+#pragma once
+#include "common.hpp"
+#include "conv_halo3_common.hpp"
+
+namespace {
+
+constexpr int X3_OFF_XH = 0, X3_OFF_XL = BM * PSTR, X3_OFF_WH = 2 * BM * PSTR, X3_OFF_WL = X3_OFF_WH + B_BYTES, X3_OFF_SHL = X3_OFF_WL + B_BYTES;
+constexpr int X3_OFF_RED = X3_OFF_SHL + SHL_BYTES, X3_LDS = X3_OFF_RED + 64;
+constexpr int X3_XIT = BM * 8 / NT;
+constexpr int X3_WIT = 2 * BN * 4 / NT;
+
+static_assert(4 * EPI_F32_WAVE <= X3_OFF_SHL, "the epilogue's staging tiles reuse the x / w buffers, the shift table stays");
+
+__device__ __forceinline__ void conv1x1_x3_body(const ds_conv_params& p, char* const smem, const int wid) {
+    float* const shl = reinterpret_cast<float*>(smem + X3_OFF_SHL);
+    float* const red = reinterpret_cast<float*>(smem + X3_OFF_RED);
+    const int tid = threadIdx.x, lane = tid & 63, wave = tid >> 6, m = lane & 15, q = lane >> 4;
+    const int gy = p.cout_pad / BN, HW = p.H * p.W, gx = (HW + BM - 1) / BM;
+    const int by = wid % gy, bxz = wid / gy, bx = bxz % gx;
+    const int zb = bxz / gx, ksplit = p.ksplit > 1 ? p.ksplit : 1, kz = zb / p.B;
+    const int b = zb - kz * p.B, n0 = by * BN, px0 = bx * BM;
+    const int NC0 = p.C0 >> 5, NCC = (p.C0 + p.C1) >> 5;
+    const int ncs = (NCC + ksplit - 1) / ksplit, c_lo = kz * ncs, c_hi = min(NCC, c_lo + ncs);
+    const bool raw = p.ksplit > 1;
+
+    const float* const sp0 = reinterpret_cast<const float*>(p.src0) + (size_t)b * HW * p.C0;
+    const float* const sp1 = p.C1 ? reinterpret_cast<const float*>(p.src1) + (size_t)b * p.H1 * p.W1 * p.C1 : nullptr;
+    unsigned off0[X3_XIT], off1[X3_XIT];
+#pragma unroll
+    for (int it = 0; it < X3_XIT; ++it) {
+        const int px = px0 + (tid >> 3) + 32 * it;
+        off0[it] = ((unsigned)(px * p.C0 + 4 * (tid & 7)) * 4u & 0x7fffffffu) | ((unsigned)(px >= HW) << 31);
+        off1[it] = 0x80000000u;
+        if (p.C1) {
+            const int h = px / p.W - p.off_h1, w = px % p.W - p.off_w1;
+            const unsigned bad = (unsigned)(px >= HW) | (unsigned)((unsigned)h >= (unsigned)p.H1) | (unsigned)((unsigned)w >= (unsigned)p.W1);
+            off1[it] = ((unsigned)((h * p.W1 + w) * p.C1 + 4 * (tid & 7)) * 4u & 0x7fffffffu) | (bad << 31);
+        }
+    }
+    const rsrc_t rs0 = __builtin_amdgcn_make_buffer_rsrc(const_cast<float*>(sp0), (short)0, HW * p.C0 * 4, 0x00020000);
+    const rsrc_t rs1 = __builtin_amdgcn_make_buffer_rsrc(const_cast<float*>(p.C1 ? sp1 : sp0), (short)0, p.C1 ? p.H1 * p.W1 * p.C1 * 4 : 0, 0x00020000);
+    const char* const wbase = reinterpret_cast<const char*>(p.wpk);
+    const size_t wchunk = (size_t)2 * p.cout_pad * 64;
+    f32x4 rx[X3_XIT];
+    u32x4 rw[X3_WIT];
+    auto load_chunk = [&](int cc) {
+        const bool first = cc < NC0;
+        const float* const s = first ? sp0 : sp1;
+        const int c0 = (first ? cc : cc - NC0) * 32;
+#if DS_BOUNDS
+#pragma unroll
+        for (int it = 0; it < X3_XIT; ++it) {
+            const unsigned o = first ? off0[it] : off1[it];
+            const bool in = o < 0x80000000u;
+            const f32x4 v = DS_LD(f32x4, reinterpret_cast<const f32x4*>(reinterpret_cast<const char*>(s) + (in ? o + c0 * 4 : 0)), first ? DS_BX_SRC0 : DS_BX_SRC1);
+            rx[it] = in ? v : f32x4{0.f, 0.f, 0.f, 0.f};
+        }
+#else
+        (void)s;
+#pragma unroll
+        for (int it = 0; it < X3_XIT; ++it)
+            rx[it] = __builtin_bit_cast(f32x4, __builtin_amdgcn_raw_buffer_load_b128(first ? rs0 : rs1, (int)((first ? off0[it] : off1[it]) + c0 * 4), 0, 0));
+#endif
+#pragma unroll
+        for (int it = 0; it < X3_WIT; ++it) {
+            const int piece = tid + it * NT, plane = piece / (BN * 4), r = piece - plane * (BN * 4);
+            rw[it] = DS_LD(u32x4, reinterpret_cast<const u32x4*>(wbase + (size_t)cc * wchunk + ((size_t)plane * p.cout_pad + n0) * 64 + (size_t)r * 16), DS_BX_W);
+        }
+    };
+    auto store_chunk = [&]() {
+#pragma unroll
+        for (int it = 0; it < X3_XIT; ++it) {
+            const int pl = (tid >> 3) + 32 * it, e = tid & 7;
+            const int a = pl * PSTR + ((((e >> 1) ^ (((pl >> 2) & 1) << 1))) << 4) + ((e & 1) << 3);
+            const f32x4 v = rx[it];
+            uint2 hi, lo;
+            ds_split2(v[0], v[1], hi.x, lo.x);
+            ds_split2(v[2], v[3], hi.y, lo.y);
+            *reinterpret_cast<uint2*>(smem + X3_OFF_XH + a) = hi;
+            *reinterpret_cast<uint2*>(smem + X3_OFF_XL + a) = lo;
+        }
+#pragma unroll
+        for (int it = 0; it < X3_WIT; ++it) {
+            const int piece = tid + it * NT, plane = piece / (BN * 4), r = piece - plane * (BN * 4), row = r >> 2, qq = r & 3;
+            *reinterpret_cast<u32x4*>(smem + (plane ? X3_OFF_WL : X3_OFF_WH) + row * PSTR + ((qq ^ W_SWZ(row)) << 4)) = rw[it];
+        }
+    };
+
+    load_chunk(c_lo);
+    float gn_a = 1.f, gn_am = 0.f;
+    const bool fold = p.gn_ab != nullptr && !raw;
+    if (fold) {
+        gn_a = DS_LD(float, p.gn_ab + 2 * b, DS_BX_GNAB);
+        gn_am = DS_LD(float, p.gn_ab + 2 * b + 1, DS_BX_GNAB);
+    }
+    for (int e = tid; e < 10 * BN; e += NT) {
+        float v = 0.f;
+        const int n = n0 + e;
+        if (e < BN && n < p.Cout) {
+            if (fold) v = DS_LD(float, p.fold_t1 + n, DS_BX_T1) - gn_am * DS_LD(float, p.fold_t2 + n, DS_BX_T2);
+            else if (p.bias && !raw) v = DS_LD(float, p.bias + n, DS_BX_BIAS);
+        }
+        shl[e] = v;
+    }
+    int xa[XT];
+#pragma unroll
+    for (int i = 0; i < XT; ++i) {
+        const int pl = 64 * wave + 16 * i + m;
+        xa[i] = pl * PSTR + ((q ^ (((pl >> 2) & 1) << 1)) << 4);
+    }
+    const int wa = W_ROW0(m) * PSTR + ((q ^ ((-(m >> 2)) & 3)) << 4);
+    f32x4 acc[XT][WT];
+#pragma unroll
+    for (int i = 0; i < XT; ++i)
+#pragma unroll
+        for (int j = 0; j < WT; ++j) acc[i][j] = f32x4{0.f, 0.f, 0.f, 0.f};
+
+    for (int cc = c_lo; cc < c_hi; ++cc) {
+        store_chunk();
+        __syncthreads();
+        if (cc + 1 < c_hi) load_chunk(cc + 1);
+        bf16x8 xh[XT], xl[XT];
+#pragma unroll
+        for (int i = 0; i < XT; ++i) {
+            xh[i] = *reinterpret_cast<const bf16x8*>(smem + X3_OFF_XH + xa[i]);
+            xl[i] = *reinterpret_cast<const bf16x8*>(smem + X3_OFF_XL + xa[i]);
+        }
+#pragma unroll
+        for (int j = 0; j < WT; ++j) {
+            const bf16x8 wh = *reinterpret_cast<const bf16x8*>(smem + X3_OFF_WH + wa + EPI_CH(j) * PSTR);
+            const bf16x8 wl = *reinterpret_cast<const bf16x8*>(smem + X3_OFF_WL + wa + EPI_CH(j) * PSTR);
+#pragma unroll
+            for (int i = 0; i < XT; ++i) {
+                acc[i][j] = __builtin_amdgcn_mfma_f32_16x16x32_bf16(wl, xh[i], acc[i][j], 0, 0, 0);
+                acc[i][j] = __builtin_amdgcn_mfma_f32_16x16x32_bf16(wh, xl[i], acc[i][j], 0, 0, 0);
+                acc[i][j] = __builtin_amdgcn_mfma_f32_16x16x32_bf16(wh, xh[i], acc[i][j], 0, 0, 0);
+            }
+        }
+        __syncthreads();
+    }
+
+    auto coord2 = [&](int i, int mm) {
+        ConvCoord c;
+        const int px = px0 + 64 * wave + 16 * i + mm;
+        c.ok = px < HW;
+        c.ho = 0;
+        c.wo = 0;
+        c.pix = px;
+        return c;
+    };
+    auto coord = [&](int i) { return coord2(i, m); };
+    float s1 = 0.f, s2 = 0.f;
+    char* const stage = smem + wave * EPI_F32_WAVE;
+    if (raw) {
+        ds_conv_params qp = p;
+        qp.out = p.slab;
+        qp.out_C = (p.Cout + 7) / 8 * 8;
+        qp.out_c0 = 0;
+        qp.res = nullptr;
+        halo3_epilogue_rows_f32<false, false>(qp, acc, zb, n0, HW, shl, coord, coord2, stage, s1, s2, 1.0f, lane);
+        return;
+    }
+    if (p.res) halo3_epilogue_rows_f32<false, true>(p, acc, b, n0, HW, shl, coord, coord2, stage, s1, s2, gn_a, lane);
+    else halo3_epilogue_rows_f32<false, false>(p, acc, b, n0, HW, shl, coord, coord2, stage, s1, s2, gn_a, lane);
+    if (p.stats_part) block_stats_write(s1, s2, red, p.stats_part + ((size_t)b * (gx * gy) + by * gx + bx) * 2);
+}
+
+}
diff --git a/diffusynth_amd/csrc/conv3x3_halo3.hip b/diffusynth_amd/csrc/conv3x3_halo3.hip
--- a/diffusynth_amd/csrc/conv3x3_halo3.hip
+++ b/diffusynth_amd/csrc/conv3x3_halo3.hip
@@ -7,6 +7,8 @@
 #endif
 
 #include "conv_halo3_common.hpp"
+#include "conv1x1_x3_body.hpp"
+#include "resmix_decode.hpp"
 
 namespace {
 
@@ -17,12 +19,11 @@
 #else
 #define DS_VGPR_ATTR
 #endif
-template <int TWL, bool HP, bool PAIR = false>
-__global__ __launch_bounds__(NT, PAIR ? 1 : DS_MINBLK) DS_VGPR_ATTR void conv3x3_halo3_kernel(const ds_conv_params p) {
+template <int TWL, bool HP, bool PAIR>
+__device__ __forceinline__ void conv3x3_halo3_body(const ds_conv_params& p, char* const smem, const int wid, const int gx, const int gy, const int gz) {
     static_assert(!PAIR || (HP && TWL == 3), "two samples per block: the 8 x 32 tile of the split-precision instantiation");
     using G = HG<TWL>;
     constexpr int TW = G::TW, TH = G::TH, HCP = G::HCP, NPX = G::NPX, H_IT = G::H_IT, HH0 = G::HH0, HH1 = G::HH1;
-    extern __shared__ __attribute__((aligned(16))) char smem[];
     float* const shl = reinterpret_cast<float*>(smem + OFF_SHL);
     float* const red = reinterpret_cast<float*>(smem + OFF_B);
 
@@ -30,13 +31,10 @@
     const long st_k0 = DS_STAMP ? __builtin_amdgcn_s_memrealtime() : 0;
     const int m = lane & 15, q = lane >> 4;
     const int tiles_w = (p.W + TW - 1) >> TWL;
-    const int gx = gridDim.x, gy = gridDim.y, nwg = gx * gy * gridDim.z;
-    int wid = blockIdx.x + gx * (blockIdx.y + gy * blockIdx.z);
-    if ((nwg & 7) == 0) wid = (wid & 7) * (nwg >> 3) + (wid >> 3);
     constexpr int NGROUP = 2;
     int by, bxz;
     if (gy % NGROUP == 0 && gy > NGROUP) {
-        const int lo = wid % NGROUP, t = wid / NGROUP, nxz = gx * (int)gridDim.z;
+        const int lo = wid % NGROUP, t = wid / NGROUP, nxz = gx * gz;
         bxz = t % nxz;
         by = (t / nxz) * NGROUP + lo;
     } else {
@@ -506,7 +504,7 @@
     }
     __syncthreads();
     if (p.stats_part && !raw) {
-        const int parts = gridDim.x * gridDim.y;
+        const int parts = gx * gy;
         if constexpr (PAIR) {
             s1 = wave_sum(s1);
             s2 = wave_sum(s2);
@@ -532,6 +530,31 @@
     }
 }
 
+template <int TWL, bool HP, bool PAIR = false>
+__global__ __launch_bounds__(NT, PAIR ? 1 : DS_MINBLK) DS_VGPR_ATTR void conv3x3_halo3_kernel(const ds_conv_params p) {
+    extern __shared__ __attribute__((aligned(16))) char smem[];
+    const int gx = gridDim.x, gy = gridDim.y, gz = gridDim.z, nwg = gx * gy * gz;
+    int wid = blockIdx.x + gx * (blockIdx.y + gy * blockIdx.z);
+    if ((nwg & 7) == 0) wid = (wid & 7) * (nwg >> 3) + (wid >> 3);
+    conv3x3_halo3_body<TWL, HP, PAIR>(p, smem, wid, gx, gy, gz);
+}
+
+#if !DS_BOUNDS
+static_assert(X3_LDS <= HG<3>::LDS && X3_LDS <= HG<4>::LDS && X3_LDS <= HG<5>::LDS, "a res item fits the 3x3 block's LDS");
+template <int TWL>
+__global__ __launch_bounds__(NT, DS_MINBLK) DS_VGPR_ATTR void conv3x3_halo3_res_kernel(const ds_conv_params p3, const ds_conv_params p1, const int n3) {
+    extern __shared__ __attribute__((aligned(16))) char smem[];
+    const ResmixItem it = resmix_decode((int)blockIdx.x, n3, (int)gridDim.x - n3);
+    if (it.res) {
+        conv1x1_x3_body(p1, smem, it.item);
+    } else {
+        using G = HG<TWL>;
+        const int gx = ((p3.H + G::TH - 1) / G::TH) * ((p3.W + G::TW - 1) >> TWL), gy = p3.cout_pad / BN;
+        conv3x3_halo3_body<TWL, true, false>(p3, smem, it.item, gx, gy, p3.B);
+    }
+}
+#endif
+
 }
 
 int ds_conv3x3_halo3_parts(const ds_conv_params* p) {
@@ -541,7 +564,7 @@
 
 static int halo3_batch(const ds_conv_params* p) { return p->batch_hint > 0 ? p->batch_hint : p->B; }
 
-int ds_conv3x3_halo3_launch(const ds_conv_params* p, hipStream_t st) {
+static int halo3_validate(const ds_conv_params* p) {
     DS_REQUIRE(p->dtype == DS_BF16, "conv3x3_halo3: bf16 only");
     DS_REQUIRE(p->KH == 3 && p->KW == 3 && p->stride == 1 && p->pad_h == 1 && p->pad_w == 1 && !p->transposed,
                "conv3x3_halo3: 3x3 stride 1 pad 1 only");
@@ -572,6 +595,35 @@
                    (long long)(nchunks * 9 + p->res_steps) * p->cout_pad * 64 < (1ll << 31),
                "conv3x3_halo3: one sample / the packed weights must stay below 2 GiB (32-bit buffer offsets)");
     DS_REQUIRE((long long)p->H * p->W * p->out_C * (out_mode == 2 ? 4 : 2) < (1ll << 31), "conv3x3_halo3: one output sample must stay below 2 GiB (32-bit buffer offsets)");
+    return DS_OK;
+}
+
+static int halo3_gelu_table() {
+    static DsDevOnce once;
+    int dev;
+    if (once.need(&dev)) {
+        float h[GELU_TAB_N];
+        auto T = [](double a) { return a * 0.5 * erfc(a * 0.70710678118654752440); };
+        for (int i = 0; i < GELU_TAB_N; ++i) {
+            const unsigned lo = (unsigned)(GELU_TAB_BASE + i) << 16, hi = lo + 0x10000u;
+            float flo, fhi;
+            memcpy(&flo, &lo, 4);
+            memcpy(&fhi, &hi, 4);
+            h[i] = (float)T(0.5 * ((double)flo + (double)fhi));
+        }
+        hipError_t e = hipMemcpyToSymbol(HIP_SYMBOL(g_gelu_lut), h, sizeof(h));
+        if (e != hipSuccess) DS_FAIL(DS_ELAUNCH, "conv3x3_halo3: GELU table upload: %s", hipGetErrorString(e));
+        once.done(dev);
+    }
+    return DS_OK;
+}
+
+int ds_conv3x3_halo3_launch(const ds_conv_params* p, hipStream_t st) {
+    {
+        const int rc = halo3_validate(p);
+        if (rc) return rc;
+    }
+    [[maybe_unused]] const int nchunks = (p->flags & DS_CONV_F_SPLIT_IN) ? (p->C0 / 32) * 3 / 2 : p->C0 / 32, out_mode = (p->flags >> 1) & 3;
     const int twl = halo_twl(p->W), TW = 1 << twl, TH = BM >> twl;
     const bool pair = p->flags != 0 && twl == 3 && 2 * p->H <= TH && p->W <= TW && p->ksplit <= 1 && !p->res_steps && halo3_batch(p) >= 2;
     dim3 grid(((p->H + TH - 1) / TH) * ((p->W + TW - 1) / TW), p->cout_pad / BN, pair ? (p->B + 1) / 2 : p->B * (p->ksplit > 1 ? p->ksplit : 1));
@@ -591,22 +643,8 @@
     }
 #endif
     {
-        static DsDevOnce once;
-        int dev;
-        if (once.need(&dev)) {
-            float h[GELU_TAB_N];
-            auto T = [](double a) { return a * 0.5 * erfc(a * 0.70710678118654752440); };
-            for (int i = 0; i < GELU_TAB_N; ++i) {
-                const unsigned lo = (unsigned)(GELU_TAB_BASE + i) << 16, hi = lo + 0x10000u;
-                float flo, fhi;
-                memcpy(&flo, &lo, 4);
-                memcpy(&fhi, &hi, 4);
-                h[i] = (float)T(0.5 * ((double)flo + (double)fhi));
-            }
-            hipError_t e = hipMemcpyToSymbol(HIP_SYMBOL(g_gelu_lut), h, sizeof(h));
-            if (e != hipSuccess) DS_FAIL(DS_ELAUNCH, "conv3x3_halo3: GELU table upload: %s", hipGetErrorString(e));
-            once.done(dev);
-        }
+        const int rc = halo3_gelu_table();
+        if (rc) return rc;
     }
     int lds = twl == 3 ? HG<3>::LDS : (twl == 4 ? HG<4>::LDS : HG<5>::LDS);
 #define DS_H3_LAUNCH(TWL_, HP_, PAIR_)                                                                        \
@@ -632,6 +670,66 @@
     return DS_OK;
 }
 
+int ds_conv_igemm_validate(const ds_conv_params* p);
+int ds_conv1x1_x3_validate(const ds_conv_params* p);
+extern "C" int ds_conv1x1_x3(const ds_conv_params* p, void* stream);
+
+extern "C" int ds_conv3x3_halo3_res(const ds_conv_params* conv, const ds_conv_params* res, void* stream) {
+    DS_REQUIRE(conv && res, "conv3x3_halo3_res: null parameter struct");
+    DS_REQUIRE(conv->ksplit <= 1 && res->ksplit <= 1, "conv3x3_halo3_res: whole-K launches only (ksplit %d / %d)", conv->ksplit, res->ksplit);
+    int rc = ds_conv_igemm_validate(conv);
+    if (rc) return rc;
+    DS_REQUIRE(conv->tile == DS_CONV_TILE_HALO3_256x96, "conv3x3_halo3_res: the 3x3 half runs on DS_CONV_TILE_HALO3_256x96, not tile %d", conv->tile);
+    if ((rc = halo3_validate(conv)) != DS_OK) return rc;
+    if ((rc = ds_conv1x1_x3_validate(res)) != DS_OK) return rc;
+    const int twl = halo_twl(conv->W), TW = 1 << twl, TH = BM >> twl;
+    const bool pair = twl == 3 && 2 * conv->H <= TH && conv->W <= TW && halo3_batch(conv) >= 2;
+    DS_REQUIRE(conv->flags != 0 && !pair, "conv3x3_halo3_res: the 3x3 half must be a split-precision launch (flags != 0) off the two-sample tile");
+    DS_REQUIRE(conv->B == res->B && conv->H == res->H && conv->W == res->W, "conv3x3_halo3_res: the halves differ in B / H / W (%d %d %d against %d %d %d)",
+               conv->B, conv->H, conv->W, res->B, res->H, res->W);
+    {
+        const long long npx = (long long)conv->B * conv->H * conv->W, out_mode = (conv->flags >> 1) & 3;
+        auto overlap = [](const void* a, long long na, const void* b, long long nb) {
+            const char *pa = static_cast<const char*>(a), *pb = static_cast<const char*>(b);
+            return a && b && na > 0 && nb > 0 && pa < pb + nb && pb < pa + na;
+        };
+        const long long n_ro = npx * res->out_C * 4, n_co = npx * conv->out_C * (out_mode == 2 ? 4 : 2);
+        const int parts3 = ds_conv3x3_halo3_parts(conv), parts1 = ((res->H * res->W + BM - 1) / BM) * (res->cout_pad / BN);
+        const long long n_cs = (long long)conv->B * parts3 * 8, n_rs = (long long)res->B * parts1 * 8;
+        const bool bad = overlap(res->out, n_ro, conv->src0, npx * conv->C0 * 2) || overlap(res->out, n_ro, conv->out, n_co) ||
+                         overlap(res->out, n_ro, conv->res, n_co) || overlap(res->out, n_ro, conv->stats_part, n_cs) ||
+                         overlap(res->out, n_ro, conv->gn_part, (long long)conv->B * conv->gn_parts * 8) ||
+                         overlap(res->stats_part, n_rs, conv->src0, npx * conv->C0 * 2) || overlap(res->stats_part, n_rs, conv->out, n_co) ||
+                         overlap(res->stats_part, n_rs, conv->stats_part, n_cs) ||
+                         overlap(conv->out, n_co, res->src0, npx * res->C0 * 4) ||
+                         overlap(conv->out, n_co, res->C1 ? res->src1 : nullptr, (long long)res->B * res->H1 * res->W1 * res->C1 * 4) ||
+                         overlap(conv->out, n_co, res->res, n_ro) || overlap(conv->stats_part, n_cs, res->src0, npx * res->C0 * 4);
+        DS_REQUIRE(!bad, "conv3x3_halo3_res: the output of one half aliases a tensor of the other");
+    }
+#if DS_BOUNDS
+    if ((rc = ds_conv3x3_halo3_launch(conv, reinterpret_cast<hipStream_t>(stream))) != DS_OK) return rc;
+    return ds_conv1x1_x3(res, stream);
+#else
+    const long long n3 = (long long)ds_conv3x3_halo3_parts(conv) * conv->B;
+    const long long n1 = (long long)((res->H * res->W + BM - 1) / BM) * (res->cout_pad / BN) * res->B;
+    DS_REQUIRE(n3 + n1 < (1ll << 31), "conv3x3_halo3_res: %lld + %lld blocks are beyond a 1-D grid", n3, n1);
+    if ((rc = halo3_gelu_table()) != DS_OK) return rc;
+    hipStream_t st = reinterpret_cast<hipStream_t>(stream);
+    const dim3 grid((unsigned)(n3 + n1));
+#define DS_H3R_LAUNCH(TWL_)                                                                                                        \
+    do {                                                                                                                           \
+        DS_SET_MAX_LDS((conv3x3_halo3_res_kernel<TWL_>), 100 * 1024, "conv3x3_halo3_res");                                         \
+        hipLaunchKernelGGL((conv3x3_halo3_res_kernel<TWL_>), grid, dim3(NT), HG<TWL_>::LDS, st, *conv, *res, (int)n3);             \
+    } while (0)
+    if (twl == 5) DS_H3R_LAUNCH(5);
+    else if (twl == 4) DS_H3R_LAUNCH(4);
+    else DS_H3R_LAUNCH(3);
+#undef DS_H3R_LAUNCH
+    DS_CHECK_LAUNCH("conv3x3_halo3_res");
+    return DS_OK;
+#endif
+}
+
 #if DS_BOUNDS
 extern "C" int ds_bounds_fetch_conv_halo3(ds_bounds_rec* out, int reset) { return ds_bounds_fetch_tu(out, reset); }
 #endif
diff --git a/diffusynth_amd/csrc/conv_igemm.hip b/diffusynth_amd/csrc/conv_igemm.hip
--- a/diffusynth_amd/csrc/conv_igemm.hip
+++ b/diffusynth_amd/csrc/conv_igemm.hip
@@ -371,6 +371,8 @@
 
 }
 
+int ds_conv_igemm_validate(const ds_conv_params* p) { return validate(p); }
+
 int ds_conv_splitk_parts(const ds_conv_params* p);
 int ds_conv3x3_halo3_launch(const ds_conv_params* p, hipStream_t st);
 int ds_conv3x3_halo3_parts(const ds_conv_params* p);
diff --git a/diffusynth_amd/csrc/resmix_decode.hpp b/diffusynth_amd/csrc/resmix_decode.hpp
--- /dev/null
+++ b/diffusynth_amd/csrc/resmix_decode.hpp
@@ -0,0 +1,21 @@
+#pragma once
+#if defined(__HIPCC__) || defined(__CUDACC__)
+#define RESMIX_HD __host__ __device__
+#else
+#define RESMIX_HD
+#endif
+
+struct ResmixItem {
+    int res;
+    int item;
+};
+
+RESMIX_HD inline ResmixItem resmix_decode(int L, int n3, int n1) {
+    const bool chunked = ((n3 | n1) & 7) == 0;
+    const int x = chunked ? (L & 7) : 0, s = chunked ? (L >> 3) : L;
+    const int c3 = chunked ? (n3 >> 3) : n3, c1 = chunked ? (n1 >> 3) : n1;
+    ResmixItem r;
+    r.res = s >= c3;
+    r.item = r.res ? x * c1 + (s - c3) : x * c3 + s;
+    return r;
+}
diff --git a/diffusynth_amd/engine.py b/diffusynth_amd/engine.py
--- a/diffusynth_amd/engine.py
+++ b/diffusynth_amd/engine.py
@@ -505,6 +505,7 @@
 
 class UnetEngine(_EngineBase):
     use_cfg_pair = True
+    use_res_mixed = True
 
     def __init__(self, module, compute_dtype="fp32"):
         self._init_common(module, compute_dtype)
@@ -732,6 +733,8 @@
         self.op("ds_dwconv7", C.byref(p))
         src1_, st1 = self.stats_src(h, dim * H * W)
         g = self.conv(d["conv1"], h, pad=1, gn_src=src1_, act=L.ACT_GELU, want_stats=True, out_split=sp)
+        out = self._res_mixed(d, h, s0, s1, off1) if sp else None
+        mixed = out is not None
         self.free(h)
         self.free_raw(st1)
         src2_, st2 = self.stats_src(g, d["conv1"].Cout * H * W)
@@ -739,10 +742,29 @@
         if c2.res_steps and self._halo3_ksplit(c2, g, g.split) == 1:
             out = self.conv(c2, g, pad=1, gn_src=src2_, want_stats=want_stats, res_fuse=(s0, s1, off1))
         else:
-            out = self.conv(d["res"], s0, s1, off1) if d["res"] is not None else None
+            if not mixed:
+                out = self.conv(d["res"], s0, s1, off1) if d["res"] is not None else None
             out = self.conv(c2, g, pad=1, gn_src=src2_, res=s0 if out is None else out, want_stats=want_stats, out=out)
         self.free(g)
         self.free_raw(st2)
+        return out
+
+    def _res_mixed(self, d, h, s0, s1, off1):
+        e, rc, c1 = self.e, d["res"], d["conv1"]
+        if not e.use_res_mixed or rc is None or rc.w_x3 is None or s0.split or s0.C % 32 or (s1 is not None and s1.C % 32):
+            return None
+        H, W, cin = s0.H, s0.W, s0.C + (s1.C if s1 is not None else 0)
+        if not policy.res_mixed(self.Btile, H, W, h.C, c1.Cout, cin, rc.Cout, self._halo3_ksplit(c1, h, True),
+                                policy.x3_1x1_ksplit(self.Btile, H, W, rc.x3_cout_pad, cin // 32)):
+            return None
+        k = len(self.ops) - 1
+        assert self.ops[k].name == "ds_conv_igemm" and k in self.conv_meta, "conv1 of the block is not the last recorded op"
+        out = self.conv(rc, s0, s1, off1)
+        assert len(self.ops) == k + 2 and self.ops[k + 1].name == "ds_conv1x1_x3"
+        res_op = self.ops.pop()
+        self.ops[k] = _Op("ds_conv3x3_halo3_res", self.lib.ds_conv3x3_halo3_res, (self.ops[k].args[0], res_op.args[0]), None)
+        tile, flops, desc = self.conv_meta[k]
+        self.conv_meta[k] = (tile, flops + 2.0 * self.B * H * W * rc.Cout * cin, desc + f" | mixed 1x1 {cin}->{rc.Cout}")
         return out
 
     def resnet(self, d, x, want_stats):
diff --git a/include/diffusynth_hip.h b/include/diffusynth_hip.h
--- a/include/diffusynth_hip.h
+++ b/include/diffusynth_hip.h
@@ -66,6 +66,7 @@
 int ds_conv_igemm(const ds_conv_params* p, void* stream);
 int ds_split_planes(const float* x, void* out_bf16, long long npix, int C, void* stream);
 int ds_conv1x1_x3(const ds_conv_params* p, void* stream);
+int ds_conv3x3_halo3_res(const ds_conv_params* conv, const ds_conv_params* res, void* stream);
 int ds_conv1x1_x3_stats_parts(const ds_conv_params* p);
 size_t ds_conv1x1_x3_weight_elems(int Cin, int Cout);
 int ds_conv_splitk_reduce(const ds_conv_params* p, void* stream);
```

Result: no change. 718.8 denoising-steps/s, median of 2 (+0.0%).
